# LCSL/nys-koop-lqr

Hardware: AMD Instinct MI355X
Metric: Nyström-Koopman fits/sec (K_nm build + A,B,C solve), N=1e5 m=2000 d=384 (higher is better)
Workload: dtype f64

## Files before the change

### include/nyskoop.h

```cpp
#ifndef NYSKOOP_H
#define NYSKOOP_H

#include <stdint.h>

#ifdef __cplusplus
extern "C" {
#endif

#define NK_ABI_VERSION 2

enum {
  NK_OK = 0,
  NK_ERR_BAD_ARG = -1,
  NK_ERR_HIP = -2,
  NK_ERR_NOT_SPD = -3,
  NK_ERR_OOM = -4,
  NK_ERR_NO_CONVERGENCE = -5,
  NK_ERR_NO_DEVICE = -6
};

enum { NK_KERNEL_RBF = 0, NK_KERNEL_MATERN52 = 1, NK_KERNEL_LINEAR = 2, NK_KERNEL_TPS = 3 };

typedef struct nk_kernel_desc {
  int32_t type;
  int32_t d;
  int32_t n_lengthscale;
  int32_t reserved;
  const double* lengthscale;
  double sigma0;
} nk_kernel_desc;

typedef struct nk_fit_stats {
  double ms_total;
  double ms_upload;
  double ms_kmat;
  double ms_gram;
  double ms_sqrt;
  double ms_solve;
  double ms_gram_kernel_avg;
  int32_t gram_kernel_launches;
  int32_t sqrt_iters;
  double sqrt_residual;
  double gram_flops;
  double kmat_pairs;
  int32_t rank_inner;
  int32_t rank_inner_rec;
  double pivot_ratio_inner;
  double pivot_ratio_inner_rec;
  int32_t refined;
  int32_t reserved_;
  double refine_ratio_inner;
  double refine_ratio_inner_rec;
} nk_fit_stats;

typedef struct nk_ctx nk_ctx;
typedef struct nk_model nk_model;

int nk_version(void);
const char* nk_last_error(void);
int nk_device_count(void);
int nk_create(int device, nk_ctx** out);
int nk_destroy(nk_ctx* ctx);
int nk_synchronize(nk_ctx* ctx);
void* nk_stream(nk_ctx* ctx);
int nk_set_kmat_mode(nk_ctx* ctx, int mode);
int nk_set_strict_spd(nk_ctx* ctx, int strict);
int nk_set_refine(nk_ctx* ctx, double pivot_ratio, int32_t steps);
#define NK_DTYPE_F64 0
#define NK_DTYPE_F32 1
int nk_set_compute_dtype(nk_ctx* ctx, int dtype);
int nk_wait_stream(nk_ctx* ctx, void* producer_stream);
int nk_group_create(int device, int size, nk_ctx** members);
typedef struct nk_cv_unit {
  const nk_kernel_desc* kernel;
  double gamma;
  double jitter;
  int32_t m;
  int32_t reserved;
  int64_t test_begin, test_end;
  const int64_t* landmark_rows;
} nk_cv_unit;
int nk_cv_grid(nk_ctx* const* members, int32_t n_members, const double* X, int64_t ldx, const double* Y, int64_t ldy,
               int64_t n, int32_t d, int32_t p, const nk_cv_unit* units, int32_t n_units, double* scores, int32_t* status);
typedef struct nk_spline_cv_unit {
  double gamma;
  int32_t m;
  int32_t reserved;
  int64_t test_begin, test_end;
  const double* centers;
} nk_spline_cv_unit;
int nk_spline_cv_grid(nk_ctx* const* members, int32_t n_members, const double* X, int64_t ldx, const double* Y,
                      int64_t ldy, int64_t n, int32_t d, int32_t p, const nk_spline_cv_unit* units, int32_t n_units,
                      double* scores, int32_t* status);
typedef struct nk_sysid_unit {
  const nk_kernel_desc* kernel;
  double gamma, jitter;
  int32_t m, n_ranges;
  const int64_t* row_ranges;
  const int64_t* landmark_rows;
  const double* centers;
  const int32_t* traj;
  int32_t n_traj, reserved;
} nk_sysid_unit;
int nk_sysid_grid(nk_ctx* const* members, int32_t n_members, const double* X, int64_t ldx, const double* Y, int64_t ldy,
                  int64_t n, int32_t d, int32_t p, const double* trajs, const double* U, int32_t n_trajs, int32_t T,
                  const nk_sysid_unit* units, int32_t n_units, double* err_abs, double* err_rel, int32_t* status);
int nk_group_enter(nk_ctx* member);
int nk_group_leave(nk_ctx* member);
int nk_group_stats(nk_ctx* member, uint64_t* out4);
int nk_runtime_counters(uint64_t* out, int32_t n);
int nk_shutdown(void);

void* nk_host_alloc(uint64_t bytes);
void nk_host_free(void* ptr);

int nk_kernel_matrix(nk_ctx* ctx, const nk_kernel_desc* kd,
                     const double* A, int64_t lda, int64_t nA,
                     const double* B, int64_t ldb, int64_t nB,
                     double* out, int64_t ldo);

int nk_nystrom_fit(nk_ctx* ctx, const nk_kernel_desc* kd,
                   const double* X, int64_t ldx, const double* Y, int64_t ldy,
                   int64_t n, int32_t d, int32_t p,
                   const int64_t* row_ranges, int32_t n_ranges,
                   const double* Zin, int64_t ldzi, const double* Zout, int64_t ldzo, int32_t m,
                   double gamma, double jitter,
                   nk_model** model, nk_fit_stats* stats);

int nk_gram_doubles(int32_t m, int32_t d, int32_t p, int64_t* count);
int nk_nystrom_gram(nk_ctx* ctx, const nk_kernel_desc* kd,
                    const double* X, int64_t ldx, const double* Y, int64_t ldy,
                    int64_t n, int32_t d, int32_t p,
                    const int64_t* row_ranges, int32_t n_ranges,
                    const double* Zin, int64_t ldzi, const double* Zout, int64_t ldzo, int32_t m,
                    double* gram, nk_fit_stats* stats);
int nk_nystrom_solve(nk_ctx* ctx, const nk_kernel_desc* kd,
                     const double* Zin, int64_t ldzi, const double* Zout, int64_t ldzo, int32_t m, int32_t d, int32_t p,
                     const double* gram, int64_t n_total, double gamma, double jitter,
                     nk_model** model, nk_fit_stats* stats);

int nk_model_create(nk_ctx* ctx, const nk_kernel_desc* kd, const double* Zout, int64_t ldz,
                    int32_t m, int32_t d, int32_t p, double jitter,
                    const double* A, const double* B, const double* C, const double* W,
                    nk_model** model);
int nk_model_destroy(nk_model* model);

int nk_spline_fit(nk_ctx* ctx, const double* X, int64_t ldx, const double* Y, int64_t ldy, int64_t n, int32_t d, int32_t p,
                  const int64_t* row_ranges, int32_t n_ranges, const double* centers, int64_t ldc, int32_t m, double gamma,
                  nk_model** model, nk_fit_stats* stats);
int nk_spline_model_create(nk_ctx* ctx, const double* centers, int64_t ldc, int32_t m, int32_t d, int32_t p,
                           const double* A, const double* B, const double* C, const double* W, nk_model** model);

int nk_model_get(nk_ctx* ctx, const nk_model* model, char which, double* out, int64_t ldo);
int nk_model_dims(const nk_model* model, int32_t* m, int32_t* d, int32_t* p);
int nk_model_get_ops(nk_ctx* ctx, const nk_model* model, double* G, int64_t ldg, double* C, int64_t ldc, double* W,
                     int64_t ldw);
int nk_model_get_ops_async(nk_ctx* ctx, nk_model* model, double* G, int64_t ldg, double* C, int64_t ldc, double* W,
                           int64_t ldw);
int nk_model_wait(nk_model* model);

int nk_lift(nk_ctx* ctx, const nk_model* model, const double* Xq, int64_t ldx, int64_t nq,
            double* out, int64_t ldo);

int nk_predict(nk_ctx* ctx, const nk_model* model, const double* Xaug, int64_t ldx, int64_t nq,
               double* out, int64_t ldo);

int nk_score_neg_rmse(nk_ctx* ctx, const nk_model* model, const double* Xaug, int64_t ldx,
                      const double* Ytrue, int64_t ldy, int64_t nq, double* score);

int nk_rollout(nk_ctx* ctx, const nk_model* model, const double* x0, int64_t ldx0,
               const double* U, int32_t T, int32_t batch, double* out_x, double* out_z);

int nk_rollout_err(nk_ctx* ctx, const nk_model* model, const double* traj, const double* U, int32_t T, int32_t batch,
                   double* err_abs, double* err_rel);

int nk_closed_loop(nk_ctx* ctx, const nk_model* model, const double* K, const double* phi0,
                   const double* phi_ref, int32_t steps, double* out_x, double* out_u);
int nk_closed_loop_batch(nk_ctx* ctx, const nk_model* model, const double* K, const double* phi0,
                         const double* phi_ref, int32_t steps, int32_t batch, double* out_x, double* out_u);
#define NK_PLANT_DUFFING 0
#define NK_PLANT_DOUBLE_INTEGRATOR 1
#define NK_PLANT_HJB 2
int nk_plant_step(int plant, double Ts, const double* x, const double* u, double* x_next);
int nk_plant_loop(nk_ctx* ctx, const nk_model* model, int plant, double Ts, const double* K, const double* x0,
                  const double* x_ref, int32_t steps, int32_t batch, double* out_x, double* out_u);
typedef struct nk_plant_unit {
  const nk_model* model;
  const double* K;
  const double* x0;
  const double* x_ref;
  int32_t uopt;
  int32_t reserved;
} nk_plant_unit;
int nk_plant_loop_multi(nk_ctx* ctx, int plant, double Ts, int32_t steps, const nk_plant_unit* units, int32_t n_units,
                        const double* u_opt, int32_t n_uopt, double* out_x, double* out_u, double* scores);
#define NK_DARE_WS_CAP_BYTES (1ll << 30)
typedef struct nk_dare_problem {
  int32_t m, p;
  const double* A; int64_t lda;
  const double* B; int64_t ldb;
  const double* Q; int64_t ldq;
  const double* R; int64_t ldr;
  double* out_K;
  double* out_P;
  double* out_delta;
} nk_dare_problem;
int nk_dare_batch(nk_ctx* ctx, const nk_dare_problem* problems, int32_t n, double tol, int32_t max_iter,
                  int32_t* out_status, int32_t* out_iters);
int nk_model_lqr_gain_batch(nk_ctx* ctx, const nk_model* const* models, int32_t n, double c, const double* R_or_NULL,
                            double tol, int32_t max_iter, double* out_K, int32_t* out_status, int32_t* out_iters);
int nk_model_lqr_cost(nk_ctx* ctx, const nk_model* model, double c, double* Q, int64_t ldq);
int nk_linear_rollout(nk_ctx* ctx, const double* A, const double* B, const double* C, int32_t m, int32_t d, int32_t p,
                      const double* z0, const double* U, int32_t T, int32_t batch, double* out_x, double* out_z);

int nk_gemm_f32(nk_ctx* ctx, int64_t M, int64_t N, int64_t K, const float* A, int64_t lda, const float* B, int64_t ldb,
                double* C, int64_t ldc);
int nk_gemm(nk_ctx* ctx, int transA, int transB, int64_t M, int64_t N, int64_t K, double alpha,
            const double* A, int64_t lda, const double* B, int64_t ldb, double beta, double* C, int64_t ldc);
int nk_sqrtm_spd(nk_ctx* ctx, const double* P, int64_t ldp, int32_t m, double* S, double* Sinv,
                 int32_t* iters, double* residual);
int nk_solve_spd(nk_ctx* ctx, const double* P, int64_t ldp, int32_t m, const double* R, int64_t ldr,
                 int32_t nrhs, double* X, int64_t ldxo);

int nk_bench_gram(nk_ctx* ctx, int64_t n, int32_t m, int32_t p, int32_t d, int32_t reps, double* ms_avg, double* flop);

#define NK_CHOL_FLOW_GIVEUP (-0x40000000)
int nk_chol_aug(nk_ctx* ctx, int32_t nsys, const double* const* P, const int64_t* ldp, const int32_t* m,
                const double* const* R, const int32_t* extra, double* const* L, double* const* X, int32_t* failed,
                double* piv_ratio);

#ifdef __cplusplus
}
#endif
#endif
```

### nys_koop_lqr_amd/_lib.py

```python
import atexit
import ctypes as C
import os
import sys
import threading

import numpy as np

_HERE = os.path.dirname(os.path.abspath(__file__))

NK_KERNEL_RBF, NK_KERNEL_MATERN52, NK_KERNEL_LINEAR, NK_KERNEL_TPS = 0, 1, 2, 3
NK_PLANT_DUFFING, NK_PLANT_DOUBLE_INTEGRATOR, NK_PLANT_HJB = 0, 1, 2
NK_OK = 0
_ERR_NAMES = {-1: "NK_ERR_BAD_ARG", -2: "NK_ERR_HIP", -3: "NK_ERR_NOT_SPD", -4: "NK_ERR_OOM",
              -5: "NK_ERR_NO_CONVERGENCE", -6: "NK_ERR_NO_DEVICE"}


class NyskoopError(RuntimeError):
    def __init__(self, code, msg):
        super().__init__(f"{_ERR_NAMES.get(code, code)}: {msg}")
        self.code = code


class KernelDesc(C.Structure):
    _fields_ = [("type", C.c_int32), ("d", C.c_int32), ("n_lengthscale", C.c_int32), ("reserved", C.c_int32),
                ("lengthscale", C.POINTER(C.c_double)), ("sigma0", C.c_double)]


class CvUnit(C.Structure):
    _fields_ = [("kernel", C.POINTER(KernelDesc)), ("gamma", C.c_double), ("jitter", C.c_double), ("m", C.c_int32),
                ("reserved", C.c_int32), ("test_begin", C.c_int64), ("test_end", C.c_int64),
                ("landmark_rows", C.POINTER(C.c_int64))]


class SplineCvUnit(C.Structure):
    _fields_ = [("gamma", C.c_double), ("m", C.c_int32), ("reserved", C.c_int32), ("test_begin", C.c_int64),
                ("test_end", C.c_int64), ("centers", C.POINTER(C.c_double))]


class SysidUnit(C.Structure):
    _fields_ = [("kernel", C.POINTER(KernelDesc)), ("gamma", C.c_double), ("jitter", C.c_double), ("m", C.c_int32),
                ("n_ranges", C.c_int32), ("row_ranges", C.POINTER(C.c_int64)), ("landmark_rows", C.POINTER(C.c_int64)),
                ("centers", C.POINTER(C.c_double)), ("traj", C.POINTER(C.c_int32)), ("n_traj", C.c_int32),
                ("reserved", C.c_int32)]


class PlantUnit(C.Structure):
    _fields_ = [("model", C.c_void_p), ("K", C.c_void_p), ("x0", C.c_void_p), ("x_ref", C.c_void_p),
                ("uopt", C.c_int32), ("reserved", C.c_int32)]


class DareProblem(C.Structure):
    _fields_ = [("m", C.c_int32), ("p", C.c_int32), ("A", C.c_void_p), ("lda", C.c_int64), ("B", C.c_void_p),
                ("ldb", C.c_int64), ("Q", C.c_void_p), ("ldq", C.c_int64), ("R", C.c_void_p), ("ldr", C.c_int64),
                ("out_K", C.c_void_p), ("out_P", C.c_void_p), ("out_delta", C.c_void_p)]


class FitStats(C.Structure):
    _fields_ = [("ms_total", C.c_double), ("ms_upload", C.c_double), ("ms_kmat", C.c_double),
                ("ms_gram", C.c_double), ("ms_sqrt", C.c_double), ("ms_solve", C.c_double),
                ("ms_gram_kernel_avg", C.c_double), ("gram_kernel_launches", C.c_int32),
                ("sqrt_iters", C.c_int32), ("sqrt_residual", C.c_double), ("gram_flops", C.c_double),
                ("kmat_pairs", C.c_double), ("rank_inner", C.c_int32), ("rank_inner_rec", C.c_int32),
                ("pivot_ratio_inner", C.c_double), ("pivot_ratio_inner_rec", C.c_double), ("refined", C.c_int32),
                ("reserved_", C.c_int32), ("refine_ratio_inner", C.c_double), ("refine_ratio_inner_rec", C.c_double)]

    def as_dict(self):
        return {k: getattr(self, k) for k, _ in self._fields_}


_P = C.c_void_p
_I64 = C.c_int64
_I32 = C.c_int32
_D = C.c_double

SIGNATURES = {
    "nk_version": (C.c_int, []),
    "nk_last_error": (C.c_char_p, []),
    "nk_device_count": (C.c_int, []),
    "nk_create": (C.c_int, [C.c_int, C.POINTER(_P)]),
    "nk_destroy": (C.c_int, [_P]),
    "nk_synchronize": (C.c_int, [_P]),
    "nk_stream": (_P, [_P]),
    "nk_set_kmat_mode": (C.c_int, [_P, C.c_int]),
    "nk_set_strict_spd": (C.c_int, [_P, C.c_int]),
    "nk_set_refine": (C.c_int, [_P, C.c_double, C.c_int32]),
    "nk_wait_stream": (C.c_int, [_P, _P]),
    "nk_shutdown": (C.c_int, []),
    "nk_group_create": (C.c_int, [C.c_int, C.c_int, C.POINTER(_P)]),
    "nk_group_enter": (C.c_int, [_P]),
    "nk_group_leave": (C.c_int, [_P]),
    "nk_set_compute_dtype": (C.c_int, [_P, C.c_int]),
    "nk_group_stats": (C.c_int, [_P, C.POINTER(C.c_uint64)]),
    "nk_runtime_counters": (C.c_int, [C.POINTER(C.c_uint64), C.c_int32]),
    "nk_cv_grid": (C.c_int, [C.POINTER(_P), _I32, _P, _I64, _P, _I64, _I64, _I32, _I32, C.POINTER(CvUnit), _I32,
                             C.POINTER(_D), C.POINTER(_I32)]),
    "nk_spline_cv_grid": (C.c_int, [C.POINTER(_P), _I32, _P, _I64, _P, _I64, _I64, _I32, _I32, C.POINTER(SplineCvUnit),
                                    _I32, C.POINTER(_D), C.POINTER(_I32)]),
    "nk_sysid_grid": (C.c_int, [C.POINTER(_P), _I32, _P, _I64, _P, _I64, _I64, _I32, _I32, _P, _P, _I32, _I32,
                                C.POINTER(SysidUnit), _I32, C.POINTER(_D), C.POINTER(_D), C.POINTER(_I32)]),
    "nk_host_alloc": (_P, [C.c_uint64]),
    "nk_host_free": (None, [_P]),
    "nk_kernel_matrix": (C.c_int, [_P, C.POINTER(KernelDesc), _P, _I64, _I64, _P, _I64, _I64, _P, _I64]),
    "nk_nystrom_fit": (C.c_int, [_P, C.POINTER(KernelDesc), _P, _I64, _P, _I64, _I64, _I32, _I32,
                                 C.POINTER(_I64), _I32, _P, _I64, _P, _I64, _I32, _D, _D,
                                 C.POINTER(_P), C.POINTER(FitStats)]),
    "nk_gram_doubles": (C.c_int, [_I32, _I32, _I32, C.POINTER(_I64)]),
    "nk_nystrom_gram": (C.c_int, [_P, C.POINTER(KernelDesc), _P, _I64, _P, _I64, _I64, _I32, _I32,
                                  C.POINTER(_I64), _I32, _P, _I64, _P, _I64, _I32, _P, C.POINTER(FitStats)]),
    "nk_nystrom_solve": (C.c_int, [_P, C.POINTER(KernelDesc), _P, _I64, _P, _I64, _I32, _I32, _I32, _P, _I64, _D, _D,
                                   C.POINTER(_P), C.POINTER(FitStats)]),
    "nk_model_create": (C.c_int, [_P, C.POINTER(KernelDesc), _P, _I64, _I32, _I32, _I32, _D, _P, _P, _P, _P,
                                  C.POINTER(_P)]),
    "nk_spline_fit": (C.c_int, [_P, _P, _I64, _P, _I64, _I64, _I32, _I32, C.POINTER(_I64), _I32, _P, _I64, _I32, _D,
                                C.POINTER(_P), C.POINTER(FitStats)]),
    "nk_spline_model_create": (C.c_int, [_P, _P, _I64, _I32, _I32, _I32, _P, _P, _P, _P, C.POINTER(_P)]),
    "nk_model_destroy": (C.c_int, [_P]),
    "nk_model_get": (C.c_int, [_P, _P, C.c_char, _P, _I64]),
    "nk_model_dims": (C.c_int, [_P, C.POINTER(_I32), C.POINTER(_I32), C.POINTER(_I32)]),
    "nk_model_get_ops": (C.c_int, [_P, _P, _P, _I64, _P, _I64, _P, _I64]),
    "nk_model_get_ops_async": (C.c_int, [_P, _P, _P, _I64, _P, _I64, _P, _I64]),
    "nk_model_wait": (C.c_int, [_P]),
    "nk_lift": (C.c_int, [_P, _P, _P, _I64, _I64, _P, _I64]),
    "nk_predict": (C.c_int, [_P, _P, _P, _I64, _I64, _P, _I64]),
    "nk_score_neg_rmse": (C.c_int, [_P, _P, _P, _I64, _P, _I64, _I64, C.POINTER(_D)]),
    "nk_rollout": (C.c_int, [_P, _P, _P, _I64, _P, _I32, _I32, _P, _P]),
    "nk_rollout_err": (C.c_int, [_P, _P, _P, _P, _I32, _I32, C.POINTER(_D), C.POINTER(_D)]),
    "nk_closed_loop": (C.c_int, [_P, _P, _P, _P, _P, _I32, _P, _P]),
    "nk_closed_loop_batch": (C.c_int, [_P, _P, _P, _P, _P, _I32, _I32, _P, _P]),
    "nk_plant_step": (C.c_int, [C.c_int, _D, _P, _P, _P]),
    "nk_plant_loop": (C.c_int, [_P, _P, C.c_int, _D, _P, _P, _P, _I32, _I32, _P, _P]),
    "nk_plant_loop_multi": (C.c_int, [_P, C.c_int, _D, _I32, C.POINTER(PlantUnit), _I32, _P, _I32, _P, _P, _P]),
    "nk_dare_batch": (C.c_int, [_P, C.POINTER(DareProblem), _I32, _D, _I32, C.POINTER(_I32), C.POINTER(_I32)]),
    "nk_model_lqr_gain_batch": (C.c_int, [_P, C.POINTER(_P), _I32, _D, _P, _D, _I32, _P, C.POINTER(_I32),
                                          C.POINTER(_I32)]),
    "nk_model_lqr_cost": (C.c_int, [_P, _P, _D, _P, _I64]),
    "nk_linear_rollout": (C.c_int, [_P, _P, _P, _P, _I32, _I32, _I32, _P, _P, _I32, _I32, _P, _P]),
    "nk_gemm_f32": (C.c_int, [_P, _I64, _I64, _I64, _P, _I64, _P, _I64, _P, _I64]),
    "nk_gemm": (C.c_int, [_P, C.c_int, C.c_int, _I64, _I64, _I64, _D, _P, _I64, _P, _I64, _D, _P, _I64]),
    "nk_sqrtm_spd": (C.c_int, [_P, _P, _I64, _I32, _P, _P, C.POINTER(_I32), C.POINTER(_D)]),
    "nk_solve_spd": (C.c_int, [_P, _P, _I64, _I32, _P, _I64, _I32, _P, _I64]),
    "nk_bench_gram": (C.c_int, [_P, _I64, _I32, _I32, _I32, _I32, C.POINTER(_D), C.POINTER(_D)]),
    "nk_chol_aug": (C.c_int, [_P, _I32, _P, _P, _P, _P, _P, _P, _P, _P, _P]),
}

_lib = None
_lib_lock = threading.Lock()


def library_path():
    return os.environ.get("NYSKOOP_LIB", os.path.join(_HERE, "libnyskoop.so"))


def load_library():
    global _lib
    with _lib_lock:
        if _lib is None:
            path = library_path()
            if not os.path.exists(path):
                raise NyskoopError(-6, f"{path} not found: build it with `python -c 'import __graft_entry__ as g; "
                                       f"g.build()'` or `make -C nys_koop_lqr_amd/csrc` (there is no CPU fallback)")
            if os.environ.get("NYSKOOP_PRELOAD_TORCH", "1") == "1" and "torch" not in sys.modules:
                try:
                    import torch
                except Exception:
                    pass
            lib = C.CDLL(path)
            for name, (res, args) in SIGNATURES.items():
                fn = getattr(lib, name)
                fn.restype = res
                fn.argtypes = args
            _lib = lib
            atexit.register(shutdown)
    return _lib


def shutdown():
    lib = _lib
    if lib is None:
        return
    with _pools_lock:
        pools = list(_pools.values())
        _pools.clear()
        lpools = list(_lockstep_pools.values())
        _lockstep_pools.clear()
    for pool in pools:
        pool.shutdown(wait=True)
    for pool in lpools:
        pool.close()
    _PinnedBlock.drain()
    lib.nk_shutdown()


def check(rc):
    if rc != NK_OK:
        raise NyskoopError(rc, load_library().nk_last_error().decode("utf-8", "replace"))


def runtime_counters():
    v = (C.c_uint64 * 5)()
    check(load_library().nk_runtime_counters(v, 5))
    return dict(chain_giveups=int(v[0]), jacobi_giveups=int(v[1]), rank_truncated_fits=int(v[2]), sqrt_retries=int(v[3]),
                refined_fits=int(v[4]))


def torch_if_cuda():
    try:
        import torch
    except Exception:
        return None
    try:
        return torch if torch.cuda.is_available() else None
    except Exception:
        return None


class Mat:

    def __init__(self, obj, rows=None, cols=None):
        if hasattr(obj, "data_ptr") and hasattr(obj, "stride"):
            if str(getattr(obj, "dtype", "")).split(".")[-1] not in ("float64", "double"):
                raise TypeError("device tensors must be float64")
            if obj.dim() != 2 or (obj.shape[1] > 1 and obj.stride(1) != 1):
                raise ValueError("device tensors must be 2-D with unit inner stride")
            self.owner, self.ptr, self.ld = obj, obj.data_ptr(), int(obj.stride(0))
            self.shape = (int(obj.shape[0]), int(obj.shape[1]))
        else:
            a = np.asarray(obj, dtype=np.float64)
            if a.ndim == 1:
                a = a.reshape(1, -1)
            if a.ndim != 2:
                raise ValueError("expected a 2-D array")
            if a.shape[1] > 0 and a.shape[0] > 0 and (a.strides[1] != 8 or a.strides[0] % 8 or a.strides[0] < 8 * a.shape[1]):
                a = np.ascontiguousarray(a)
            self.owner, self.ptr = a, a.ctypes.data
            self.ld = a.strides[0] // 8 if a.shape[0] > 1 else max(a.shape[1], 1)
            self.shape = a.shape
        if self.shape[0] <= 1:
            self.ld = max(self.ld, self.shape[1], 1)
        if rows is not None and self.shape[0] != rows or cols is not None and self.shape[1] != cols:
            raise ValueError(f"expected a {rows} x {cols} matrix, got {self.shape}")


class Context:

    def __init__(self, device=0, handle=None):
        self.lib = load_library()
        if handle is None:
            handle = _P()
            check(self.lib.nk_create(int(device), C.byref(handle)))
        self.handle = handle
        self.device = int(device)

    def enter(self):
        check(self.lib.nk_group_enter(self.handle))

# ... 445 lines not shown
```

### nys_koop_lqr_amd/csrc/nk_api.hip

```cpp
#include "nk_common.h"
#include "nk_api_internal.h"

#include <cmath>
#include <cstdarg>
#include <cstdio>
#include <cstring>
#include <cstdlib>
#include <algorithm>
#include <mutex>
#include <set>

namespace nk {

static thread_local std::string g_err;

void set_error(const char* fmt, ...) {
  char buf[1024];
  va_list ap;
  va_start(ap, fmt);
  vsnprintf(buf, sizeof(buf), fmt, ap);
  va_end(ap);
  g_err = buf;
}

// ... 477 lines not shown

int nk_set_compute_dtype(nk_ctx* ctx, int dtype) {
  NK_REQUIRE(ctx != nullptr && (dtype == NK_DTYPE_F64 || dtype == NK_DTYPE_F32), "nk_set_compute_dtype: bad argument");
  ctx->compute_f32 = dtype == NK_DTYPE_F32 ? 1 : 0;
  return NK_OK;
}

int nk_set_strict_spd(nk_ctx* ctx, int strict) {
  NK_REQUIRE(ctx != nullptr && strict >= 0 && strict <= 2, "nk_set_strict_spd: bad argument");
  ctx->strict_spd = strict;
  return NK_OK;
}

int nk_set_refine(nk_ctx* ctx, double pivot_ratio, int32_t steps) {
  NK_REQUIRE(ctx != nullptr && pivot_ratio >= 0.0 && pivot_ratio <= 1.0 && steps >= 0 && steps <= 8, "nk_set_refine: bad argument");
  ctx->refine_pivot = pivot_ratio;
  ctx->refine_steps = steps;
  return NK_OK;
}

int nk_wait_stream(nk_ctx* ctx, void* producer_stream) {
  NK_REQUIRE(ctx != nullptr, "nk_wait_stream: null context");
  NK_HIP(hipSetDevice(ctx->device));
  if (ctx->group) {
    hipError_t e = real_stream_sync(reinterpret_cast<hipStream_t>(producer_stream));
    if (e != hipSuccess) { set_error("synchronising the producer stream failed: %s", hipGetErrorString(e)); return NK_ERR_HIP; }
    return NK_OK;
  }
  NK_HIP(hipEventRecord(ctx->ev_ext, reinterpret_cast<hipStream_t>(producer_stream)));
  NK_HIP(hipStreamWaitEvent(ctx->stream_main, ctx->ev_ext, 0));
  NK_HIP(hipStreamWaitEvent(ctx->stream_side, ctx->ev_ext, 0));
  NK_HIP(hipStreamWaitEvent(ctx->stream_prep, ctx->ev_ext, 0));
  NK_HIP(hipStreamWaitEvent(ctx->stream_copy, ctx->ev_ext, 0));
  return NK_OK;
}

int nk_group_create(int device, int size, nk_ctx** out) {
  NK_REQUIRE(out != nullptr && size >= 1 && size <= 256, "nk_group_create: bad argument");
  for (int i = 0; i < size; ++i) out[i] = nullptr;
  for (int i = 0; i < size; ++i) {
    int rc = nk_create(device, &out[i]);
    if (rc != NK_OK) {
      for (int j = 0; j < i; ++j) { nk_destroy(out[j]); out[j] = nullptr; }
      return rc;
    }
  }
  nk_group* g = group_new(device, size);
  if (!g) {
    for (int i = 0; i < size; ++i) { nk_destroy(out[i]); out[i] = nullptr; }
    set_error("nk_group_create: could not create the shared stream / argument table");
    return NK_ERR_HIP;
  }
  for (int i = 0; i < size; ++i) group_attach(g, i, out[i]);
  return NK_OK;
}

int nk_group_enter(nk_ctx* ctx) {
  NK_REQUIRE(ctx != nullptr, "nk_group_enter: null context");
  return group_enter(ctx);
}

int nk_group_leave(nk_ctx* ctx) {
  NK_REQUIRE(ctx != nullptr, "nk_group_leave: null context");
  tl_ctx = ctx;
  const int rc = group_leave(ctx);
  tl_ctx = nullptr;
  return rc;
}

int nk_runtime_counters(uint64_t* out, int32_t n) {
  NK_REQUIRE(out != nullptr && n >= 0, "nk_runtime_counters: bad argument");
  for (int i = 0; i < n && i < CNT_N; ++i) out[i] = nk::read_counter(i);
  return NK_OK;
}

int nk_group_stats(nk_ctx* ctx, uint64_t* out4) {
  NK_REQUIRE(ctx != nullptr && out4 != nullptr, "nk_group_stats: null argument");
  group_stats(ctx, out4);
  return NK_OK;
}

int nk_synchronize(nk_ctx* ctx) {
  NK_REQUIRE(ctx != nullptr, "null context");
  tl_ctx = ctx;
  NK_HIP(hipStreamSynchronize(ctx->stream));
  return NK_OK;
}

void* nk_stream(nk_ctx* ctx) { return ctx ? reinterpret_cast<void*>(ctx->stream) : nullptr; }

void* nk_host_alloc(uint64_t bytes) {
  void* p = nullptr;
  if (hipHostMalloc(&p, bytes ? bytes : 1, hipHostMallocDefault) != hipSuccess) {
    (void)hipGetLastError();
    set_error("hipHostMalloc of %llu bytes failed", (unsigned long long)bytes);
    return nullptr;
  }
  std::lock_guard<std::mutex> lk(g_reg_mu);
  g_host_blocks.insert(p);
  return p;
}

void nk_host_free(void* ptr) {
  if (!ptr) return;
  {
    std::lock_guard<std::mutex> lk(g_reg_mu);
    if (g_host_blocks.erase(ptr) == 0) return;
  }
  (void)hipHostFree(ptr);
}

int nk_set_kmat_mode(nk_ctx* ctx, int mode) {
  NK_REQUIRE(ctx != nullptr && (mode == 0 || mode == 1), "nk_set_kmat_mode: bad argument");
  ctx->kmat_mode = mode;
  return NK_OK;
}

int nk_kernel_matrix(nk_ctx* ctx, const nk_kernel_desc* kd, const double* A, int64_t lda, int64_t nA, const double* B,
                     int64_t ldb, int64_t nB, double* out, int64_t ldo) {
  NK_TRY(check_ctx(ctx));
  NK_REQUIRE(kd && A && B && out, "nk_kernel_matrix: null argument");
  NK_REQUIRE(nA >= 0 && nB >= 0 && kd->d > 0, "nk_kernel_matrix: negative size");
  NK_REQUIRE(lda >= kd->d && ldb >= kd->d && ldo >= nB, "nk_kernel_matrix: leading dimension too small");
  if (nA == 0 || nB == 0) return NK_OK;
  const int d = kd->d;
  double* winv = nullptr;
  NK_TRY(arena_alloc_t(ctx, (size_t)d, &winv));
  NK_TRY(make_winv(ctx, kd, d, winv));
  MatIn a, b;
  NK_TRY(stage_in(ctx, A, lda, nA, d, &a));
  NK_TRY(stage_in(ctx, B, ldb, nB, d, &b));
  MatOut o;
  NK_TRY(stage_out(ctx, out, ldo, nA, nB, &o));
  if (kd->type == NK_KERNEL_TPS && ctx->kmat_mode == 0 && d >= 32 && nA >= 2 && nB >= 2) {
    const int64_t lta = (nA + 1) & ~(int64_t)1, ltb = (nB + 1) & ~(int64_t)1;
    double *center = nullptr, *At = nullptr, *sqa = nullptr, *Bt = nullptr, *sqb = nullptr;
    NK_TRY(arena_alloc_t(ctx, (size_t)d, &center));
    NK_TRY(arena_alloc_t(ctx, (size_t)d * lta, &At));
    NK_TRY(arena_alloc_t(ctx, (size_t)nA, &sqa));
    NK_TRY(arena_alloc_t(ctx, (size_t)d * ltb, &Bt));
    NK_TRY(arena_alloc_t(ctx, (size_t)nB, &sqb));
    NK_TRY(launch_colmean(ctx, b.ptr, b.ld, (int)nB, d, center));
    NK_TRY(prep_rows(ctx, a.ptr, a.ld, nA, d, winv, center, At, lta, sqa));
    NK_TRY(prep_rows(ctx, b.ptr, b.ld, nB, d, winv, center, Bt, ltb, sqb));
    NK_TRY(launch_kmat_gram(ctx, NK_KERNEL_TPS, At, lta, sqa, nA, Bt, ltb, sqb, nB, d, 0.0, o.dev, o.ld));
  } else {
    NK_TRY(launch_kmat(ctx, kd->type, a.ptr, a.ld, nA, b.ptr, b.ld, nB, d, winv, kd->sigma0, o.dev, o.ld));
  }
  NK_TRY(finish_out(ctx, o));
  NK_HIP(hipStreamSynchronize(ctx->stream));
  return NK_OK;
}

int nk_model_create(nk_ctx* ctx, const nk_kernel_desc* kd, const double* Zout, int64_t ldz, int32_t m, int32_t d,
                    int32_t p, double jitter, const double* A, const double* B, const double* C, const double* W,
                    nk_model** model) {
  NK_TRY(check_ctx(ctx));
  NK_REQUIRE(kd && Zout && model, "nk_model_create: null argument");
  NK_REQUIRE(m > 0 && d > 0 && p >= 0 && ldz >= d, "nk_model_create: bad sizes");
  NK_REQUIRE(kd->type != NK_KERNEL_TPS, "nk_model_create: spline models come from nk_spline_model_create");
  *model = nullptr;
  nk_model* mdl = nullptr;
  NK_TRY(model_alloc(ctx, m, d, p, &mdl));
  struct Guard { nk_model* m; ~Guard() { if (m) nk_model_destroy(m); } } guard{mdl};
  mdl->ktype = kd->type; mdl->sigma0 = kd->sigma0; mdl->jitter = jitter;
  NK_TRY(make_winv(ctx, kd, d, mdl->winv));
  MatIn z;
  NK_TRY(stage_in(ctx, Zout, ldz, m, d, &z));
  NK_TRY(launch_copy2d(ctx, z.ptr, z.ld, mdl->Z, d, m, d));
  double* Kj = nullptr;
  NK_TRY(arena_alloc_t(ctx, (size_t)m * m, &Kj));
  NK_TRY(launch_kmat(ctx, kd->type, mdl->Z, d, m, mdl->Z, d, m, d, mdl->winv, kd->sigma0, Kj, m));
  NK_TRY(launch_add_diag(ctx, Kj, m, m, jitter));
  NK_TRY(sqrtm_spd(ctx, Kj, m, m, mdl->S, mdl->Sinv, nullptr, nullptr));
  const int mp = m + p;
  if (A && C) {
    NK_REQUIRE(p == 0 || B != nullptr, "nk_model_create: B missing");
    MatIn a, b, c, w;
    NK_TRY(stage_in(ctx, A, m, m, m, &a));
    NK_TRY(launch_copy2d(ctx, a.ptr, a.ld, mdl->A, mp, m, m));
    if (p > 0) {
      NK_TRY(stage_in(ctx, B, p, m, p, &b));
      NK_TRY(launch_copy2d(ctx, b.ptr, b.ld, mdl->B, mp, m, p));
    }
    NK_TRY(stage_in(ctx, C, m, d, m, &c));
    NK_TRY(launch_copy2d(ctx, c.ptr, c.ld, mdl->C, m, d, m));
    if (W) {
      NK_TRY(stage_in(ctx, W, mp, d, mp, &w));
      NK_TRY(launch_copy2d(ctx, w.ptr, w.ld, mdl->W, mp, d, mp));
    } else {
      NK_TRY(launch_gemm(ctx, false, false, d, mp, m, 1.0, mdl->C, m, mdl->A, mp, 0.0, mdl->W, mp));
    }
    mdl->has_ops = true;
  }
  NK_HIP(hipStreamSynchronize(ctx->stream));
  guard.m = nullptr;
  *model = mdl;
  return NK_OK;
}

int nk_spline_model_create(nk_ctx* ctx, const double* centers, int64_t ldc, int32_t m, int32_t d, int32_t p,
                           const double* A, const double* B, const double* C, const double* W, nk_model** model) {
  NK_TRY(check_ctx(ctx));
  NK_REQUIRE(centers && model, "nk_spline_model_create: null argument");
  NK_REQUIRE(m > 0 && d > 0 && p >= 0 && ldc >= d, "nk_spline_model_create: bad sizes");
  *model = nullptr;
  nk_model* mdl = nullptr;
  NK_TRY(model_alloc(ctx, m, d, p, &mdl, NK_MODEL_SPLINE));
  struct Guard { nk_model* m; ~Guard() { if (m) nk_model_destroy(m); } } guard{mdl};
  mdl->ktype = NK_KERNEL_TPS; mdl->sigma0 = 0.0; mdl->jitter = 0.0;
  NK_TRY(launch_fill(ctx, mdl->winv, d, 1, d, 1.0));
  MatIn z;
  NK_TRY(stage_in(ctx, centers, ldc, m, d, &z));
  NK_TRY(launch_copy2d(ctx, z.ptr, z.ld, mdl->Z, d, m, d));
  const int mp = m + p;
  if (A && C) {
    NK_REQUIRE(p == 0 || B != nullptr, "nk_spline_model_create: B missing");
    MatIn a, b, c, w;
    NK_TRY(stage_in(ctx, A, m, m, m, &a));
    NK_TRY(launch_copy2d(ctx, a.ptr, a.ld, mdl->A, mp, m, m));
    if (p > 0) {
      NK_TRY(stage_in(ctx, B, p, m, p, &b));
      NK_TRY(launch_copy2d(ctx, b.ptr, b.ld, mdl->B, mp, m, p));
    }
    NK_TRY(stage_in(ctx, C, m, d, m, &c));
    NK_TRY(launch_copy2d(ctx, c.ptr, c.ld, mdl->C, m, d, m));
    if (W) {
      NK_TRY(stage_in(ctx, W, mp, d, mp, &w));
      NK_TRY(launch_copy2d(ctx, w.ptr, w.ld, mdl->W, mp, d, mp));
    } else {
      NK_TRY(launch_gemm(ctx, false, false, d, mp, m, 1.0, mdl->C, m, mdl->A, mp, 0.0, mdl->W, mp));
    }
    mdl->has_ops = true;
  }
  NK_HIP(hipStreamSynchronize(ctx->stream));
  guard.m = nullptr;
  *model = mdl;
  return NK_OK;
}

int nk_model_destroy(nk_model* model) {
  if (!model) return NK_OK;
  {
    std::lock_guard<std::mutex> lk(g_reg_mu);
    if (g_models.erase(model) == 0) return NK_OK;
  }
  destroy_model_unregistered(model, true);
  return NK_OK;
}

int nk_model_dims(const nk_model* model, int32_t* m, int32_t* d, int32_t* p) {
  NK_REQUIRE(model != nullptr, "null model");
  if (m) *m = model->m;
  if (d) *d = model->d;
  if (p) *p = model->p;
  return NK_OK;
}

int nk_model_get(nk_ctx* ctx, const nk_model* mdl, char which, double* out, int64_t ldo) {
  NK_TRY(check_ctx(ctx));
  NK_REQUIRE(mdl && out, "nk_model_get: null argument");
  const int m = mdl->m, d = mdl->d, p = mdl->p, mp = m + p;
  const double* src = nullptr;
  int64_t lds = 0, rows = 0, cols = 0;
  switch (which) {
    case 'A': src = mdl->A; lds = mp; rows = m; cols = m; break;
    case 'B': src = mdl->B; lds = mp; rows = m; cols = p; break;
    case 'C': src = mdl->C; lds = m; rows = d; cols = m; break;
    case 'W': src = mdl->W; lds = mp; rows = d; cols = mp; break;
    case 'S': src = mdl->S; lds = m; rows = m; cols = m; break;
    case 'I': src = mdl->Sinv; lds = m; rows = m; cols = m; break;
  }
  if ((which == 'S' || which == 'I') && mdl->kind == NK_MODEL_SPLINE) {
    set_error("nk_model_get: a spline model has no K_mm^{1/2} / K_mm^{-1/2} ('%c')", which);
    return NK_ERR_BAD_ARG;
  }
  switch (which) {
    case 'A': case 'B': case 'C': case 'W': case 'S': case 'I': break;
    case 'Z': src = mdl->Z; lds = d; rows = m; cols = d; break;
    default: set_error("nk_model_get: unknown selector '%c'", which); return NK_ERR_BAD_ARG;
  }
  if ((which == 'A' || which == 'B' || which == 'C' || which == 'W') && !mdl->has_ops) {
    set_error("nk_model_get: model holds no fitted operators");
    return NK_ERR_BAD_ARG;
  }
  if (rows == 0 || cols == 0) return NK_OK;
  NK_REQUIRE(ldo >= cols, "nk_model_get: leading dimension too small");
  NK_HIP(hipMemcpy2DAsync(out, (size_t)ldo * 8, src, (size_t)lds * 8, (size_t)cols * 8, (size_t)rows,
                          is_device_ptr(out) ? hipMemcpyDeviceToDevice : hipMemcpyDeviceToHost, ctx->stream));
  NK_HIP(hipStreamSynchronize(ctx->stream));
  return NK_OK;
}

int nk_model_get_ops(nk_ctx* ctx, const nk_model* mdl, double* G, int64_t ldg, double* Cm, int64_t ldc, double* W,
                     int64_t ldw) {
  NK_TRY(check_ctx(ctx));
  NK_REQUIRE(mdl != nullptr, "nk_model_get_ops: null model");
  if (!mdl->has_ops) {
    set_error("nk_model_get_ops: model holds no fitted operators");
    return NK_ERR_BAD_ARG;
  }
  const int m = mdl->m, d = mdl->d, mp = m + mdl->p;
  NK_REQUIRE((!G || ldg >= mp) && (!Cm || ldc >= m) && (!W || ldw >= mp), "nk_model_get_ops: leading dimension too small");
  auto copy = [&](double* dst, int64_t ldd, const double* src, int64_t lds, int64_t rows, int64_t cols,
                  hipStream_t st) -> hipError_t {
    const hipMemcpyKind kind = is_device_ptr(dst) ? hipMemcpyDeviceToDevice : hipMemcpyDeviceToHost;
// ... 368 lines not shown
```

### nys_koop_lqr_amd/csrc/nk_common.h

```cpp
#pragma once
#include <hip/hip_runtime.h>
#include <stdint.h>
#include <stddef.h>
#include <string>
#include <vector>

#include "nyskoop.h"
#include "nk_lockstep.h"

namespace nk {

void set_error(const char* fmt, ...);

#define NK_HIP(call)                                                                         \
  do {                                                                                       \
    hipError_t e_ = (call);                                                                  \
    if (e_ != hipSuccess) {                                                                  \
      nk::set_error("%s failed: %s (%s:%d)", #call, hipGetErrorString(e_), __FILE__, __LINE__); \
      return e_ == hipErrorOutOfMemory ? NK_ERR_OOM : NK_ERR_HIP;                            \
    }                                                                                        \
  } while (0)

#define NK_TRY(call)            \
  do {                          \
// ... 56 lines not shown
  nk::Arena arena;
  nk::Arena arena_side;
  nk::Arena* cur_arena = nullptr;
  hipStream_t stream_la[2] = {nullptr, nullptr};
  hipEvent_t ev_la[2][4] = {};
  int compute_f32 = 0;
  hipEvent_t ev_fork = nullptr, ev_join = nullptr, ev_chain = nullptr;
  int* d_info = nullptr;
  unsigned long long* d_piv = nullptr;
  unsigned long long* h_piv = nullptr;
  double* d_scalars = nullptr;
  double* h_scalars = nullptr;
  int* h_info = nullptr;
  double* d_zeros = nullptr;
  hipEvent_t ev[EV_COUNT];
  int num_cu = 256;
  int kmat_mode = 0;
  double refine_pivot = 0.0;
  int refine_steps = 2;
  int strict_spd = 0;
  hipEvent_t ev_ext = nullptr;
  hipEvent_t ev_up[8] = {};
  nk_group* group = nullptr;
  nk_member_state* gstate = nullptr;
  int* d_flow[2] = {nullptr, nullptr};
  size_t flow_words[2] = {0, 0};
  bool spline_defer_svd = false;
  bool chol_flow_off = false;
  double* h_stage = nullptr;
  size_t h_stage_bytes = 0;
};

enum { NK_MODEL_NYSTROM = 0, NK_MODEL_SPLINE = 1 };
struct nk_model {
  int device = 0;
  int32_t m = 0, d = 0, p = 0;
  int32_t ktype = 0;
  double sigma0 = 0.0;
  double jitter = 0.0;
  double* buf = nullptr;
  size_t bytes = 0;
  double *A = nullptr, *B = nullptr, *C = nullptr, *W = nullptr, *S = nullptr, *Sinv = nullptr, *Z = nullptr,
         *winv = nullptr;
  bool has_ops = false;
  int32_t kind = 0;
  hipEvent_t ev_fetch = nullptr;
};

namespace nk {

struct SideScope {
  nk_ctx* c;
  hipStream_t s0;
  Arena* a0;
  explicit SideScope(nk_ctx* ctx, hipStream_t s = nullptr) : c(ctx), s0(ctx->stream), a0(ctx->cur_arena) {
    c->stream = s ? s : c->stream_side;
    c->cur_arena = &c->arena_side;
  }
  ~SideScope() {
    c->stream = s0;
    c->cur_arena = a0;
  }
};

struct ChainOnly {
  nk_ctx* c;
  bool b0;
  explicit ChainOnly(nk_ctx* ctx) : c(ctx), b0(ctx->chol_flow_off) { c->chol_flow_off = true; }
  ~ChainOnly() { c->chol_flow_off = b0; }
};

inline int info_base(const nk_ctx* c) { return c->stream != c->stream_main ? 2 : 0; }

__device__ __forceinline__ double exp_nonpos_ca() {
  double ca = __longlong_as_double(0x3e5ade156a5dcb37LL);
  asm volatile("" : "+v"(ca));
  return ca;
}
__device__ __forceinline__ double exp_nonpos(double x, double ca_v) {
  const double k = __builtin_rint(x * __longlong_as_double(0x3ff71547652b82feLL));
  double r = __builtin_fma(__longlong_as_double((long long)0xbfe62e42fefa39efULL), k, x);
  r = __builtin_fma(__longlong_as_double((long long)0xbc7abc9e3b39803fULL), k, r);
  double p;
#define NK_EXP_STEP(c) asm("v_fma_f64 %0, %1, %2, %3" : "=v"(p) : "v"(r), "v"(p), "s"(c))
  asm("v_fma_f64 %0, %1, %2, %3" : "=v"(p) : "v"(r), "v"(ca_v), "s"(__longlong_as_double(0x3e928af3fca7ab0cLL)));
  NK_EXP_STEP(__longlong_as_double(0x3ec71dee623fde64LL));
  NK_EXP_STEP(__longlong_as_double(0x3efa01997c89e6b0LL));
  NK_EXP_STEP(__longlong_as_double(0x3f2a01a014761f6eLL));
  NK_EXP_STEP(__longlong_as_double(0x3f56c16c1852b7b0LL));
  NK_EXP_STEP(__longlong_as_double(0x3f81111111122322LL));
  NK_EXP_STEP(__longlong_as_double(0x3fa55555555502a1LL));
  NK_EXP_STEP(__longlong_as_double(0x3fc5555555555511LL));
  NK_EXP_STEP(__longlong_as_double(0x3fe000000000000bLL));
#undef NK_EXP_STEP
  p = __builtin_fma(r, p, 1.0);
  p = __builtin_fma(r, p, 1.0);
  return x < -1075.0 ? 0.0 : ldexp(p, (int)k);
}
__device__ __forceinline__ double exp_nonpos(double x) { return exp_nonpos(x, exp_nonpos_ca()); }

__host__ __device__ __forceinline__ double log_pos(double x) {
#pragma clang fp contract(off)
  const double ln2_hi = 6.93147180369123816490e-01, ln2_lo = 1.90821492927058770002e-10;
  const double Lg1 = 6.666666666666735130e-01, Lg2 = 3.999999999940941908e-01, Lg3 = 2.857142874366239149e-01,
               Lg4 = 2.222219843214978396e-01, Lg5 = 1.818357216161805012e-01, Lg6 = 1.531383769920937332e-01,
               Lg7 = 1.479819860511658591e-01;
  uint64_t bits;
  __builtin_memcpy(&bits, &x, 8);
  int32_t hx = (int32_t)(bits >> 32);
  int k = 0;
  if (hx < 0x00100000) {
    x *= 1.80143985094819840000e+16;
    k -= 54;
    __builtin_memcpy(&bits, &x, 8);
    hx = (int32_t)(bits >> 32);
  }
  k += (hx >> 20) - 1023;
  hx &= 0x000fffff;
  const int32_t i = (hx + 0x95f64) & 0x100000;
  bits = ((uint64_t)(uint32_t)(hx | (i ^ 0x3ff00000)) << 32) | (bits & 0xffffffffULL);
  __builtin_memcpy(&x, &bits, 8);
  k += i >> 20;
  const double f = x - 1.0;
  const double dk = (double)k;
  if ((0x000fffff & (2 + hx)) < 3) {
    if (f == 0.0) return k == 0 ? 0.0 : dk * ln2_hi + dk * ln2_lo;
    const double R = f * f * (0.5 - 0.33333333333333333 * f);
    return k == 0 ? f - R : dk * ln2_hi - ((R - dk * ln2_lo) - f);
  }
  const double s = f / (2.0 + f);
  const double z = s * s;
  const double w = z * z;
  const double t1 = w * (Lg2 + w * (Lg4 + w * Lg6));
  const double t2 = z * (Lg1 + w * (Lg3 + w * (Lg5 + w * Lg7)));
  const double R = t2 + t1;
  if (((hx - 0x6147a) | (0x6b851 - hx)) > 0) {
    const double hfsq = 0.5 * f * f;
    return k == 0 ? f - (hfsq - s * (hfsq + R)) : dk * ln2_hi - ((hfsq - (s * (hfsq + R) + dk * ln2_lo)) - f);
  }
  return k == 0 ? f - s * (f - R) : dk * ln2_hi - ((s * (f - R) - dk * ln2_lo) - f);
}
__host__ __device__ __forceinline__ double tps_value(double r2) {
#pragma clang fp contract(off)
  return r2 > 0.0 ? r2 * log_pos(sqrt(r2)) : 0.0;
}

nk_group* group_new(int device, int size);
void group_attach(nk_group* g, int slot, nk_ctx* c);
void group_detach(nk_ctx* c);
int group_enter(nk_ctx* c);
int group_leave(nk_ctx* c);
void group_stats(nk_ctx* c, uint64_t out[4]);
enum { CNT_CHAIN_GIVEUP = 0, CNT_JACOBI_GIVEUP = 1, CNT_RANK_TRUNCATED = 2, CNT_SQRT_RETRY = 3, CNT_REFINED = 4,
       CNT_CHOL_FLOW_GIVEUP = 5, CNT_CHOL_FLOW = 6, CNT_N = 7 };
void count_event(int which);
uint64_t read_counter(int which);
hipError_t real_stream_sync(hipStream_t s);
hipError_t real_event_sync(hipEvent_t e);

int arena_reset(nk_ctx* ctx);
ArenaMark arena_mark(nk_ctx* ctx);
void arena_release(nk_ctx* ctx, ArenaMark mk);
int arena_alloc(nk_ctx* ctx, size_t bytes, void** out);
template <typename T>
inline int arena_alloc_t(nk_ctx* ctx, size_t count, T** out) {
  return arena_alloc(ctx, count * sizeof(T), reinterpret_cast<void**>(out));
}
bool is_device_ptr(const void* p);

int launch_kmat(nk_ctx* ctx, int ktype, const double* A, int64_t lda, int64_t nA, const double* B, int64_t ldb,
                int64_t nB, int d, const double* winv, double sigma0, double* out, int64_t ldo);

enum { TRI_FULL = 0, TRI_UPPER_MIRROR = 1, TRI_LOWER = 2 };
struct GemmOpts {
  int tri = TRI_FULL;
  int splitk = 0;
};
int launch_gemm(nk_ctx* ctx, bool transA, bool transB, int64_t M, int64_t N, int64_t K, double alpha, const double* A,
                int64_t lda, const double* B, int64_t ldb, double beta, double* C, int64_t ldc,
                const GemmOpts& opts = GemmOpts(), float* ms_kernel = nullptr);

struct GemmCall {
  int64_t M = 0, N = 0, K = 0;
  double alpha = 1.0, beta = 0.0;
  const double* A = nullptr;
  const double* B = nullptr;
  double* C = nullptr;
  int64_t lda = 0, ldb = 0, ldc = 0;
  GemmOpts opts;
};
int launch_gemm_pair(nk_ctx* ctx, bool transA, bool transB, const GemmCall* calls, int ncalls);

struct TnSkip;
int launch_add_diag(nk_ctx* ctx, double* A, int64_t lda, int n, double v);
int launch_copy2d(nk_ctx* ctx, const double* src, int64_t lds, double* dst, int64_t ldd, int64_t rows, int64_t cols);
int launch_axpby2d(nk_ctx* ctx, double a, const double* X, int64_t ldx, double b, double* Y, int64_t ldy,
                   int64_t rows, int64_t cols);
int launch_scale_add_identity(nk_ctx* ctx, double a, const double* X, int64_t ldx, double c, double* Y, int64_t ldy,
                              int n, const TnSkip* skip = nullptr);
int launch_fill(nk_ctx* ctx, double* A, int64_t lda, int64_t rows, int64_t cols, double v);
int launch_frob_minus_identity(nk_ctx* ctx, const double* M, int64_t ldm, int n, double* d_out,
                               const TnSkip* skip = nullptr);
int launch_max_abs_rowsum(nk_ctx* ctx, const double* M, int64_t ldm, int n, double* d_out);
int launch_colsum_sqdiff(nk_ctx* ctx, const double* P, int64_t ldp, const double* Y, int64_t ldy, int64_t rows,
                         int cols, double* d_colsum);

int sqrtm_spd(nk_ctx* ctx, const double* P, int64_t ldp, int m, double* S, double* Sinv, int* iters, double* resid);
struct SqrtPlan {
  const double* P = nullptr;
  int64_t ldp = 0;
  int m = 0;
  double* W = nullptr;
  double* Linv = nullptr;
  double* X0 = nullptr;
  double* X0t = nullptr;
  double* d_sc = nullptr;
  ArenaMark mark{0, 0};
  bool deferred = false;
  int rc = 0, iters = 0, kmax = 0;
  double resid = 0.0;
  double lambda_min_hint = 0.0;
  bool early = false;
  int info_slot = 2;
  bool flow_gave_up = false;
  hipEvent_t pause_event = nullptr;
  int pause_step = -1;
};
constexpr int NK_SQRT_RETRY = 1;
int sqrtm_spd_coupled(nk_ctx* ctx, const double* P, int64_t ldp, int m, double* S, double* Sinv, int* iters, double* resid);
int sqrtm_prepare(nk_ctx* ctx, const double* P, int64_t ldp, int m, SqrtPlan* plan);
int sqrtm_finish(nk_ctx* ctx, SqrtPlan* plan, double* S, double* Sinv);
int sqrtm_verdict(nk_ctx* ctx, SqrtPlan* plan, int* iters, double* resid);
int cholesky_lower(nk_ctx* ctx, double* P, int64_t ldp, int m, double* Linv );
int cholesky_solve(nk_ctx* ctx, const double* L, int64_t ldl, int m, const double* Linv, double* R, int64_t ldr,
                   int nrhs);
struct CholSys {
  double* P = nullptr;
  int64_t ldp = 0;
  int m = 0;
  int extra = 0;
  bool backward = true;
  double* Linv = nullptr;
  double* pivlog = nullptr;
  double* R = nullptr;
  int64_t ldr = 0;
  int nrhs = 0;
};
int cholesky_lower_pair(nk_ctx* ctx, const CholSys* sys, int nsys);
int cholesky_lower_pair_async(nk_ctx* ctx, const CholSys* sys, int nsys);
int cholesky_check_pair(nk_ctx* ctx, const CholSys* sys, int nsys);
int cholesky_solve_pair(nk_ctx* ctx, const CholSys* sys, int nsys);
int cholesky_aug_pair_async(nk_ctx* ctx, const CholSys* sys, int nsys, hipEvent_t pause = nullptr, int pause_step = -1);
constexpr int CHOL_NB = 64;
constexpr int CHOL_WS = 2 * CHOL_NB * CHOL_NB + 8;
constexpr double CHOL_FIX_KAPPA = 8.0 * CHOL_NB;
inline int chol_fix_enabled() {
  const char* e = getenv("NYSKOOP_CHOL_FIX");
  return (e && e[0] == '0') ? 0 : ((e && e[0] == '2') ? 2 : 1);
}
bool launch_chol_trail_pair(nk_ctx* ctx, const GemmCall* calls, int ncalls, int* rc);
bool launch_chol_trail_potrf_pair(nk_ctx* ctx, const GemmCall* calls, int ncalls, const int* nb, double* const* Linv, int blk,
                                  double* const* plog, int* rc);
inline bool chol_fuse_enabled() {
  const char* e = getenv("NYSKOOP_CHOL_FUSE");
  return !(e && e[0] == '0');
}
bool chol_flow_enabled();
int cholesky_flow_pair(nk_ctx* ctx, const CholSys* sys, int nsys);
constexpr int CHOL_FLOW_GIVEUP = -0x40000000;
bool launch_chol_panel_pair(nk_ctx* ctx, const GemmCall* calls, int ncalls, int* rc);
int launch_trsm_right_lower_pair(nk_ctx* ctx, const CholSys* sys, int nsys);

struct PinvInfo {
  int rank = 0, sweeps = 0;
  bool converged = false;
  double sigma_max = 0.0, sigma_min_kept = 0.0, sigma_min = 0.0;
};
int pinv_right_divide(nk_ctx* ctx, const double* P, int64_t ldp, int m, const double* E, int64_t lde, int rows,
                      double* E_out, int64_t ldeo, double rcond, PinvInfo* info);
int cholesky_fail_flags(nk_ctx* ctx, const CholSys* sys, int nsys, int* failed , double* piv_ratio = nullptr);

int launch_lifted_step(nk_ctx* ctx, const double* G, int64_t ldg, int m, int mz, int pu, const double* z, int64_t zstride,
                       const double* u, int64_t ustride, const double* bias, double* out, int64_t ostride, int batch);

struct ChainArgs {
  const double* G = nullptr; int64_t ldg = 0; int m = 0, pu = 0;
  const double* z0 = nullptr; int64_t z0_stride = 0;
  bool lift = false;
  const double* x0 = nullptr; int64_t x0_stride = 0;
  const double* Zl = nullptr; int d = 0; const double* winv = nullptr; const double* Sinv = nullptr; int ktype = 0;
  double sigma0 = 0.0;
  const double* U = nullptr; int64_t u_stride = 0;
  const double* bias = nullptr; int64_t bias_stride = 0;
  double* Zall = nullptr; int64_t z_stride = 0;
  int T = 0, batch = 0;
};
int launch_ref_minus_traj(nk_ctx* ctx, const double* ref, int64_t ref_stride, const double* Phi, int64_t phi_stride,
                          double* D, int64_t d_stride, int steps, int m, int batch);
bool lifted_chain_ok(int m, int pu, int d_lift);
int traj_err_tile(int m);
int launch_traj_err(nk_ctx* ctx, const double* Zall, int64_t z_stride, const double* Cop, int64_t ldc, const double* Xtrue,
                    int64_t x_stride, int m, int d, int T, int batch, double* out);
int launch_lifted_chain(nk_ctx* ctx, const ChainArgs& a);
bool lifted_chain_mw_ok(const nk_ctx* ctx, int m, int pu);
int chain_mw_workgroups(int m);
int chain_mw_group(int m, int batch);
int launch_lifted_chain_mw(nk_ctx* ctx, const ChainArgs& a);
int lifted_chain_mw_reset(nk_ctx* ctx);
int lifted_chain_mw_fetch_status(nk_ctx* ctx);
bool lifted_chain_mw_timed_out(nk_ctx* ctx, int* row, int* step, int* traj);

int plant_loop_max_m();
int launch_plant_loop(nk_ctx* ctx, const nk_model* mdl, int plant, double Ts, const double* w, const double* x0,
                      int64_t x0_stride, const double* xref, int64_t xref_stride, int steps, int batch, double* out_x,
                      int64_t ldx, double* out_u, int64_t ldu);
struct PlantLoopUnit {
  const double* Z;
  const double* winv;
  const double* w;
  const double* x0;
  const double* xref;
  double* out_x;
  double* out_u;
  const double* u_opt;
  double* score;
  int64_t ldx, ldu;
  double sigma0sq;
  int m, reserved;
};
int launch_plant_loop_multi(nk_ctx* ctx, int plant, double Ts, int steps, PlantLoopUnit* units, const int* ktypes,
                            int n_units);

constexpr int DARE_MAX_M = 256;
constexpr int DARE_MAX_P = 8;
struct DareRec {
  const double* A; int64_t lda;
  const double* B; int64_t ldb;
  const double* Q; int64_t ldq;
  const double* C; int64_t ldc;
  const double* R;
  double c;
  double* ws;
  double* outK;
  double* outP;
  double* delta;
  int* status;
  int* iters;
  int m, p, M, d;
  int q_only;
  int reserved;
};
inline int dare_pad(int m) { return (m + 15) & ~15; }
inline size_t dare_ws_doubles(int M) { return (size_t)7 * M * M; }
int launch_dare(nk_ctx* ctx, const DareRec* table_dev, int count, double tol, int max_iter);

}

namespace nk {
enum { KTRIM_NONE = 0, KTRIM_B_UPPER = 1 , KTRIM_A_LOWER = 2  };
struct TnProblem {
  const double* A = nullptr;
  const double* B = nullptr;
  double* C = nullptr;
  int64_t lda = 0, ldb = 0, ldc = 0;
  int M = 0, N = 0;
  int tri = TRI_FULL;
  int ktrim = 0;
  double alpha = 1.0, beta = 0.0;
  double* Ct = nullptr;
  int64_t ldct = 0;
  const double* A_even = nullptr;
  const double* B_even = nullptr;
  double* Caff = nullptr;
  double aff_a = 0.0, aff_c = 0.0;
};
struct TnSkip {
  const double* state = nullptr;
  int step = 0;
  const double* select = nullptr;
  double* resid_partials = nullptr;
  int* resid_count = nullptr;
};
bool tn_fast_ok(const TnProblem& p);
struct TnProblemF {
  const float* A = nullptr;
  const float* B = nullptr;
  double* C = nullptr;
  int64_t lda = 0, ldb = 0, ldc = 0;
  int M = 0, N = 0;
  int tri = TRI_FULL;
  double beta = 0.0;
};
bool tnf_fast_ok(const TnProblemF& p);
int launch_gemm_tn_f32_multi(nk_ctx* ctx, const TnProblemF* probs, int nprob, int64_t K, int splitk ,
                             float* ms_kernel = nullptr, bool sync_timing = true);
int prep_rows_f32(nk_ctx* ctx, const double* X, int64_t ldx, int64_t rows, int d, const double* winv, const double* center,
                  float* Xt, int64_t ldt, float* sq);
int launch_cvt_f64_f32(nk_ctx* ctx, const double* src, int64_t lds_, float* dst, int64_t ldd, int64_t rows, int cols);
int launch_kmat_gram_f32(nk_ctx* ctx, int ktype, const float* At, int64_t ldat, const float* sqa, int64_t nA, const float* Bt,
                         int64_t ldbt, const float* sqb, int64_t nB, int d, double sigma0, float* out, int64_t ldo);
int launch_gemm_tn_multi(nk_ctx* ctx, const TnProblem* probs, int nprob, int64_t K, int splitk ,
                         float* ms_kernel = nullptr, bool sync_timing = true, const TnSkip* skip = nullptr);
int launch_transpose(nk_ctx* ctx, const double* src, int64_t lds, double* dst, int64_t ldd, int rows, int cols);
constexpr int refine_partial_blocks() { return 512; }
int launch_refine_apply(nk_ctx* ctx, const double* dX, int64_t ldd, double* X, int64_t ldx, int64_t rows, int64_t cols, int step,
                        double* state, double* partial);
int launch_resid_dd(nk_ctx* ctx, const double* X, int64_t ldx, const double* P, int64_t ldp, const double* R, int64_t ldr,
                    double* Res, int64_t ldres, int nr, int mq);
int launch_colmean(nk_ctx* ctx, const double* Z, int64_t ldz, int rows, int d, double* mean);
int prep_rows(nk_ctx* ctx, const double* X, int64_t ldx, int64_t rows, int d, const double* winv, const double* center,
              double* Xt, int64_t ldt, double* sq);
int launch_kmat_gram(nk_ctx* ctx, int ktype, const double* At, int64_t ldat, const double* sqa, int64_t nA,
                     const double* Bt, int64_t ldbt, const double* sqb, int64_t nB, int d, double sigma0, double* out,
                     int64_t ldo);
}

#if defined(__HIPCC__)
namespace nk {
typedef unsigned chain_u2 __attribute__((ext_vector_type(2)));
template <int CTRL> __device__ __forceinline__ double dpp_f64(double v) {
  int lo = __double2loint(v), hi = __double2hiint(v);
  lo = __builtin_amdgcn_update_dpp(0, lo, CTRL, 0xf, 0xf, true);
  hi = __builtin_amdgcn_update_dpp(0, hi, CTRL, 0xf, 0xf, true);
  return __hiloint2double(hi, lo);
}
__device__ __forceinline__ void swap16_f64(double& a, double& b) {
  const chain_u2 lo = __builtin_amdgcn_permlane16_swap((unsigned)__double2loint(a), (unsigned)__double2loint(b), false, false);
  const chain_u2 hi = __builtin_amdgcn_permlane16_swap((unsigned)__double2hiint(a), (unsigned)__double2hiint(b), false, false);
  a = __hiloint2double((int)hi.x, (int)lo.x);
  b = __hiloint2double((int)hi.y, (int)lo.y);
}
__device__ __forceinline__ void swap32_f64(double& a, double& b) {
  const chain_u2 lo = __builtin_amdgcn_permlane32_swap((unsigned)__double2loint(a), (unsigned)__double2loint(b), false, false);
  const chain_u2 hi = __builtin_amdgcn_permlane32_swap((unsigned)__double2hiint(a), (unsigned)__double2hiint(b), false, false);
  a = __hiloint2double((int)hi.x, (int)lo.x);
  b = __hiloint2double((int)hi.y, (int)lo.y);
}
__device__ __forceinline__ double wave_sum64_dpp(double c) {
  c += dpp_f64<0xB1>(c);
  c += dpp_f64<0x4E>(c);
  c += dpp_f64<0x141>(c);
  c += dpp_f64<0x140>(c);
  double a = c, b = c;
  swap16_f64(a, b);
  c = a + b;
  a = c; b = c;
  swap32_f64(a, b);
  return a + b;
}

__device__ __forceinline__ double chain_kfun(int ktype, double acc, double sigma0sq) {
  if (ktype == NK_KERNEL_RBF) return exp_nonpos(-0.5 * acc);
  if (ktype == NK_KERNEL_MATERN52) {
    const double t = sqrt(acc) * 2.23606797749978969641;
    return (1.0 + t + t * t / 3.0) * exp_nonpos(-t);
  }
  return acc + sigma0sq;
}

}
#endif
```

### nys_koop_lqr_amd/csrc/nk_fit.hip

```cpp
#include "nk_common.h"
#include "nk_api_internal.h"

#include <cmath>
#include <cstring>
#include <cstdlib>
#include <algorithm>
#include <initializer_list>

using namespace nk;

static inline size_t gram_block1(int m, int p) { return (((size_t)(2 * m + p) * (m + p)) + 1) & ~(size_t)1; }
static inline size_t gram_doubles(int m, int d, int p) { return gram_block1(m, p) + (size_t)(m + d) * m; }


static int select_rows(const char* who, const int64_t* row_ranges, int32_t n_ranges, int64_t n, std::vector<int64_t>* rng,
                       int64_t* n_eff) {
  if (row_ranges && n_ranges > 0) {
    for (int i = 0; i < n_ranges; ++i) {
      const int64_t b = row_ranges[2 * i], e = row_ranges[2 * i + 1];
      NK_REQUIRE(0 <= b && b <= e && e <= n, "%s: row range %d = [%lld,%lld) outside [0,%lld)", who, i, (long long)b,
                 (long long)e, (long long)n);
      if (e > b) { rng->push_back(b); rng->push_back(e); }
    }
  } else {
    rng->push_back(0); rng->push_back(n);
  }
  *n_eff = 0;
  for (size_t i = 0; i < rng->size(); i += 2) *n_eff += (*rng)[i + 1] - (*rng)[i];
  NK_REQUIRE(*n_eff > 0, "%s: no training rows selected", who);
  return NK_OK;
}

static int gather_ranges(nk_ctx* ctx, int d, int p, int64_t n_eff, std::vector<int64_t>* rng, MatIn* x, MatIn* y) {
  if (!(rng->size() > 2 && (double)n_eff * (2.0 * d + p) * 8.0 <= 256e6)) return NK_OK;
  const int64_t ldxg = (d + p + 1) & ~(int64_t)1, ldyg = (d + 1) & ~(int64_t)1;
  double *xg = nullptr, *yg = nullptr;
  NK_TRY(arena_alloc_t(ctx, (size_t)n_eff * ldxg, &xg));
  NK_TRY(arena_alloc_t(ctx, (size_t)n_eff * ldyg, &yg));
  int64_t o = 0;
  for (size_t i = 0; i < rng->size(); i += 2) {
    const int64_t b = (*rng)[i], len = (*rng)[i + 1] - (*rng)[i];
    NK_TRY(launch_copy2d(ctx, x->ptr + b * x->ld, x->ld, xg + o * ldxg, ldxg, len, d + p));
    NK_TRY(launch_copy2d(ctx, y->ptr + b * y->ld, y->ld, yg + o * ldyg, ldyg, len, d));
    o += len;
  }
  x->ptr = xg; x->ld = ldxg; y->ptr = yg; y->ld = ldyg;
  rng->assign({(int64_t)0, n_eff});
  return NK_OK;
}

static int64_t pass_rows_for(int64_t ldf, double bytes_per_elem) {
  const char* b = getenv("NYSKOOP_F_BUDGET_GB");
  const double budget = (b ? atof(b) : 48.0) * 1073741824.0;
  int64_t pass_rows = (int64_t)(budget / ((double)ldf * bytes_per_elem));
  if (pass_rows < 1024) pass_rows = 1024;
  return pass_rows & ~(int64_t)1023;
}

struct Piece { int64_t b, len; };
static std::vector<std::vector<Piece>> plan_passes(const std::vector<int64_t>& rng, int64_t pass_rows) {
  std::vector<std::vector<Piece>> passes(1);
  int64_t used = 0;
  for (size_t i = 0; i < rng.size(); i += 2) {
    int64_t b = rng[i];
    const int64_t e = rng[i + 1];
    while (b < e) {
      if (used == pass_rows) { passes.emplace_back(); used = 0; }
      const int64_t len = std::min(e - b, pass_rows - used);
      passes.back().push_back(Piece{b, len});
      used += len;
      b += len;
    }
  }
  return passes;
}

struct KernelBlocks {
  int ktype = 0;
  double sigma0 = 0.0;
  int d = 0, p = 0, m = 0;
  const double* winv = nullptr;
  bool gram_form = false;
  MatIn zi, zo;
  double *center = nullptr, *Rt = nullptr, *sqr = nullptr, *Zto = nullptr, *sqzo = nullptr, *Zti = nullptr, *sqzi = nullptr;
  int64_t ldt = 0, ldzt = 0;
  int64_t ldf = 0, off_out = 0;
  int copy_inputs(nk_ctx* ctx, const double* xs, int64_t ldx, int64_t len, double* Fo) const {
    if (p > 0) NK_TRY(launch_copy2d(ctx, xs + d, ldx, Fo + m, ldf, len, p));
    return NK_OK;
  }
  int piece(nk_ctx* ctx, const double* xs, int64_t ldx, const double* ys, int64_t ldy, int64_t len, double* Fo) const {
    if (gram_form) {
      NK_TRY(prep_rows(ctx, xs, ldx, len, d, winv, center, Rt, ldt, sqr));
      NK_TRY(launch_kmat_gram(ctx, ktype, Rt, ldt, sqr, len, Zti, ldzt, sqzi, m, d, sigma0, Fo, ldf));
      NK_TRY(prep_rows(ctx, ys, ldy, len, d, winv, center, Rt, ldt, sqr));
      NK_TRY(launch_kmat_gram(ctx, ktype, Rt, ldt, sqr, len, Zto, ldzt, sqzo, m, d, sigma0, Fo + off_out, ldf));
    } else {
      NK_TRY(launch_kmat(ctx, ktype, xs, ldx, len, zi.ptr, zi.ld, m, d, winv, sigma0, Fo, ldf));
      NK_TRY(launch_kmat(ctx, ktype, ys, ldy, len, zo.ptr, zo.ld, m, d, winv, sigma0, Fo + off_out, ldf));
    }
    return copy_inputs(ctx, xs, ldx, len, Fo);
  }
};

static void fill_gram_stats(nk_ctx* ctx, nk_fit_stats* stats, bool staged, bool gram_deferred, float ms_gram_kernel,
                            int gram_launches) {
  memset(stats, 0, sizeof(*stats));
  stats->ms_upload = staged ? ev_ms(ctx, EV_FIT_BEGIN, EV_STAGED) : 0.0;
  stats->ms_kmat = ev_ms(ctx, EV_STAGED, EV_KMAT_DONE);
  stats->ms_gram = ev_ms(ctx, EV_KMAT_DONE, EV_GRAM_DONE);
  if (gram_deferred) ms_gram_kernel = ev_ms(ctx, EV_GEMM_T0, EV_GEMM_T1);
  stats->ms_gram_kernel_avg = gram_launches ? ms_gram_kernel / gram_launches : 0.0;
  stats->gram_kernel_launches = gram_launches;
}

struct FitGuard {
  nk_model* m = nullptr;
  hipStream_t s[5] = {};
  int ns = 0;
  void arm(nk_model* mdl, std::initializer_list<hipStream_t> streams) {
    m = mdl;
    for (hipStream_t q : streams) s[ns++] = q;
  }
  ~FitGuard() {
    if (m) {
      for (int i = 0; i < ns; ++i) (void)hipStreamSynchronize(s[i]);
      nk_model_destroy(m);
    }
  }
};


enum { FIT_FULL = 0, FIT_GRAM = 1, FIT_SOLVE = 2 };

struct NystromFit {
  nk_ctx* ctx; const nk_kernel_desc* kd;
  const double* X; int64_t ldx; const double* Y; int64_t ldy; int64_t n; int32_t d, p;
  const int64_t* row_ranges; int32_t n_ranges;
  const double* Zin; int64_t ldzi; const double* Zout; int64_t ldzo; int32_t m;
  double gamma, jitter; nk_model** model; nk_fit_stats* stats; int mode; double* gram_io;
  HostTrace tr;
  std::vector<int64_t> rng;
  int64_t n_eff = 0;
  bool same_centers = false;
  int mp = 0;
  double gamma_n = 0.0;
  nk_model* mdl = nullptr;
  FitGuard guard;
  MatIn x, y, zi, zo;
  int host_passes = 1;
  double *Kmm = nullptr, *Kj = nullptr, *Kj_in = nullptr, *Kxo = nullptr;
  bool landmarks_aside = false;
  double *G1 = nullptr, *G2 = nullptr, *G3 = nullptr, *G4 = nullptr;
  int64_t ldd = 0;
  float ms_gram_kernel = 0.f;
  int gram_launches = 0;
  bool gram_deferred = false, timed = false;
  bool f32 = false, overlap_prep = false, multi_pass = false, pipelined = false;
  KernelBlocks kb;
  std::vector<std::vector<Piece>> passes;
  int64_t f_rows = 0, maxlen = 0, ldt32 = 0, ldzt32 = 0, ldy32 = 0;
  double *F = nullptr, *Rt2 = nullptr, *sqr2 = nullptr;
  float *F32 = nullptr, *Rt32 = nullptr, *sq32 = nullptr, *Zt32 = nullptr, *sqz32 = nullptr, *Y32 = nullptr;
  SqrtPlan splan;
  int it = 0;
  double resid = 0.0;
  double *Sinvt = nullptr, *T1t = nullptr, *X1 = nullptr;
  double *Gsave = nullptr, *V1 = nullptr, *Wc = nullptr, *Ct = nullptr;
  CholSys sys[2];
  int chol_failed[2] = {0, 0}, rank_sys[2] = {0, 0}, refined[2] = {0, 0};
  double piv_ratio[2] = {1.0, 1.0}, refine_ratio[2] = {0.0, 0.0};
  bool redo_products = false;

  int run();
  int validate(), stage_rows(), stage_landmarks(), landmark_matrices(), alloc_gram(), load_gram(), prepare_features(), run_passes();
  int upload_pass(size_t ip), pass_f32(size_t ip), pass_f64(size_t ip), blocks_overlapped(const Piece& pc, double* Fo);
  int return_gram();
  int queue_sqrt_prep(), assemble_and_factor(), queue_sqrt_side(), sqrt_products(), operator_products();
  int settle_factorisations(), refine(), settle_sqrt();
  void read_refinement(), write_stats();
};

int NystromFit::validate() {
  NK_TRY(check_ctx(ctx));
  tr.mark("check_ctx/arena_reset");
  NK_REQUIRE(kd && Zout, "nk_nystrom_fit: null argument");
  NK_REQUIRE(mode == FIT_SOLVE || (X && Y), "nk_nystrom_fit: null data pointer");
  NK_REQUIRE(mode == FIT_GRAM || model != nullptr, "nk_nystrom_fit: null model pointer");
  NK_REQUIRE(mode == FIT_FULL || gram_io != nullptr, "nk_nystrom_gram/solve: null accumulator");
  NK_REQUIRE(n > 0 && d > 0 && p >= 0 && m > 0, "nk_nystrom_fit: sizes must be positive (n=%lld d=%d p=%d m=%d)",
             (long long)n, d, p, m);
  NK_REQUIRE(mode == FIT_SOLVE || (ldx >= d + p && ldy >= d), "nk_nystrom_fit: leading dimension too small");
  NK_REQUIRE(ldzo >= d, "nk_nystrom_fit: leading dimension too small");
  NK_REQUIRE(std::isfinite(gamma) && std::isfinite(jitter), "nk_nystrom_fit: gamma/jitter not finite");
  NK_REQUIRE(kd->type != NK_KERNEL_TPS, "nk_nystrom_fit: the thin-plate spline has no Nystrom fit (nk_spline_fit)");
  if (model) *model = nullptr;
  NK_TRY(select_rows("nk_nystrom_fit", row_ranges, n_ranges, n, &rng, &n_eff));
  same_centers = (Zin == nullptr) || (Zin == Zout && ldzi == ldzo);
  mp = m + p;
  gamma_n = gamma * (double)n_eff;

  NK_TRY(model_alloc(ctx, m, d, p, &mdl));
  guard.arm(mdl, {ctx->stream_main, ctx->stream_side, ctx->stream_prep, ctx->stream_la[0], ctx->stream_la[1]});
  mdl->ktype = kd->type; mdl->sigma0 = kd->sigma0; mdl->jitter = jitter;
  tr.mark("validate + model_alloc");
  return NK_OK;
}

int NystromFit::stage_rows() {
  const char* e = getenv("NYSKOOP_HOST_PASSES");
  const int want = e ? atoi(e) : 6;
  if (want > 1 && rng.size() == 2 && !ctx_recording(ctx) && (double)n_eff * (2.0 * d + p) * 8.0 >= 64e6 &&
      !is_device_ptr(X) && !is_device_ptr(Y))
    host_passes = want > 8 ? 8 : want;
  if (host_passes > 1) {
    x.ld = (d + p + 1) & ~(int64_t)1;
    y.ld = (d + 1) & ~(int64_t)1;
    double *xd = nullptr, *yd = nullptr;
    NK_TRY(arena_alloc_t(ctx, (size_t)n * x.ld, &xd));
    NK_TRY(arena_alloc_t(ctx, (size_t)n * y.ld, &yd));
    x.ptr = xd; y.ptr = yd; x.staged = y.staged = true;
  } else {
    NK_TRY(stage_in(ctx, X, ldx, n, d + p, &x));
    NK_TRY(stage_in(ctx, Y, ldy, n, d, &y));
  }
  return gather_ranges(ctx, d, p, n_eff, &rng, &x, &y);
}

int NystromFit::stage_landmarks() {
  NK_TRY(stage_in(ctx, Zout, ldzo, m, d, &zo));
  if (same_centers) zi = zo; else NK_TRY(stage_in(ctx, Zin, ldzi, m, d, &zi));
  NK_TRY(launch_copy2d(ctx, zo.ptr, zo.ld, mdl->Z, d, m, d));
  NK_HIP(hipEventRecord(ctx->ev[EV_STAGED], ctx->stream));
  tr.mark("staging issued");
  return NK_OK;
}

int NystromFit::landmark_matrices() {
  NK_TRY(arena_alloc_t(ctx, (size_t)m * m, &Kmm));
  NK_TRY(arena_alloc_t(ctx, (size_t)m * m, &Kj));
  if (same_centers) {
    Kj_in = Kj;
    Kxo = Kmm;
  } else {
    NK_TRY(arena_alloc_t(ctx, (size_t)m * m, &Kj_in));
    NK_TRY(arena_alloc_t(ctx, (size_t)m * m, &Kxo));
  }
  {
    const char* la = getenv("NYSKOOP_LANDMARKS_ASIDE");
    landmarks_aside = mode == FIT_FULL && n_eff >= 20000 && m >= 1024 && !ctx_recording(ctx) && !(la && la[0] == '0');
  }
  hipStream_t s0 = ctx->stream;
  if (landmarks_aside) {
    NK_HIP(hipEventRecord(ctx->ev[EV_FORK], ctx->stream));
    ctx->stream = ctx->stream_prep;
    NK_HIP(hipStreamWaitEvent(ctx->stream, ctx->ev[EV_FORK], 0));
  }
  int rc_l = launch_kmat(ctx, kd->type, zo.ptr, zo.ld, m, zo.ptr, zo.ld, m, d, mdl->winv, kd->sigma0, Kmm, m);
  if (rc_l == NK_OK) rc_l = launch_copy2d(ctx, Kmm, m, Kj, m, m, m);
  if (rc_l == NK_OK) rc_l = launch_add_diag(ctx, Kj, m, m, jitter);
  if (rc_l == NK_OK && !same_centers) {
    rc_l = launch_kmat(ctx, kd->type, zi.ptr, zi.ld, m, zi.ptr, zi.ld, m, d, mdl->winv, kd->sigma0, Kj_in, m);
    if (rc_l == NK_OK) rc_l = launch_add_diag(ctx, Kj_in, m, m, jitter);
    if (rc_l == NK_OK) rc_l = launch_kmat(ctx, kd->type, zi.ptr, zi.ld, m, zo.ptr, zo.ld, m, d, mdl->winv, kd->sigma0, Kxo, m);
  }
  const hipError_t he = rc_l == NK_OK ? hipEventRecord(ctx->ev[EV_LANDMARKS], ctx->stream) : hipSuccess;
  ctx->stream = s0;
  NK_TRY(rc_l);
  NK_HIP(he);
  return NK_OK;
}

int NystromFit::alloc_gram() {
  ldd = d + (d & 1);
  NK_TRY(arena_alloc_t(ctx, gram_doubles(m, d, p), &G1));
  G2 = G1 + (size_t)mp * mp;
  G3 = G1 + gram_block1(m, p);
  G4 = G3 + (size_t)m * m;
  timed = stats != nullptr;
  return NK_OK;
}

int NystromFit::load_gram() {
  NK_HIP(hipMemcpyAsync(G1, gram_io, gram_doubles(m, d, p) * sizeof(double),
                        is_device_ptr(gram_io) ? hipMemcpyDeviceToDevice : hipMemcpyHostToDevice, ctx->stream));
  NK_HIP(hipEventRecord(ctx->ev[EV_KMAT_DONE], ctx->stream));
  return NK_OK;
}

int NystromFit::prepare_features() {
  f32 = ctx->compute_f32 != 0 && ctx->kmat_mode == 0 && d >= 32 && !ctx_recording(ctx) && m >= 4 && d >= 4;
  kb.off_out = f32 ? ((mp + 3) & ~3) : ((mp + 1) & ~1);
  kb.ldf = f32 ? ((kb.off_out + m + 3) & ~(int64_t)3) : ((kb.off_out + m + 1) & ~(int64_t)1);
  const int64_t ldf = kb.ldf;
  int64_t pass_rows = pass_rows_for(ldf, f32 ? 4.0 : 8.0);
  if (host_passes > 1) {
    const int64_t per = ((n_eff + host_passes - 1) / host_passes + 1023) & ~(int64_t)1023;
    if (per < pass_rows) pass_rows = per;
  }
  passes = plan_passes(rng, pass_rows);
  f_rows = passes.size() > 1 ? pass_rows : n_eff;
  NK_TRY(arena_alloc_t(ctx, f32 ? ((size_t)f_rows * ldf + 1) / 2 + 64 : (size_t)f_rows * ldf + 64, &F));
  kb.ktype = kd->type; kb.sigma0 = kd->sigma0; kb.d = d; kb.p = p; kb.m = m; kb.winv = mdl->winv; kb.zi = zi; kb.zo = zo;
  kb.gram_form = ctx->kmat_mode == 0 && d >= 32;
  for (auto& ps : passes) for (auto& pc : ps) maxlen = std::max(maxlen, pc.len);
  kb.ldt = (maxlen + 1) & ~(int64_t)1;
  kb.ldzt = (m + 1) & ~1;
  overlap_prep = kb.gram_form && passes.size() == 1 && passes[0].size() == 1;
  if (kb.gram_form) {
    NK_TRY(arena_alloc_t(ctx, (size_t)d, &kb.center));
    if (!f32) {
      NK_TRY(arena_alloc_t(ctx, (size_t)d * kb.ldt, &kb.Rt));
      NK_TRY(arena_alloc_t(ctx, (size_t)maxlen, &kb.sqr));
    }
    if (overlap_prep && !f32) {
      NK_TRY(arena_alloc_t(ctx, (size_t)d * kb.ldt, &Rt2));
      NK_TRY(arena_alloc_t(ctx, (size_t)maxlen, &sqr2));
    }
    NK_TRY(arena_alloc_t(ctx, (size_t)d * kb.ldzt, &kb.Zto));
    NK_TRY(arena_alloc_t(ctx, (size_t)m, &kb.sqzo));
    if (kd->type == NK_KERNEL_LINEAR) NK_TRY(launch_fill(ctx, kb.center, d, 1, d, 0.0));
    else NK_TRY(launch_colmean(ctx, zo.ptr, zo.ld, m, d, kb.center));
    NK_TRY(prep_rows(ctx, zo.ptr, zo.ld, m, d, mdl->winv, kb.center, kb.Zto, kb.ldzt, kb.sqzo));
    if (same_centers) {
      kb.Zti = kb.Zto; kb.sqzi = kb.sqzo;
    } else {
      NK_TRY(arena_alloc_t(ctx, (size_t)d * kb.ldzt, &kb.Zti));
      NK_TRY(arena_alloc_t(ctx, (size_t)m, &kb.sqzi));
      NK_TRY(prep_rows(ctx, zi.ptr, zi.ld, m, d, mdl->winv, kb.center, kb.Zti, kb.ldzt, kb.sqzi));
    }
  }
  F32 = reinterpret_cast<float*>(F);
  ldt32 = (maxlen + 3) & ~(int64_t)3; ldzt32 = (m + 3) & ~3; ldy32 = (d + 3) & ~3;
  if (f32) {
    NK_REQUIRE(same_centers, "fp32 engine: separate input landmarks are not supported");
    double* tmp = nullptr;
    NK_TRY(arena_alloc_t(ctx, ((size_t)d * ldt32 + 1) / 2 + 2, &tmp)); Rt32 = reinterpret_cast<float*>(tmp);
    NK_TRY(arena_alloc_t(ctx, ((size_t)maxlen + 1) / 2 + 2, &tmp)); sq32 = reinterpret_cast<float*>(tmp);
    NK_TRY(arena_alloc_t(ctx, ((size_t)d * ldzt32 + 1) / 2 + 2, &tmp)); Zt32 = reinterpret_cast<float*>(tmp);
    NK_TRY(arena_alloc_t(ctx, ((size_t)m + 1) / 2 + 2, &tmp)); sqz32 = reinterpret_cast<float*>(tmp);
    NK_TRY(arena_alloc_t(ctx, ((size_t)f_rows * ldy32 + 1) / 2 + 2, &tmp)); Y32 = reinterpret_cast<float*>(tmp);
    NK_TRY(prep_rows_f32(ctx, zo.ptr, zo.ld, m, d, mdl->winv, kb.center, Zt32, ldzt32, sqz32));
  }
  multi_pass = passes.size() > 1;
  pipelined = host_passes > 1;
  return NK_OK;
}

int NystromFit::upload_pass(size_t ip) {
  for (const Piece& pc : passes[ip]) {
    NK_HIP(hipMemcpy2DAsync(const_cast<double*>(x.ptr) + pc.b * x.ld, (size_t)x.ld * 8, X + pc.b * ldx, (size_t)ldx * 8,
                            (size_t)(d + p) * 8, (size_t)pc.len, hipMemcpyHostToDevice, ctx->stream_side));
    NK_HIP(hipMemcpy2DAsync(const_cast<double*>(y.ptr) + pc.b * y.ld, (size_t)y.ld * 8, Y + pc.b * ldy, (size_t)ldy * 8,
                            (size_t)d * 8, (size_t)pc.len, hipMemcpyHostToDevice, ctx->stream_side));
  }
  NK_HIP(hipEventRecord(ctx->ev_up[ip & 7], ctx->stream_side));
  return NK_OK;
}

int NystromFit::run_passes() {
  if (pipelined) {
    NK_HIP(hipEventRecord(ctx->ev[EV_FORK], ctx->stream));
    NK_HIP(hipStreamWaitEvent(ctx->stream_side, ctx->ev[EV_FORK], 0));
    NK_TRY(upload_pass(0));
  }
  for (size_t ip = 0; ip < passes.size(); ++ip) {
    if (pipelined) NK_HIP(hipStreamWaitEvent(ctx->stream, ctx->ev_up[ip & 7], 0));
    NK_TRY(f32 ? pass_f32(ip) : pass_f64(ip));
    if (pipelined && ip + 1 < passes.size()) NK_TRY(upload_pass(ip + 1));
  }
  return NK_OK;
}

int NystromFit::pass_f32(size_t ip) {
  const std::vector<Piece>& ps = passes[ip];
  const double beta = ip == 0 ? 0.0 : 1.0;
  const int64_t ldf = kb.ldf, off_out = kb.off_out;
  int64_t o32 = 0;
  for (const Piece& pc : ps) {
    const double* xs = x.ptr + pc.b * x.ld;
    const double* ys = y.ptr + pc.b * y.ld;
    NK_TRY(prep_rows_f32(ctx, xs, x.ld, pc.len, d, mdl->winv, kb.center, Rt32, ldt32, sq32));
    NK_TRY(launch_kmat_gram_f32(ctx, kd->type, Rt32, ldt32, sq32, pc.len, Zt32, ldzt32, sqz32, m, d, kd->sigma0,
                                F32 + o32 * ldf, ldf));
    NK_TRY(prep_rows_f32(ctx, ys, y.ld, pc.len, d, mdl->winv, kb.center, Rt32, ldt32, sq32));
    NK_TRY(launch_kmat_gram_f32(ctx, kd->type, Rt32, ldt32, sq32, pc.len, Zt32, ldzt32, sqz32, m, d, kd->sigma0,
                                F32 + o32 * ldf + off_out, ldf));
    if (p > 0) NK_TRY(launch_cvt_f64_f32(ctx, xs + d, x.ld, F32 + o32 * ldf + m, ldf, pc.len, p));
    NK_TRY(launch_cvt_f64_f32(ctx, ys, y.ld, Y32 + o32 * ldy32, ldy32, pc.len, d));
    o32 += pc.len;
  }
  if (ip == 0) {
    NK_HIP(hipEventRecord(ctx->ev[EV_KMAT_DONE], ctx->stream));
    tr.mark("kmat issued");
  }
  TnProblemF pf[4];
  pf[0].A = F32; pf[0].B = F32; pf[0].lda = pf[0].ldb = ldf; pf[0].M = pf[0].N = mp; pf[0].C = G1; pf[0].ldc = mp;
  pf[0].tri = TRI_UPPER_MIRROR;
  pf[1].A = F32 + off_out; pf[1].B = F32; pf[1].lda = pf[1].ldb = ldf; pf[1].M = m; pf[1].N = mp; pf[1].C = G2; pf[1].ldc = mp;
  pf[2].A = F32 + off_out; pf[2].B = F32 + off_out; pf[2].lda = pf[2].ldb = ldf; pf[2].M = pf[2].N = m; pf[2].C = G3;
  pf[2].ldc = m; pf[2].tri = TRI_UPPER_MIRROR;
  pf[3].A = Y32; pf[3].lda = ldy32; pf[3].M = d; pf[3].N = m; pf[3].C = G4; pf[3].ldc = m; pf[3].B = F32 + off_out;
  pf[3].ldb = ldf;
  for (int q = 0; q < 4; ++q) pf[q].beta = beta;
  float ms1 = 0.f;
  NK_TRY(launch_gemm_tn_f32_multi(ctx, pf, 4, o32, 0, timed ? &ms1 : nullptr, multi_pass));
  if (multi_pass) ms_gram_kernel += ms1; else gram_deferred = timed;
  gram_launches += 1;
  return NK_OK;
}

int NystromFit::blocks_overlapped(const Piece& pc, double* Fo) {
  const double* xs = x.ptr + pc.b * x.ld;
  const double* ys = y.ptr + pc.b * y.ld;
  NK_HIP(hipEventRecord(ctx->ev[EV_FORK], ctx->stream));
  {
    SideScope side(ctx);
    NK_HIP(hipStreamWaitEvent(ctx->stream, ctx->ev[EV_FORK], 0));
    NK_TRY(prep_rows(ctx, ys, y.ld, pc.len, d, mdl->winv, kb.center, Rt2, kb.ldt, sqr2));
    NK_HIP(hipEventRecord(ctx->ev[EV_YPREP_DONE], ctx->stream));
  }
  NK_TRY(prep_rows(ctx, xs, x.ld, pc.len, d, mdl->winv, kb.center, kb.Rt, kb.ldt, kb.sqr));
  NK_TRY(launch_kmat_gram(ctx, kd->type, kb.Rt, kb.ldt, kb.sqr, pc.len, kb.Zti, kb.ldzt, kb.sqzi, m, d, kd->sigma0, Fo, kb.ldf));
  NK_HIP(hipStreamWaitEvent(ctx->stream, ctx->ev[EV_YPREP_DONE], 0));
  NK_TRY(launch_kmat_gram(ctx, kd->type, Rt2, kb.ldt, sqr2, pc.len, kb.Zto, kb.ldzt, kb.sqzo, m, d, kd->sigma0,
                          Fo + kb.off_out, kb.ldf));
  return kb.copy_inputs(ctx, xs, x.ld, pc.len, Fo);
}

int NystromFit::pass_f64(size_t ip) {
  const std::vector<Piece>& ps = passes[ip];
  const double beta = ip == 0 ? 0.0 : 1.0;
  const int64_t ldf = kb.ldf, off_out = kb.off_out;
  int64_t o = 0;
  for (const Piece& pc : ps) {
    if (overlap_prep) NK_TRY(blocks_overlapped(pc, F + o * ldf));
    else NK_TRY(kb.piece(ctx, x.ptr + pc.b * x.ld, x.ld, y.ptr + pc.b * y.ld, y.ld, pc.len, F + o * ldf));
    o += pc.len;
  }
  const int64_t rows = o;
  if (ip == 0) {
    NK_HIP(hipEventRecord(ctx->ev[EV_KMAT_DONE], ctx->stream));
    tr.mark("kmat issued");
  }
  TnProblem pr[4];
  pr[0].A = F; pr[0].B = F; pr[0].lda = pr[0].ldb = ldf; pr[0].M = pr[0].N = mp; pr[0].C = G1; pr[0].ldc = mp;
  pr[0].tri = TRI_UPPER_MIRROR;
  pr[1].A = F + off_out; pr[1].B = F; pr[1].lda = pr[1].ldb = ldf; pr[1].M = m; pr[1].N = mp; pr[1].C = G2;
  pr[1].ldc = mp;
  pr[2].A = F + off_out; pr[2].B = F + off_out; pr[2].lda = pr[2].ldb = ldf; pr[2].M = pr[2].N = m; pr[2].C = G3;
  pr[2].ldc = m; pr[2].tri = TRI_UPPER_MIRROR;
  pr[3].A = y.ptr + ps[0].b * y.ld; pr[3].lda = y.ld; pr[3].M = d; pr[3].N = m; pr[3].C = G4; pr[3].ldc = m;
  pr[3].B = F + off_out; pr[3].ldb = ldf;
  for (int q = 0; q < 4; ++q) pr[q].beta = beta;
  const bool single = ps.size() == 1;
  const bool fast = tn_fast_ok(pr[0]) && tn_fast_ok(pr[1]) && tn_fast_ok(pr[2]);
  const bool fast_y = fast && tn_fast_ok(pr[3]);
  bool y_done = false;
  if (fast) {
    const int np = (single && fast_y) ? 4 : 3;
    float ms1 = 0.f;
    NK_TRY(launch_gemm_tn_multi(ctx, pr, np, rows, 0, (timed && !pipelined) ? &ms1 : nullptr, multi_pass));
    if (multi_pass) ms_gram_kernel += ms1; else gram_deferred = timed;
    gram_launches += 1;
    y_done = np == 4;
  } else {
    GemmOpts sym;
    sym.tri = TRI_UPPER_MIRROR;
    float t3[3] = {0.f, 0.f, 0.f};
    NK_TRY(launch_gemm(ctx, true, false, mp, mp, rows, 1.0, F, ldf, F, ldf, beta, G1, mp, sym, timed ? &t3[0] : nullptr));
    NK_TRY(launch_gemm(ctx, true, false, m, mp, rows, 1.0, F + off_out, ldf, F, ldf, beta, G2, mp, GemmOpts(),
                       timed ? &t3[1] : nullptr));
    NK_TRY(launch_gemm(ctx, true, false, m, m, rows, 1.0, F + off_out, ldf, F + off_out, ldf, beta, G3, m, sym,
                       timed ? &t3[2] : nullptr));
    ms_gram_kernel += t3[0] + t3[1] + t3[2];
    gram_launches += 3;
  }
  if (!y_done) {
    int64_t oo = 0;
    bool first = true;
    for (const Piece& pc : ps) {
      NK_TRY(launch_gemm(ctx, true, false, d, m, pc.len, 1.0, y.ptr + pc.b * y.ld, y.ld, F + oo * ldf + off_out, ldf,
                         (first && ip == 0) ? 0.0 : 1.0, G4, m));
      oo += pc.len;
      first = false;
    }
  }
  return NK_OK;
}

int NystromFit::return_gram() {
  NK_HIP(hipMemcpyAsync(gram_io, G1, gram_doubles(m, d, p) * sizeof(double),
                        is_device_ptr(gram_io) ? hipMemcpyDeviceToDevice : hipMemcpyDeviceToHost, ctx->stream));
  NK_HIP(hipStreamSynchronize(ctx->stream));
  if (stats) {
    fill_gram_stats(ctx, stats, x.staged || y.staged, gram_deferred, ms_gram_kernel, gram_launches);
    stats->ms_total = ev_ms(ctx, EV_FIT_BEGIN, EV_GRAM_DONE);
  }
  if (ctx->arena.chunks.size() > 1 || ctx->arena_side.chunks.size() > 1) NK_TRY(arena_reset(ctx));
  return NK_OK;
}


int NystromFit::sqrt_products() {
  NK_TRY(launch_transpose(ctx, mdl->Sinv, m, Sinvt, m, m, m));
  if (same_centers) {
    NK_TRY(launch_copy2d(ctx, mdl->S, m, T1t, m, m, m));
    NK_TRY(launch_axpby2d(ctx, -jitter, mdl->Sinv, m, 1.0, T1t, m, m, m));
  } else {
    NK_TRY(launch_transpose(ctx, Kxo, m, X1, m, m, m));
    NK_TRY(launch_gemm(ctx, true, false, m, m, m, 1.0, X1, m, mdl->Sinv, m, 0.0, T1t, m));
  }
  return NK_OK;
}

int NystromFit::queue_sqrt_prep() {
  SideScope prep(ctx, ctx->stream_prep);
  NK_HIP(hipStreamWaitEvent(ctx->stream, ctx->ev[EV_LANDMARKS], 0));
  splan.lambda_min_hint = jitter > 0.0 ? jitter : 0.0;
  if (mode == FIT_FULL && n_eff >= 20000 && m >= 1024) {
    static const double frac = getenv("NYSKOOP_PREP_PAUSE") ? atof(getenv("NYSKOOP_PREP_PAUSE")) : 0.0;
    const int nb = (m + CHOL_NB - 1) / CHOL_NB;
    if (frac < 1.0) {
      splan.pause_event = ctx->ev_fork;
      splan.pause_step = std::max(0, std::min(nb - 1, (int)(frac * nb)));
    }
  }
  NK_TRY(sqrtm_prepare(ctx, Kj, m, m, &splan));
  NK_HIP(hipEventRecord(ctx->ev[EV_SQRT_PREPARED], ctx->stream));
  return NK_OK;
}

int NystromFit::assemble_and_factor() {
  if (landmarks_aside) NK_HIP(hipStreamWaitEvent(ctx->stream, ctx->ev[EV_LANDMARKS], 0));
  NK_TRY(launch_axpby2d(ctx, gamma_n, Kj_in, m, 1.0, G1, mp, m, m));
  if (p > 0) NK_TRY(launch_add_diag(ctx, G1 + (int64_t)m * mp + m, mp, p, gamma_n));
  NK_TRY(launch_axpby2d(ctx, gamma_n, Kj, m, 1.0, G3, m, m, m));
  NK_TRY(arena_alloc_t(ctx, gram_doubles(m, d, p), &Gsave));
  NK_HIP(hipMemcpyAsync(Gsave, G1, gram_doubles(m, d, p) * sizeof(double), hipMemcpyDeviceToDevice, ctx->stream));
  double *Linv = nullptr, *Linv2 = nullptr, *pivlog = nullptr;
  const int nblk = (mp + CHOL_NB - 1) / CHOL_NB;
  NK_TRY(arena_alloc_t(ctx, (size_t)nblk * CHOL_WS, &Linv));
  NK_TRY(arena_alloc_t(ctx, (size_t)nblk * CHOL_WS, &Linv2));
  NK_TRY(arena_alloc_t(ctx, (size_t)m * m, &V1));
  NK_TRY(arena_alloc_t(ctx, (size_t)m * m, &Sinvt));
  NK_TRY(arena_alloc_t(ctx, (size_t)m * m, &T1t));
  NK_TRY(arena_alloc_t(ctx, (size_t)m * m, &X1));
  NK_TRY(arena_alloc_t(ctx, (size_t)m * ldd, &Wc));
  NK_TRY(arena_alloc_t(ctx, (size_t)m * ldd, &Ct));
  NK_TRY(arena_alloc_t(ctx, (size_t)mp + m + 4, &pivlog));
  sys[0].P = G1; sys[0].ldp = mp; sys[0].m = mp; sys[0].Linv = Linv; sys[0].extra = m;
  sys[1].P = G3; sys[1].ldp = m; sys[1].m = m; sys[1].Linv = Linv2; sys[1].extra = d;
  sys[0].pivlog = pivlog; sys[1].pivlog = pivlog + mp + (mp & 1);
  NK_TRY(cholesky_aug_pair_async(ctx, sys, 2));
  tr.mark("cholesky + solves issued");
  return NK_OK;
}

int NystromFit::queue_sqrt_side() {
  SideScope side(ctx);
  NK_HIP(hipStreamWaitEvent(ctx->stream, ctx->ev_fork, 0));
  NK_HIP(hipStreamWaitEvent(ctx->stream, ctx->ev[EV_SQRT_PREPARED], 0));
  NK_HIP(hipEventRecord(ctx->ev[EV_SQRT_BEGIN], ctx->stream));
  NK_TRY(sqrtm_finish(ctx, &splan, mdl->S, mdl->Sinv));
  NK_HIP(hipEventRecord(ctx->ev[EV_SQRT_END], ctx->stream));
  NK_TRY(sqrt_products());
  NK_HIP(hipEventRecord(ctx->ev_join, ctx->stream));
  return NK_OK;
}

int NystromFit::operator_products() {
  NK_TRY(launch_transpose(ctx, G2, mp, V1, m, m, m));
  NK_TRY(launch_gemm(ctx, true, false, m, m, m, 1.0, V1, m, T1t, m, 0.0, X1, m));
  NK_TRY(launch_gemm(ctx, true, false, m, m, m, 1.0, Sinvt, m, X1, m, 0.0, mdl->A, mp));
  if (p > 0) NK_TRY(launch_gemm(ctx, true, false, m, p, m, 1.0, Sinvt, m, G2 + m, mp, 0.0, mdl->B, mp));
  NK_TRY(launch_transpose(ctx, G4, m, Wc, ldd, d, m));
  NK_TRY(launch_gemm(ctx, true, false, m, d, m, 1.0, mdl->S, m, Wc, ldd, 0.0, Ct, ldd));
  NK_TRY(launch_transpose(ctx, Ct, ldd, mdl->C, m, m, d));
  NK_TRY(launch_gemm(ctx, true, false, d, mp, m, 1.0, Ct, ldd, mdl->A, mp, 0.0, mdl->W, mp));
// ... 404 lines not shown
```

### nys_koop_lqr_amd/csrc/nk_gemm_tn.hip

```cpp
#include "nk_common.h"
#include "nk_tn_kstep.inc"
#include "nk_tn_shared.h"

#include <cstdlib>
#include <cstring>

namespace nk {

typedef double d4 __attribute__((ext_vector_type(4)));

constexpr int TBK = 16;
constexpr int TSTRIDE = 144;
constexpr int TSTAGE = 2 * TBK * TSTRIDE;
constexpr int TN_LDS_BYTES = 2 * TSTAGE * 8;

struct TnDev {
  const double* A;
  const double* B;
  int64_t lda, ldb;
  int M, N;
  int tiles_n;
  int tri;
  int ktrim;
  int tile_begin;
  double* C;
  int64_t ldc;
  double alpha, beta;
  double* Ct;
  int64_t ldct;
  const double* A_even;
  const double* B_even;
  double* Caff;
  double aff_a, aff_c;
};
struct TnParams {
  TnDev p[TN_MAXP];
  int nprob;
  int ntiles;
  int K, splitk, klen;
  int kmask;
  int use_asm;
  const double* zeros;
  double* slab;
  const double* skip_state;
  int skip_step;
  const double* select_state;
  const double* sqa;
  const double* sqb;
  double* out;
  int64_t ldo;
  int ktype;
  double sigma0sq;
};

__device__ __forceinline__ uint64_t uniform_u64(uint64_t v) {
  return ((uint64_t)(uint32_t)__builtin_amdgcn_readfirstlane((uint32_t)(v >> 32)) << 32) |
         (uint64_t)(uint32_t)__builtin_amdgcn_readfirstlane((uint32_t)v);
}
__device__ __forceinline__ void dma_row(const double* row_base, uint32_t lane_off_bytes, uint32_t lds_addr) {
  const uint64_t rbu = uniform_u64((uint64_t)(uintptr_t)row_base);
  asm volatile("s_mov_b32 m0, %2\n\ts_nop 0\n\tglobal_load_lds_dwordx4 %0, %1"
               :
               : "v"(lane_off_bytes), "s"(rbu), "s"((uint32_t)__builtin_amdgcn_readfirstlane(lds_addr))
               : "m0");
}
__device__ __forceinline__ void dma_wait_all() { asm volatile("s_waitcnt vmcnt(0)" ::: "memory"); }

template <int EPI>
__device__ __forceinline__ void tn_body(const TnParams& P) {
  extern __shared__ __attribute__((aligned(16))) double smem[];
  const int split = blockIdx.x % P.splitk;
  const int gt = blockIdx.x / P.splitk;
  int pi = 0;
#pragma unroll
  for (int q = 1; q < TN_MAXP; ++q)
    if (q < P.nprob && gt >= P.p[q].tile_begin) pi = q;
  const TnDev pr = P.p[pi];
  int tm, tn;
  if (EPI >= 1) {
    const int xcd = blockIdx.x & 7, i = blockIdx.x >> 3;
    const int cols = (pr.tiles_n - xcd + 7) >> 3;
    if (cols <= 0) return;
    tm = i / cols;
    tn = xcd + 8 * (i - tm * cols);
    if (tm * TBM >= pr.M) return;
  } else {
    tn_tile_coords(gt - pr.tile_begin, pr.tri, pr.tiles_n, pr.M, tm, tn);
  }
  const int lane = threadIdx.x & 63;
  const int wave = __builtin_amdgcn_readfirstlane(threadIdx.x >> 6);
  if (EPI == 0 && P.skip_state != nullptr) {
    const double f = P.skip_state[0];
    if (f != 0.0 && f <= (double)P.skip_step) return;
  }
  const double* opA = pr.A;
  const double* opB = pr.B;
  if (EPI == 0 && P.select_state != nullptr && (((int)P.select_state[0]) & 1) == 0) {
    if (pr.A_even) opA = pr.A_even;
    if (pr.B_even) opB = pr.B_even;
  }
  int kbeg = split * P.klen;
  int kend = min(P.K, kbeg + P.klen);
  if (pr.ktrim == KTRIM_B_UPPER) kend = min(kend, (tn + 1) * TBM);
  if (pr.ktrim == KTRIM_A_LOWER) kbeg = max(kbeg, tm * TBM);
  const int ktiles = kend > kbeg ? (kend - kbeg + TBK - 1) / TBK : 0;

  const uint32_t offa = (uint32_t)min(tm * TBM + lane * 2, (pr.M - 1) & ~1) * 8u;
  const uint32_t offb = (uint32_t)min(tn * TBM + lane * 2, (pr.N - 1) & ~1) * 8u;
  const uint32_t offz = (uint32_t)lane * 16u;

  const uint32_t lds0 = (uint32_t)(uintptr_t)smem;
  auto issue = [&](int kt, int stage) {
    const uint32_t sa = lds0 + (uint32_t)(stage * TSTAGE) * 8u;
    const uint32_t sb = sa + (uint32_t)(TBK * TSTRIDE) * 8u;
    const int k0 = kbeg + kt * TBK;
    if (k0 + TBK <= kend) {
#pragma unroll
      for (int q = 0; q < 4; ++q) {
        const int r = wave + 4 * q;
        dma_row(opA + (int64_t)((k0 + r) & P.kmask) * pr.lda, offa, sa + (uint32_t)(r * TSTRIDE) * 8u);
        dma_row(opB + (int64_t)((k0 + r) & P.kmask) * pr.ldb, offb, sb + (uint32_t)(r * TSTRIDE) * 8u);
      }
    } else {
#pragma unroll
      for (int q = 0; q < 4; ++q) {
        const int r = wave + 4 * q;
        const int k = k0 + r;
        if (k < kend) {
          dma_row(opA + (int64_t)k * pr.lda, offa, sa + (uint32_t)(r * TSTRIDE) * 8u);
          dma_row(opB + (int64_t)k * pr.ldb, offb, sb + (uint32_t)(r * TSTRIDE) * 8u);
        } else {
          dma_row(P.zeros, offz, sa + (uint32_t)(r * TSTRIDE) * 8u);
          dma_row(P.zeros, offz, sb + (uint32_t)(r * TSTRIDE) * 8u);
        }
      }
    }
  };

  d4 acc[4][4];
#pragma unroll
  for (int i = 0; i < 4; ++i)
#pragma unroll
    for (int j = 0; j < 4; ++j) acc[i][j] = d4{0.0, 0.0, 0.0, 0.0};

  const int wm = wave >> 1, wn = wave & 1;
  const int r16 = lane & 15, g4 = lane >> 4;

  auto frag = [&](int stage, int ks, double (&a)[4], double (&b)[4]) {
    const double* a_base = smem + stage * TSTAGE + wm * 64 + r16 + (ks * 4 + g4) * TSTRIDE;
    const double* b_base = a_base + TBK * TSTRIDE + (wn - wm) * 64;
#pragma unroll
    for (int i = 0; i < 4; ++i) a[i] = a_base[i * 16];
#pragma unroll
    for (int j = 0; j < 4; ++j) b[j] = b_base[j * 16];
  };
  auto mma = [&](const double (&a)[4], const double (&b)[4]) {
#pragma unroll
    for (int i = 0; i < 4; ++i)
#pragma unroll
      for (int j = 0; j < 4; ++j)
        acc[i][j] = __builtin_amdgcn_mfma_f64_16x16x4f64(a[i], b[j], acc[i][j], 0, 0, 0);
  };
  double a0[4], b0[4], a1[4], b1[4];
  if (ktiles > 0) {
    issue(0, 0);
    dma_wait_all();
    __syncthreads();
    frag(0, 0, a0, b0);
  }
  const uint32_t ard0 = lds0 + (uint32_t)(wm * 64 + r16 + g4 * TSTRIDE) * 8u;
  const uint32_t brd0 = lds0 + (uint32_t)(TBK * TSTRIDE + wn * 64 + r16 + g4 * TSTRIDE) * 8u;
  constexpr uint32_t STAGE_B = (uint32_t)TSTAGE * 8u;
  const uint32_t stra = (uint32_t)__builtin_amdgcn_readfirstlane((uint32_t)(pr.lda * 32));
  const uint32_t strb = (uint32_t)__builtin_amdgcn_readfirstlane((uint32_t)(pr.ldb * 32));
#define NK_TN_ACC_OPERANDS                                                                                             \
  [c00] "+v"(acc[0][0]), [c01] "+v"(acc[0][1]), [c02] "+v"(acc[0][2]), [c03] "+v"(acc[0][3]), [c10] "+v"(acc[1][0]),   \
      [c11] "+v"(acc[1][1]), [c12] "+v"(acc[1][2]), [c13] "+v"(acc[1][3]), [c20] "+v"(acc[2][0]),                      \
      [c21] "+v"(acc[2][1]), [c22] "+v"(acc[2][2]), [c23] "+v"(acc[2][3]), [c30] "+v"(acc[3][0]),                      \
      [c31] "+v"(acc[3][1]), [c32] "+v"(acc[3][2]), [c33] "+v"(acc[3][3]), [a00] "+v"(a0[0]), [a01] "+v"(a0[1]),       \
      [a02] "+v"(a0[2]), [a03] "+v"(a0[3]), [b00] "+v"(b0[0]), [b01] "+v"(b0[1]), [b02] "+v"(b0[2]), [b03] "+v"(b0[3]), \
      [a10] "=&v"(a1[0]), [a11] "=&v"(a1[1]), [a12] "=&v"(a1[2]), [a13] "=&v"(a1[3]), [b10] "=&v"(b1[0]),              \
      [b11] "=&v"(b1[1]), [b12] "=&v"(b1[2]), [b13] "=&v"(b1[3])
#define NK_TN_IN_OPERANDS                                                                                             \
  [ard0] "v"(ard0), [brd0] "v"(brd0), [ard1] "v"(ard1), [brd1] "v"(brd1), [voa] "v"(offa), [vob] "v"(offb),           \
      [rowa] "s"(rowa), [rowb] "s"(rowb), [stra] "s"(stra), [strb] "s"(strb), [dst0] "s"(dst0), [dst1] "s"(dst1)
#define NK_TN_CLOBBERS "memory", "m0", "scc", "s92", "s93", "s94", "s95"
  const int nfull = (kend - kbeg) / TBK;
  int kt_start = 0;
  if (P.kmask == -1 && P.use_asm && nfull >= 1) {
    const uint32_t dst0 = (uint32_t)__builtin_amdgcn_readfirstlane(lds0 + (uint32_t)(wave * TSTRIDE) * 8u);
    const uint32_t dst1 = dst0 + STAGE_B;
    const uint32_t ard1 = ard0 + STAGE_B, brd1 = brd0 + STAGE_B;
    const int steady = nfull - 1;
    uint32_t cnt = (uint32_t)__builtin_amdgcn_readfirstlane((uint32_t)(steady / 2));
    const uint32_t flags =
        (uint32_t)__builtin_amdgcn_readfirstlane((uint32_t)((steady & 1) | (nfull == ktiles ? 2 : 0)));
    kt_start = 2 * (int)cnt + (int)(flags & 1) + (int)(flags >> 1);
    const uint64_t rowa = uniform_u64((uint64_t)(uintptr_t)(opA + (int64_t)(kbeg + TBK + wave) * pr.lda));
    const uint64_t rowb = uniform_u64((uint64_t)(uintptr_t)(opB + (int64_t)(kbeg + TBK + wave) * pr.ldb));
    if (kt_start > 0)
      asm volatile(NK_TN_KSTEPS_ASM
                   : NK_TN_ACC_OPERANDS, [cnt] "+s"(cnt)
                   : NK_TN_IN_OPERANDS, [flags] "s"(flags)
                   : NK_TN_CLOBBERS);
  }
  for (int kt = kt_start; kt < ktiles; ++kt) {
    const int st = kt & 1;
    const bool more = kt + 1 < ktiles;
    frag(st, 1, a1, b1);
    if (more) issue(kt + 1, st ^ 1);
    mma(a0, b0);
    __builtin_amdgcn_sched_barrier(0);
    frag(st, 2, a0, b0);
    __builtin_amdgcn_sched_barrier(0);
    mma(a1, b1);
    __builtin_amdgcn_sched_barrier(0);
    frag(st, 3, a1, b1);
    __builtin_amdgcn_sched_barrier(0);
    mma(a0, b0);
    __builtin_amdgcn_sched_barrier(0);
    dma_wait_all();
    __syncthreads();
    if (more) frag(st ^ 1, 0, a0, b0);
    __builtin_amdgcn_sched_barrier(0);
    mma(a1, b1);
    __builtin_amdgcn_sched_barrier(0);
  }

  if (EPI == 0 && P.splitk == 1) {
    const bool mirror = pr.tri == TRI_UPPER_MIRROR && tm != tn;
#pragma unroll
    for (int i = 0; i < 4; ++i)
#pragma unroll
      for (int j = 0; j < 4; ++j)
#pragma unroll
        for (int reg = 0; reg < 4; ++reg) {
          const int row = tm * TBM + wm * 64 + i * 16 + g4 + 4 * reg;
          const int col = tn * TBM + wn * 64 + j * 16 + r16;
          if (row < pr.M && col < pr.N) {
            double v = pr.alpha * acc[i][j][reg];
            if (pr.beta != 0.0) v += pr.beta * pr.C[(int64_t)row * pr.ldc + col];
            pr.C[(int64_t)row * pr.ldc + col] = v;
            if (mirror) pr.C[(int64_t)col * pr.ldc + row] = v;
            if (pr.Ct) pr.Ct[(int64_t)col * pr.ldct + row] = v;
            if (pr.Caff) {
              pr.Caff[(int64_t)row * pr.ldc + col] = pr.aff_a * v + (row == col ? pr.aff_c : 0.0);
              if (mirror) pr.Caff[(int64_t)col * pr.ldc + row] = pr.aff_a * v;
            }
          }
        }
  } else if (EPI == 0) {
    double* out = P.slab + ((int64_t)gt * P.splitk + split) * (TBM * TBM);
#pragma unroll
    for (int i = 0; i < 4; ++i)
#pragma unroll
      for (int j = 0; j < 4; ++j)
#pragma unroll
        for (int reg = 0; reg < 4; ++reg) {
          const int row = wm * 64 + i * 16 + g4 + 4 * reg;
          const int col = wn * 64 + j * 16 + r16;
          out[row * TBM + col] = acc[i][j][reg];
        }
  } else {
    const bool interior = (tm + 1) * TBM <= pr.M && (tn + 1) * TBM <= pr.N;
    const double exp_ca = exp_nonpos_ca();
    double sb[4];
#pragma unroll
    for (int j = 0; j < 4; ++j) {
      const int col = tn * TBM + wn * 64 + j * 16 + r16;
      sb[j] = (EPI != 3 && col < pr.N) ? P.sqb[col] : 0.0;
    }
#pragma unroll
    for (int i = 0; i < 4; ++i)
#pragma unroll
      for (int reg = 0; reg < 4; ++reg) {
        const int row = tm * TBM + wm * 64 + i * 16 + g4 + 4 * reg;
        if (!interior && row >= pr.M) continue;
        const double sa = EPI != 3 ? P.sqa[row] : 0.0;
        double* orow = P.out + (int64_t)row * P.ldo + tn * TBM + wn * 64 + r16;
#pragma unroll
        for (int j = 0; j < 4; ++j) {
          const double dot = acc[i][j][reg];
          double v;
          if (EPI == 3) {
            v = dot + P.sigma0sq;
          } else {
            const double D = fmax(sa + sb[j] - 2.0 * dot, 0.0);
            if (EPI == 1) {
              v = exp_nonpos(-0.5 * D, exp_ca);
            } else if (EPI == 4) {
              v = tps_value(D);
            } else {
              const double t = sqrt(D) * 2.23606797749978969641;
              v = (1.0 + t + t * t / 3.0) * exp_nonpos(-t, exp_ca);
            }
          }
          if (interior || tn * TBM + wn * 64 + j * 16 + r16 < pr.N) orow[j * 16] = v;
        }
      }
  }
}

template <int EPI>
__global__ void __launch_bounds__(256, 2) gemm_tn_f64_kernel(TnParams P) {
  tn_body<EPI>(P);
}
__global__ void __launch_bounds__(256, 2) gram_fused_f64_kernel(TnParams P) {
  tn_body<0>(P);
}
template <int EPI>
__global__ void __launch_bounds__(256, 2) gemm_tn_f64_kernel_batched(const nk::ArgPack<TnParams>* table) {
  tn_body<EPI>(table[blockIdx.z].v);
}
__global__ void __launch_bounds__(256, 2) gram_fused_f64_kernel_batched(const nk::ArgPack<TnParams>* table) {
  tn_body<0>(table[blockIdx.z].v);
}
#define NK_TN_TWIN(E)                                                                                                   \
  static nk::TwinReg tn_twin_reg_##E(reinterpret_cast<const void*>(static_cast<void (*)(TnParams)>(gemm_tn_f64_kernel<E>)), \
                                     reinterpret_cast<const void*>(gemm_tn_f64_kernel_batched<E>),                        \
                                     sizeof(nk::ArgPack<TnParams>), "gemm_tn_f64_kernel<" #E ">");
NK_TN_TWIN(0) NK_TN_TWIN(1) NK_TN_TWIN(2) NK_TN_TWIN(3) NK_TN_TWIN(4)
static nk::TwinReg gram_fused_twin_reg(reinterpret_cast<const void*>(static_cast<void (*)(TnParams)>(gram_fused_f64_kernel)),
                                       reinterpret_cast<const void*>(gram_fused_f64_kernel_batched),
                                       sizeof(nk::ArgPack<TnParams>), "gram_fused_f64_kernel");

__device__ __forceinline__ void gemm_tn_reduce_kernel_body(const TnRedParams& P) {
  __shared__ double sh[16][130];
  if (P.skip_state != nullptr) {
    const double f = P.skip_state[0];
    if (f != 0.0 && f <= (double)P.skip_step) return;
  }
  const int gt = blockIdx.x / RPARTS, part = blockIdx.x % RPARTS;
  int pi = 0;
#pragma unroll
  for (int q = 1; q < TN_MAXP; ++q)
    if (q < P.nprob && gt >= P.p[q].tile_begin) pi = q;
  const TnRed pr = P.p[pi];
  int tm, tn;
  tn_tile_coords(gt - pr.tile_begin, pr.tri, pr.tiles_n, pr.M, tm, tn);
  typedef double d2 __attribute__((ext_vector_type(2)));
  const double* base = P.slab + (int64_t)gt * P.splitk * (TBM * TBM) + part * (16 * TBM) + threadIdx.x * 2;
  d2 s[4];
#pragma unroll
  for (int i = 0; i < 4; ++i) s[i] = d2{0.0, 0.0};
  for (int k = 0; k < P.splitk; ++k) {
    const double* bk = base + (int64_t)k * (TBM * TBM);
#pragma unroll
    for (int i = 0; i < 4; ++i) s[i] += *reinterpret_cast<const d2*>(bk + 512 * i);
  }
  const bool mirror = pr.tri == TRI_UPPER_MIRROR && tm != tn;
  const bool transposed = mirror || pr.Ct != nullptr;
  const int row0 = tm * TBM + part * 16, col0 = tn * TBM;
  double rsum = 0.0;
#pragma unroll
  for (int i = 0; i < 4; ++i) {
    const int idx = threadIdx.x * 2 + 512 * i;
    const int r = idx >> 7, c = idx & 127;
    const int row = row0 + r;
#pragma unroll
    for (int h = 0; h < 2; ++h) {
      const int col = col0 + c + h;
      double v = 0.0;
      if (row < pr.M && col < pr.N) {
        v = pr.alpha * s[i][h];
        if (pr.beta != 0.0) v += pr.beta * pr.C[(int64_t)row * pr.ldc + col];
        pr.C[(int64_t)row * pr.ldc + col] = v;
        if (pr.Caff) pr.Caff[(int64_t)row * pr.ldc + col] = pr.aff_a * v + (row == col ? pr.aff_c : 0.0);
        const double e = v - (row == col ? 1.0 : 0.0);
        rsum = fma(e, e, rsum);
      }
      if (transposed) sh[r][c + h] = v;
    }
  }
  if (P.resid_partials != nullptr) {
    __shared__ double wsum[4];
#pragma unroll
    for (int off = 32; off > 0; off >>= 1) rsum += __shfl_down(rsum, off, 64);
    if ((threadIdx.x & 63) == 0) wsum[threadIdx.x >> 6] = rsum;
    __syncthreads();
    if (threadIdx.x == 0) {
      const double w = (wsum[0] + wsum[1]) + (wsum[2] + wsum[3]);
      P.resid_partials[blockIdx.x] = mirror ? 2.0 * w : w;
    }
  }
  if (!transposed) return;
  __syncthreads();
  const int c = threadIdx.x >> 1, rb = (threadIdx.x & 1) * 8;
  const int col = col0 + c;
  if (col >= pr.N) return;
#pragma unroll
  for (int q = 0; q < 8; ++q) {
    const int row = row0 + rb + q;
    if (row >= pr.M) break;
    const double v = sh[rb + q][c];
    if (mirror) pr.C[(int64_t)col * pr.ldc + row] = v;
    if (pr.Ct) pr.Ct[(int64_t)col * pr.ldct + row] = v;
    if (mirror && pr.Caff) pr.Caff[(int64_t)col * pr.ldc + row] = pr.aff_a * v;
  }
}
__global__ void __launch_bounds__(256) gemm_tn_reduce_kernel(TnRedParams P) { gemm_tn_reduce_kernel_body(P); }
__global__ void __launch_bounds__(256) gemm_tn_reduce_kernel_batched(const nk::ArgPack<TnRedParams>* table) {
  gemm_tn_reduce_kernel_body(table[blockIdx.z].v);
}
static nk::TwinReg gemm_tn_reduce_twin_reg(reinterpret_cast<const void*>(static_cast<void (*)(TnRedParams)>(gemm_tn_reduce_kernel)),
                                           reinterpret_cast<const void*>(gemm_tn_reduce_kernel_batched),
                                           sizeof(nk::ArgPack<TnRedParams>), "gemm_tn_reduce_kernel");

int launch_tn_reduce(nk_ctx* ctx, const TnRedParams& R, int ntiles) {
  hipLaunchKernelGGL(gemm_tn_reduce_kernel, dim3((unsigned)ntiles * RPARTS), dim3(256), 0, ctx->stream, R);
  NK_HIP(hipGetLastError());
  return NK_OK;
}

__device__ __forceinline__ void transpose_kernel_body(const double* __restrict__ src, int64_t lds_, double* __restrict__ dst, int64_t ldd, int rows, int cols) {
  __shared__ double tile[32][33];
  const int bx = blockIdx.x * 32, by = blockIdx.y * 32;
  const int tx = threadIdx.x & 31, ty = threadIdx.x >> 5;
  for (int r = ty; r < 32; r += 8) {
    const int row = by + r, col = bx + tx;
    if (row < rows && col < cols) tile[r][tx] = src[(int64_t)row * lds_ + col];
  }
  __syncthreads();
  for (int r = ty; r < 32; r += 8) {
    const int orow = bx + r, ocol = by + tx;
    if (orow < cols && ocol < rows) dst[(int64_t)orow * ldd + ocol] = tile[tx][r];
  }
}
__global__ void __launch_bounds__(256) transpose_kernel(const double* __restrict__ src, int64_t lds_, double* __restrict__ dst, int64_t ldd, int rows, int cols) { transpose_kernel_body(src, lds_, dst, ldd, rows, cols); }
NK_BATCHED_TWIN(transpose_kernel, (256), const double*, int64_t, double*, int64_t, int, int)

int launch_transpose(nk_ctx* ctx, const double* src, int64_t lds_, double* dst, int64_t ldd, int rows, int cols) {
  if (rows <= 0 || cols <= 0) return NK_OK;
  dim3 grid((cols + 31) / 32, (rows + 31) / 32);
  hipLaunchKernelGGL(transpose_kernel, grid, dim3(256), 0, ctx->stream, src, lds_, dst, ldd, rows, cols);
  NK_HIP(hipGetLastError());
  return NK_OK;
}

static inline bool aligned16(const void* p) { return (reinterpret_cast<uintptr_t>(p) & 15) == 0; }

bool tn_fast_ok(const TnProblem& p) {
  return p.M >= 2 && p.N >= 2 && aligned16(p.A) && aligned16(p.B) && p.lda % 2 == 0 && p.ldb % 2 == 0 &&
         p.lda >= ((p.M + 1) & ~1) && p.ldb >= ((p.N + 1) & ~1);
}

static bool g_tn_attr_set = false;
static int tn_use_asm() {
  const char* e = getenv("NYSKOOP_TN_ASM");
  return (e && e[0] == '0') ? 0 : 1;
}

int tn_ensure_zero_page(nk_ctx* ctx) {
  if (ctx->d_zeros) return NK_OK;
  NK_HIP(hipMalloc(reinterpret_cast<void**>(&ctx->d_zeros), 4096));
  NK_HIP(hipMemset(ctx->d_zeros, 0, 4096));
  return NK_OK;
}

int launch_gemm_tn_multi(nk_ctx* ctx, const TnProblem* probs, int nprob, int64_t K, int splitk, float* ms_kernel,
                         bool sync_timing, const TnSkip* skip) {
  NK_REQUIRE(nprob >= 1 && nprob <= TN_MAXP, "gemm_tn_multi: 1..4 problems");
  NK_REQUIRE(K >= 0 && K < (1LL << 31), "gemm_tn_multi: K out of range");
  NK_TRY(tn_ensure_zero_page(ctx));
  TnParams P;
  TnRedParams R;
  int ntiles = 0;
  for (int q = 0; q < nprob; ++q) {
    const TnProblem& s = probs[q];
    NK_REQUIRE(tn_fast_ok(s), "gemm_tn_multi: problem %d violates the alignment contract", q);
    NK_REQUIRE(s.tri == TRI_FULL || (s.tri == TRI_UPPER_MIRROR && s.M == s.N), "gemm_tn_multi: bad tri mode");
    const int tmn = (s.M + TBM - 1) / TBM, tnn = (s.N + TBM - 1) / TBM;
    TnDev& d = P.p[q];
    d.A = s.A; d.B = s.B; d.lda = s.lda; d.ldb = s.ldb; d.M = s.M; d.N = s.N;
    d.tiles_n = tnn; d.tri = s.tri; d.ktrim = s.ktrim; d.tile_begin = ntiles;
    d.C = s.C; d.ldc = s.ldc; d.alpha = s.alpha; d.beta = s.beta; d.Ct = s.Ct; d.ldct = s.ldct;
    d.A_even = s.A_even; d.B_even = s.B_even;
    d.Caff = s.Caff; d.aff_a = s.aff_a; d.aff_c = s.aff_c;
    TnRed& r = R.p[q];
    r.Caff = s.Caff; r.aff_a = s.aff_a; r.aff_c = s.aff_c;
    r.Ct = s.Ct; r.ldct = s.ldct;
    r.C = s.C; r.ldc = s.ldc; r.M = s.M; r.N = s.N; r.tiles_n = tnn; r.tri = s.tri; r.tile_begin = ntiles;
    r.alpha = s.alpha; r.beta = s.beta;
    ntiles += s.tri == TRI_FULL ? tmn * tnn : tmn * (tmn + 1) / 2;
  }
  for (int q = nprob; q < TN_MAXP; ++q) {
    P.p[q] = P.p[0];
    P.p[q].tile_begin = 1 << 30;
    R.p[q] = R.p[0];
    R.p[q].tile_begin = 1 << 30;
  }
  const int ktiles_total = (int)((K + TBK - 1) / TBK);
  const bool want_resid = skip && skip->resid_partials != nullptr;
  if (splitk <= 0) {
    const int slots = 2 * ctx->num_cu;
    const int max_split = ktiles_total / 8 > 1 ? ktiles_total / 8 : 1;
    double best = 1e300;
    splitk = 1;
    for (int c = 1; c <= 64 && c <= max_split; ++c) {
      const int64_t wgs = (int64_t)ntiles * c;
      const double steps = (double)((ktiles_total + c - 1) / c);
      const int64_t full = wgs / slots, rem = wgs % slots;
      double t = full * 2.44 * steps;
      if (rem > 0) t += (rem <= ctx->num_cu ? 2.35 : 2.44) * steps;
      t *= 4096.0;
      if (c > 1) t += (double)wgs * (TBM * TBM * 8.0 * 2.0) / 4.0e12 * 2.4e9;
      t += 2000.0 * c / 8.0;
      if (c % 8 == 0) t *= 0.97;
      if (t < best) { best = t; splitk = c; }
    }
  }
  if (want_resid && splitk < 2) splitk = 2;
  if (nprob >= 3 && getenv("NYSKOOP_TN_SPLITK")) splitk = atoi(getenv("NYSKOOP_TN_SPLITK"));
  P.kmask = getenv("NYSKOOP_TN_KMASK") ? (int)strtol(getenv("NYSKOOP_TN_KMASK"), nullptr, 0) : -1;
  P.use_asm = tn_use_asm();
  P.nprob = nprob; P.ntiles = ntiles; P.K = (int)K; P.splitk = splitk;
  P.klen = ((ktiles_total + splitk - 1) / splitk) * TBK;
  if (P.klen == 0) P.klen = TBK;
  P.zeros = ctx->d_zeros;
  const ArenaMark mark = arena_mark(ctx);
  double* slab = nullptr;
  if (splitk > 1) NK_TRY(arena_alloc_t(ctx, (size_t)ntiles * splitk * TBM * TBM, &slab));
  P.slab = slab;
  R.nprob = nprob; R.splitk = splitk; R.slab = slab;
  P.skip_state = R.skip_state = skip ? skip->state : nullptr;
  P.skip_step = R.skip_step = skip ? skip->step : 0;
  P.select_state = skip ? skip->select : nullptr;
  R.resid_partials = (skip && splitk > 1 && nprob == 1) ? skip->resid_partials : nullptr;
  if (skip && skip->resid_count) *skip->resid_count = R.resid_partials ? ntiles * RPARTS : 0;
  if (!g_tn_attr_set) {
    NK_HIP(hipFuncSetAttribute(reinterpret_cast<const void*>(gemm_tn_f64_kernel<0>),
                               hipFuncAttributeMaxDynamicSharedMemorySize, TN_LDS_BYTES));
    NK_HIP(hipFuncSetAttribute(reinterpret_cast<const void*>(gram_fused_f64_kernel),
                               hipFuncAttributeMaxDynamicSharedMemorySize, TN_LDS_BYTES));
    NK_HIP(hipFuncSetAttribute(reinterpret_cast<const void*>(gemm_tn_f64_kernel<1>),
                               hipFuncAttributeMaxDynamicSharedMemorySize, TN_LDS_BYTES));
    NK_HIP(hipFuncSetAttribute(reinterpret_cast<const void*>(gemm_tn_f64_kernel<2>),
                               hipFuncAttributeMaxDynamicSharedMemorySize, TN_LDS_BYTES));
    NK_HIP(hipFuncSetAttribute(reinterpret_cast<const void*>(gemm_tn_f64_kernel<3>),
                               hipFuncAttributeMaxDynamicSharedMemorySize, TN_LDS_BYTES));
    NK_HIP(hipFuncSetAttribute(reinterpret_cast<const void*>(gemm_tn_f64_kernel<4>),
                               hipFuncAttributeMaxDynamicSharedMemorySize, TN_LDS_BYTES));
    NK_HIP(hipFuncSetAttribute(reinterpret_cast<const void*>(gemm_tn_f64_kernel_batched<0>),
                               hipFuncAttributeMaxDynamicSharedMemorySize, TN_LDS_BYTES));
    NK_HIP(hipFuncSetAttribute(reinterpret_cast<const void*>(gemm_tn_f64_kernel_batched<1>),
                               hipFuncAttributeMaxDynamicSharedMemorySize, TN_LDS_BYTES));
    NK_HIP(hipFuncSetAttribute(reinterpret_cast<const void*>(gemm_tn_f64_kernel_batched<2>),
                               hipFuncAttributeMaxDynamicSharedMemorySize, TN_LDS_BYTES));
    NK_HIP(hipFuncSetAttribute(reinterpret_cast<const void*>(gemm_tn_f64_kernel_batched<3>),
                               hipFuncAttributeMaxDynamicSharedMemorySize, TN_LDS_BYTES));
    NK_HIP(hipFuncSetAttribute(reinterpret_cast<const void*>(gemm_tn_f64_kernel_batched<4>),
                               hipFuncAttributeMaxDynamicSharedMemorySize, TN_LDS_BYTES));
    NK_HIP(hipFuncSetAttribute(reinterpret_cast<const void*>(gram_fused_f64_kernel_batched),
                               hipFuncAttributeMaxDynamicSharedMemorySize, TN_LDS_BYTES));
    g_tn_attr_set = true;
  }
  if (ms_kernel) NK_HIP(hipEventRecord(ctx->ev[EV_GEMM_T0], ctx->stream));
  P.sqa = P.sqb = nullptr; P.out = nullptr; P.ldo = 0; P.ktype = 0; P.sigma0sq = 0.0;
  if (nprob >= 3)
    hipLaunchKernelGGL(gram_fused_f64_kernel, dim3((unsigned)(ntiles * splitk)), dim3(256), TN_LDS_BYTES, ctx->stream, P);
  else
    hipLaunchKernelGGL(gemm_tn_f64_kernel<0>, dim3((unsigned)(ntiles * splitk)), dim3(256), TN_LDS_BYTES, ctx->stream, P);
  NK_HIP(hipGetLastError());
  if (ms_kernel) NK_HIP(hipEventRecord(ctx->ev[EV_GEMM_T1], ctx->stream));
  if (splitk > 1) {
    hipLaunchKernelGGL(gemm_tn_reduce_kernel, dim3((unsigned)ntiles * RPARTS), dim3(256), 0, ctx->stream, R);
    NK_HIP(hipGetLastError());
  }
  if (ms_kernel && sync_timing) {
    NK_HIP(hipEventSynchronize(ctx->ev[EV_GEMM_T1]));
    NK_HIP(hipEventElapsedTime(ms_kernel, ctx->ev[EV_GEMM_T0], ctx->ev[EV_GEMM_T1]));
  }
  arena_release(ctx, mark);
  return NK_OK;
}


__device__ __forceinline__ void prep_rows_kernel_body(const double* __restrict__ X, int64_t ldx, int rows, int d, const double* __restrict__ winv, const double* __restrict__ center, double* __restrict__ Xt, int64_t ldt) {
  __shared__ double tile[32][33];
  const int k0 = blockIdx.x * 32, r0 = blockIdx.y * 32;
  const int tx = threadIdx.x & 31, ty = threadIdx.x >> 5;
  for (int r = ty; r < 32; r += 8) {
    const int row = r0 + r, k = k0 + tx;
    if (row < rows && k < d) tile[r][tx] = (X[(int64_t)row * ldx + k] - center[k]) * winv[k];
  }
  __syncthreads();
  for (int r = ty; r < 32; r += 8) {
    const int k = k0 + r, row = r0 + tx;
    if (k < d && row < rows) Xt[(int64_t)k * ldt + row] = tile[tx][r];
  }
}
__global__ void __launch_bounds__(256) prep_rows_kernel(const double* __restrict__ X, int64_t ldx, int rows, int d, const double* __restrict__ winv, const double* __restrict__ center, double* __restrict__ Xt, int64_t ldt) { prep_rows_kernel_body(X, ldx, rows, d, winv, center, Xt, ldt); }
NK_BATCHED_TWIN(prep_rows_kernel, (256), const double*, int64_t, int, int, const double*, const double*, double*, int64_t)
__device__ __forceinline__ void colsq_kernel_body(const double* __restrict__ Xt, int64_t ldt, int rows, int d, double* __restrict__ sq) {
  __shared__ double part[4][64];
  const int lane = threadIdx.x & 63, w = threadIdx.x >> 6;
  const int i = blockIdx.x * 64 + lane;
  double s0 = 0.0, s1 = 0.0, s2 = 0.0, s3 = 0.0;
  if (i < rows) {
    int k = w;
    for (; k + 12 < d; k += 16) {
      const double v0 = Xt[(int64_t)k * ldt + i], v1 = Xt[(int64_t)(k + 4) * ldt + i];
      const double v2 = Xt[(int64_t)(k + 8) * ldt + i], v3 = Xt[(int64_t)(k + 12) * ldt + i];
      s0 = fma(v0, v0, s0); s1 = fma(v1, v1, s1); s2 = fma(v2, v2, s2); s3 = fma(v3, v3, s3);
    }
    for (; k < d; k += 4) {
      const double v = Xt[(int64_t)k * ldt + i];
      s0 = fma(v, v, s0);
    }
  }
  part[w][lane] = (s0 + s1) + (s2 + s3);
  __syncthreads();
  if (w == 0 && i < rows) sq[i] = (part[0][lane] + part[1][lane]) + (part[2][lane] + part[3][lane]);
}
__global__ void __launch_bounds__(256) colsq_kernel(const double* __restrict__ Xt, int64_t ldt, int rows, int d, double* __restrict__ sq) { colsq_kernel_body(Xt, ldt, rows, d, sq); }
NK_BATCHED_TWIN(colsq_kernel, (256), const double*, int64_t, int, int, double*)
__device__ __forceinline__ void colsum_partial_kernel_body(const double* __restrict__ Z, int64_t ldz, int rows, int d, int rows_per_chunk, double* __restrict__ partial) {
  const int k = blockIdx.x * blockDim.x + threadIdx.x;
  if (k >= d) return;
  const int r0 = blockIdx.y * rows_per_chunk;
  const int r1 = min(rows, r0 + rows_per_chunk);
  double s = 0.0;
  for (int r = r0; r < r1; ++r) s += Z[(int64_t)r * ldz + k];
  partial[(int64_t)blockIdx.y * d + k] = s;
}
__global__ void __launch_bounds__(256) colsum_partial_kernel(const double* __restrict__ Z, int64_t ldz, int rows, int d, int rows_per_chunk, double* __restrict__ partial) { colsum_partial_kernel_body(Z, ldz, rows, d, rows_per_chunk, partial); }
NK_BATCHED_TWIN(colsum_partial_kernel, (256), const double*, int64_t, int, int, int, double*)
__device__ __forceinline__ void colmean_finish_kernel_body(const double* __restrict__ partial, int chunks, int rows, int d, double* __restrict__ mean) {
  const int k = blockIdx.x * blockDim.x + threadIdx.x;
  if (k >= d) return;
  double s = 0.0;
  for (int c = 0; c < chunks; ++c) s += partial[(int64_t)c * d + k];
  mean[k] = s / rows;
}
__global__ void __launch_bounds__(256) colmean_finish_kernel(const double* __restrict__ partial, int chunks, int rows, int d, double* __restrict__ mean) { colmean_finish_kernel_body(partial, chunks, rows, d, mean); }
NK_BATCHED_TWIN(colmean_finish_kernel, (256), const double*, int, int, int, double*)

int launch_colmean(nk_ctx* ctx, const double* Z, int64_t ldz, int rows, int d, double* mean) {
  const ArenaMark mk = arena_mark(ctx);
  const int rpc = 32;
  const int chunks = (rows + rpc - 1) / rpc;
  double* partial = nullptr;
  NK_TRY(arena_alloc_t(ctx, (size_t)chunks * d, &partial));
  hipLaunchKernelGGL(colsum_partial_kernel, dim3((d + 255) / 256, chunks), dim3(256), 0, ctx->stream, Z, ldz, rows, d, rpc,
                     partial);
  hipLaunchKernelGGL(colmean_finish_kernel, dim3((d + 255) / 256), dim3(256), 0, ctx->stream, partial, chunks, rows, d, mean);
  NK_HIP(hipGetLastError());
  arena_release(ctx, mk);
  return NK_OK;
}

int prep_rows(nk_ctx* ctx, const double* X, int64_t ldx, int64_t rows, int d, const double* winv, const double* center,
              double* Xt, int64_t ldt, double* sq) {
  dim3 grid((d + 31) / 32, (unsigned)((rows + 31) / 32));
  hipLaunchKernelGGL(prep_rows_kernel, grid, dim3(256), 0, ctx->stream, X, ldx, (int)rows, d, winv, center, Xt, ldt);
  hipLaunchKernelGGL(colsq_kernel, dim3((unsigned)((rows + 63) / 64)), dim3(256), 0, ctx->stream, Xt, ldt, (int)rows, d, sq);
  NK_HIP(hipGetLastError());
  return NK_OK;
}

int launch_kmat_gram(nk_ctx* ctx, int ktype, const double* At, int64_t ldat, const double* sqa, int64_t nA,
                     const double* Bt, int64_t ldbt, const double* sqb, int64_t nB, int d, double sigma0, double* out,
                     int64_t ldo) {
  NK_TRY(tn_ensure_zero_page(ctx));
  TnProblem tp;
  tp.A = At; tp.B = Bt; tp.lda = ldat; tp.ldb = ldbt; tp.M = (int)nA; tp.N = (int)nB;
  NK_REQUIRE(tn_fast_ok(tp), "kmat_gram: operands violate the alignment contract");
  TnParams P;
  P.skip_state = nullptr; P.skip_step = 0; P.select_state = nullptr;
  const int tmn = (int)((nA + TBM - 1) / TBM), tnn = (int)((nB + TBM - 1) / TBM);
  TnDev& dv = P.p[0];
  dv.A = At; dv.B = Bt; dv.lda = ldat; dv.ldb = ldbt; dv.M = (int)nA; dv.N = (int)nB; dv.tiles_n = tnn; dv.tri = TRI_FULL;
  dv.tile_begin = 0; dv.ktrim = KTRIM_NONE; dv.A_even = dv.B_even = nullptr; dv.Caff = nullptr; dv.aff_a = dv.aff_c = 0.0;
  dv.C = nullptr; dv.ldc = 0; dv.alpha = 1.0; dv.beta = 0.0; dv.Ct = nullptr; dv.ldct = 0;
  for (int q = 1; q < TN_MAXP; ++q) { P.p[q] = P.p[0]; P.p[q].tile_begin = 1 << 30; }
  P.nprob = 1; P.ntiles = tmn * tnn; P.K = d; P.splitk = 1; P.kmask = -1; P.use_asm = tn_use_asm();
  P.klen = ((d + TBK - 1) / TBK) * TBK;
  P.zeros = ctx->d_zeros; P.slab = nullptr;
  P.sqa = sqa; P.sqb = sqb; P.out = out; P.ldo = ldo; P.ktype = ktype; P.sigma0sq = sigma0 * sigma0;
  if (!g_tn_attr_set) {
    NK_HIP(hipFuncSetAttribute(reinterpret_cast<const void*>(gemm_tn_f64_kernel<0>),
                               hipFuncAttributeMaxDynamicSharedMemorySize, TN_LDS_BYTES));
    NK_HIP(hipFuncSetAttribute(reinterpret_cast<const void*>(gram_fused_f64_kernel),
                               hipFuncAttributeMaxDynamicSharedMemorySize, TN_LDS_BYTES));
    NK_HIP(hipFuncSetAttribute(reinterpret_cast<const void*>(gemm_tn_f64_kernel<1>),
                               hipFuncAttributeMaxDynamicSharedMemorySize, TN_LDS_BYTES));
    NK_HIP(hipFuncSetAttribute(reinterpret_cast<const void*>(gemm_tn_f64_kernel<2>),
                               hipFuncAttributeMaxDynamicSharedMemorySize, TN_LDS_BYTES));
    NK_HIP(hipFuncSetAttribute(reinterpret_cast<const void*>(gemm_tn_f64_kernel<3>),
                               hipFuncAttributeMaxDynamicSharedMemorySize, TN_LDS_BYTES));
    NK_HIP(hipFuncSetAttribute(reinterpret_cast<const void*>(gemm_tn_f64_kernel<4>),
                               hipFuncAttributeMaxDynamicSharedMemorySize, TN_LDS_BYTES));
    NK_HIP(hipFuncSetAttribute(reinterpret_cast<const void*>(gemm_tn_f64_kernel_batched<0>),
                               hipFuncAttributeMaxDynamicSharedMemorySize, TN_LDS_BYTES));
    NK_HIP(hipFuncSetAttribute(reinterpret_cast<const void*>(gemm_tn_f64_kernel_batched<1>),
                               hipFuncAttributeMaxDynamicSharedMemorySize, TN_LDS_BYTES));
    NK_HIP(hipFuncSetAttribute(reinterpret_cast<const void*>(gemm_tn_f64_kernel_batched<2>),
                               hipFuncAttributeMaxDynamicSharedMemorySize, TN_LDS_BYTES));
    NK_HIP(hipFuncSetAttribute(reinterpret_cast<const void*>(gemm_tn_f64_kernel_batched<3>),
                               hipFuncAttributeMaxDynamicSharedMemorySize, TN_LDS_BYTES));
    NK_HIP(hipFuncSetAttribute(reinterpret_cast<const void*>(gemm_tn_f64_kernel_batched<4>),
                               hipFuncAttributeMaxDynamicSharedMemorySize, TN_LDS_BYTES));
    NK_HIP(hipFuncSetAttribute(reinterpret_cast<const void*>(gram_fused_f64_kernel_batched),
                               hipFuncAttributeMaxDynamicSharedMemorySize, TN_LDS_BYTES));
    g_tn_attr_set = true;
  }
  const unsigned grid = 8u * (unsigned)tmn * (unsigned)((tnn + 7) / 8);
  if (ktype == NK_KERNEL_RBF)
    hipLaunchKernelGGL(gemm_tn_f64_kernel<1>, dim3(grid), dim3(256), TN_LDS_BYTES, ctx->stream, P);
  else if (ktype == NK_KERNEL_MATERN52)
    hipLaunchKernelGGL(gemm_tn_f64_kernel<2>, dim3(grid), dim3(256), TN_LDS_BYTES, ctx->stream, P);
  else if (ktype == NK_KERNEL_TPS)
    hipLaunchKernelGGL(gemm_tn_f64_kernel<4>, dim3(grid), dim3(256), TN_LDS_BYTES, ctx->stream, P);
  else
    hipLaunchKernelGGL(gemm_tn_f64_kernel<3>, dim3(grid), dim3(256), TN_LDS_BYTES, ctx->stream, P);
  NK_HIP(hipGetLastError());
  return NK_OK;
}

}
```

Baseline: 24.48.

## Fuse K_in/K_out kernel-block GEMMs into one launch with persistent row runs

Builds both Nyström kernel blocks (X vs Zin and Y vs Zout) in a single fused gemm_tn launch instead of two, with each workgroup walking a run of consecutive row tiles (default 4) for a fixed column tile. Per-problem sq norms and output pointers move into the per-problem descriptor, and the epilogue is restructured so the next tile's first DMA can overlap. This removes one launch and the serialization between the two blocks, and is meant to reuse B-tile data across row runs. In exchange the kernel gets more complex control flow and register pressure, the input block now waits for Y prep before starting, and an env var can fall back to the old path. It also adds a new nk_kernel_blocks API.

After: 24.54 (median of 5 runs). No clear change (+0.2%).

```diff
diff --git a/include/nyskoop.h b/include/nyskoop.h
--- a/include/nyskoop.h
+++ b/include/nyskoop.h
@@ -119,6 +119,11 @@
                      const double* B, int64_t ldb, int64_t nB,
                      double* out, int64_t ldo);
 
+int nk_kernel_blocks(nk_ctx* ctx, const nk_kernel_desc* kd,
+                     const double* X, int64_t ldx, const double* Y, int64_t ldy, int64_t n,
+                     const double* Zin, int64_t ldzi, const double* Zout, int64_t ldzo, int32_t m,
+                     double* out_in, double* out_out, int64_t ldo);
+
 int nk_nystrom_fit(nk_ctx* ctx, const nk_kernel_desc* kd,
                    const double* X, int64_t ldx, const double* Y, int64_t ldy,
                    int64_t n, int32_t d, int32_t p,
diff --git a/nys_koop_lqr_amd/_lib.py b/nys_koop_lqr_amd/_lib.py
--- a/nys_koop_lqr_amd/_lib.py
+++ b/nys_koop_lqr_amd/_lib.py
@@ -101,6 +101,8 @@
     "nk_host_alloc": (_P, [C.c_uint64]),
     "nk_host_free": (None, [_P]),
     "nk_kernel_matrix": (C.c_int, [_P, C.POINTER(KernelDesc), _P, _I64, _I64, _P, _I64, _I64, _P, _I64]),
+    "nk_kernel_blocks": (C.c_int, [_P, C.POINTER(KernelDesc), _P, _I64, _P, _I64, _I64, _P, _I64, _P, _I64, _I32, _P, _P,
+                                   _I64]),
     "nk_nystrom_fit": (C.c_int, [_P, C.POINTER(KernelDesc), _P, _I64, _P, _I64, _I64, _I32, _I32,
                                  C.POINTER(_I64), _I32, _P, _I64, _P, _I64, _I32, _D, _D,
                                  C.POINTER(_P), C.POINTER(FitStats)]),
diff --git a/nys_koop_lqr_amd/csrc/nk_api.hip b/nys_koop_lqr_amd/csrc/nk_api.hip
--- a/nys_koop_lqr_amd/csrc/nk_api.hip
+++ b/nys_koop_lqr_amd/csrc/nk_api.hip
@@ -653,6 +653,56 @@
   return NK_OK;
 }
 
+int nk_kernel_blocks(nk_ctx* ctx, const nk_kernel_desc* kd, const double* X, int64_t ldx, const double* Y, int64_t ldy,
+                     int64_t n, const double* Zin, int64_t ldzi, const double* Zout, int64_t ldzo, int32_t m, double* out_in,
+                     double* out_out, int64_t ldo) {
+  NK_TRY(check_ctx(ctx));
+  NK_REQUIRE(kd && X && Y && Zin && Zout && out_in && out_out, "nk_kernel_blocks: null argument");
+  NK_REQUIRE(kd->type != NK_KERNEL_TPS && kd->d >= 32 && n >= 2 && m >= 2, "nk_kernel_blocks: needs d >= 32, n >= 2, m >= 2");
+  const int d = kd->d;
+  NK_REQUIRE(ldx >= d && ldy >= d && ldzi >= d && ldzo >= d && ldo >= m, "nk_kernel_blocks: leading dimension too small");
+  double *winv = nullptr, *center = nullptr, *Xt = nullptr, *Yt = nullptr, *Zti = nullptr, *Zto = nullptr;
+  double *sqx = nullptr, *sqy = nullptr, *sqzi = nullptr, *sqzo = nullptr;
+  const int64_t ldt = (n + 1) & ~(int64_t)1, ldzt = (m + 1) & ~1;
+  NK_TRY(arena_alloc_t(ctx, (size_t)d, &winv));
+  NK_TRY(make_winv(ctx, kd, d, winv));
+  MatIn x, y, zi, zo;
+  NK_TRY(stage_in(ctx, X, ldx, n, d, &x));
+  NK_TRY(stage_in(ctx, Y, ldy, n, d, &y));
+  NK_TRY(stage_in(ctx, Zin, ldzi, m, d, &zi));
+  NK_TRY(stage_in(ctx, Zout, ldzo, m, d, &zo));
+  MatOut oi, oo;
+  NK_TRY(stage_out(ctx, out_in, ldo, n, m, &oi));
+  NK_TRY(stage_out(ctx, out_out, ldo, n, m, &oo));
+  NK_TRY(arena_alloc_t(ctx, (size_t)d, &center));
+  NK_TRY(arena_alloc_t(ctx, (size_t)d * ldt, &Xt));
+  NK_TRY(arena_alloc_t(ctx, (size_t)d * ldt, &Yt));
+  NK_TRY(arena_alloc_t(ctx, (size_t)d * ldzt, &Zti));
+  NK_TRY(arena_alloc_t(ctx, (size_t)d * ldzt, &Zto));
+  NK_TRY(arena_alloc_t(ctx, (size_t)n, &sqx));
+  NK_TRY(arena_alloc_t(ctx, (size_t)n, &sqy));
+  NK_TRY(arena_alloc_t(ctx, (size_t)m, &sqzi));
+  NK_TRY(arena_alloc_t(ctx, (size_t)m, &sqzo));
+  if (kd->type == NK_KERNEL_LINEAR) NK_TRY(launch_fill(ctx, center, d, 1, d, 0.0));
+  else NK_TRY(launch_colmean(ctx, zo.ptr, zo.ld, m, d, center));
+  NK_TRY(prep_rows(ctx, zo.ptr, zo.ld, m, d, winv, center, Zto, ldzt, sqzo));
+  NK_TRY(prep_rows(ctx, zi.ptr, zi.ld, m, d, winv, center, Zti, ldzt, sqzi));
+  NK_TRY(prep_rows(ctx, x.ptr, x.ld, n, d, winv, center, Xt, ldt, sqx));
+  NK_TRY(prep_rows(ctx, y.ptr, y.ld, n, d, winv, center, Yt, ldt, sqy));
+  if (kb_pair_enabled()) {
+    const KmatGramProblem bin{Xt, ldt, sqx, Zti, ldzt, sqzi, oi.dev, oi.ld};
+    const KmatGramProblem bout{Yt, ldt, sqy, Zto, ldzt, sqzo, oo.dev, oo.ld};
+    NK_TRY(launch_kmat_gram_pair(ctx, kd->type, bin, bout, n, m, d, kd->sigma0));
+  } else {
+    NK_TRY(launch_kmat_gram(ctx, kd->type, Xt, ldt, sqx, n, Zti, ldzt, sqzi, m, d, kd->sigma0, oi.dev, oi.ld));
+    NK_TRY(launch_kmat_gram(ctx, kd->type, Yt, ldt, sqy, n, Zto, ldzt, sqzo, m, d, kd->sigma0, oo.dev, oo.ld));
+  }
+  NK_TRY(finish_out(ctx, oi));
+  NK_TRY(finish_out(ctx, oo));
+  NK_HIP(hipStreamSynchronize(ctx->stream));
+  return NK_OK;
+}
+
 int nk_model_create(nk_ctx* ctx, const nk_kernel_desc* kd, const double* Zout, int64_t ldz, int32_t m, int32_t d,
                     int32_t p, double jitter, const double* A, const double* B, const double* C, const double* W,
                     nk_model** model) {
diff --git a/nys_koop_lqr_amd/csrc/nk_common.h b/nys_koop_lqr_amd/csrc/nk_common.h
--- a/nys_koop_lqr_amd/csrc/nk_common.h
+++ b/nys_koop_lqr_amd/csrc/nk_common.h
@@ -232,7 +232,7 @@
 int group_leave(nk_ctx* c);
 void group_stats(nk_ctx* c, uint64_t out[4]);
 enum { CNT_CHAIN_GIVEUP = 0, CNT_JACOBI_GIVEUP = 1, CNT_RANK_TRUNCATED = 2, CNT_SQRT_RETRY = 3, CNT_REFINED = 4,
-       CNT_CHOL_FLOW_GIVEUP = 5, CNT_CHOL_FLOW = 6, CNT_N = 7 };
+       CNT_CHOL_FLOW_GIVEUP = 5, CNT_CHOL_FLOW = 6, CNT_KB_PAIR = 7, CNT_N = 8 };
 void count_event(int which);
 uint64_t read_counter(int which);
 hipError_t real_stream_sync(hipStream_t s);
@@ -493,6 +493,17 @@
 int launch_kmat_gram(nk_ctx* ctx, int ktype, const double* At, int64_t ldat, const double* sqa, int64_t nA,
                      const double* Bt, int64_t ldbt, const double* sqb, int64_t nB, int d, double sigma0, double* out,
                      int64_t ldo);
+struct KmatGramProblem {
+  const double* At; int64_t ldat; const double* sqa;
+  const double* Bt; int64_t ldbt; const double* sqb;
+  double* out; int64_t ldo;
+};
+int launch_kmat_gram_pair(nk_ctx* ctx, int ktype, const KmatGramProblem& in, const KmatGramProblem& outp, int64_t nA,
+                          int64_t nB, int d, double sigma0);
+inline bool kb_pair_enabled() {
+  const char* e = getenv("NYSKOOP_KB_PAIR");
+  return !(e && e[0] == '0');
+}
 }
 
 #if defined(__HIPCC__)
diff --git a/nys_koop_lqr_amd/csrc/nk_fit.hip b/nys_koop_lqr_amd/csrc/nk_fit.hip
--- a/nys_koop_lqr_amd/csrc/nk_fit.hip
+++ b/nys_koop_lqr_amd/csrc/nk_fit.hip
@@ -156,7 +156,7 @@
   float ms_gram_kernel = 0.f;
   int gram_launches = 0;
   bool gram_deferred = false, timed = false;
-  bool f32 = false, overlap_prep = false, multi_pass = false, pipelined = false;
+  bool f32 = false, overlap_prep = false, kb_pair = false, multi_pass = false, pipelined = false;
   KernelBlocks kb;
   std::vector<std::vector<Piece>> passes;
   int64_t f_rows = 0, maxlen = 0, ldt32 = 0, ldzt32 = 0, ldy32 = 0;
@@ -307,6 +307,7 @@
   kb.ldt = (maxlen + 1) & ~(int64_t)1;
   kb.ldzt = (m + 1) & ~1;
   overlap_prep = kb.gram_form && passes.size() == 1 && passes[0].size() == 1;
+  kb_pair = kb_pair_enabled();
   if (kb.gram_form) {
     NK_TRY(arena_alloc_t(ctx, (size_t)d, &kb.center));
     if (!f32) {
@@ -421,10 +422,17 @@
     NK_HIP(hipEventRecord(ctx->ev[EV_YPREP_DONE], ctx->stream));
   }
   NK_TRY(prep_rows(ctx, xs, x.ld, pc.len, d, mdl->winv, kb.center, kb.Rt, kb.ldt, kb.sqr));
-  NK_TRY(launch_kmat_gram(ctx, kd->type, kb.Rt, kb.ldt, kb.sqr, pc.len, kb.Zti, kb.ldzt, kb.sqzi, m, d, kd->sigma0, Fo, kb.ldf));
-  NK_HIP(hipStreamWaitEvent(ctx->stream, ctx->ev[EV_YPREP_DONE], 0));
-  NK_TRY(launch_kmat_gram(ctx, kd->type, Rt2, kb.ldt, sqr2, pc.len, kb.Zto, kb.ldzt, kb.sqzo, m, d, kd->sigma0,
-                          Fo + kb.off_out, kb.ldf));
+  if (kb_pair) {
+    NK_HIP(hipStreamWaitEvent(ctx->stream, ctx->ev[EV_YPREP_DONE], 0));
+    const KmatGramProblem bin{kb.Rt, kb.ldt, kb.sqr, kb.Zti, kb.ldzt, kb.sqzi, Fo, kb.ldf};
+    const KmatGramProblem bout{Rt2, kb.ldt, sqr2, kb.Zto, kb.ldzt, kb.sqzo, Fo + kb.off_out, kb.ldf};
+    NK_TRY(launch_kmat_gram_pair(ctx, kd->type, bin, bout, pc.len, m, d, kd->sigma0));
+  } else {
+    NK_TRY(launch_kmat_gram(ctx, kd->type, kb.Rt, kb.ldt, kb.sqr, pc.len, kb.Zti, kb.ldzt, kb.sqzi, m, d, kd->sigma0, Fo, kb.ldf));
+    NK_HIP(hipStreamWaitEvent(ctx->stream, ctx->ev[EV_YPREP_DONE], 0));
+    NK_TRY(launch_kmat_gram(ctx, kd->type, Rt2, kb.ldt, sqr2, pc.len, kb.Zto, kb.ldzt, kb.sqzo, m, d, kd->sigma0,
+                            Fo + kb.off_out, kb.ldf));
+  }
   return kb.copy_inputs(ctx, xs, x.ld, pc.len, Fo);
 }
 
diff --git a/nys_koop_lqr_amd/csrc/nk_gemm_tn.hip b/nys_koop_lqr_amd/csrc/nk_gemm_tn.hip
--- a/nys_koop_lqr_amd/csrc/nk_gemm_tn.hip
+++ b/nys_koop_lqr_amd/csrc/nk_gemm_tn.hip
@@ -32,6 +32,8 @@
   const double* B_even;
   double* Caff;
   double aff_a, aff_c;
+  const double* sqa;
+  const double* sqb;
 };
 struct TnParams {
   TnDev p[TN_MAXP];
@@ -45,10 +47,7 @@
   const double* skip_state;
   int skip_step;
   const double* select_state;
-  const double* sqa;
-  const double* sqb;
-  double* out;
-  int64_t ldo;
+  int run, stagger;
   int ktype;
   double sigma0sq;
 };
@@ -72,20 +71,28 @@
   const int split = blockIdx.x % P.splitk;
   const int gt = blockIdx.x / P.splitk;
   int pi = 0;
-#pragma unroll
-  for (int q = 1; q < TN_MAXP; ++q)
-    if (q < P.nprob && gt >= P.p[q].tile_begin) pi = q;
-  const TnDev pr = P.p[pi];
-  int tm, tn;
+  int tm, tn, tm_end;
   if (EPI >= 1) {
     const int xcd = blockIdx.x & 7, i = blockIdx.x >> 3;
-    const int cols = (pr.tiles_n - xcd + 7) >> 3;
+    const int cols = (P.p[0].tiles_n - xcd + 7) >> 3;
     if (cols <= 0) return;
-    tm = i / cols;
-    tn = xcd + 8 * (i - tm * cols);
-    if (tm * TBM >= pr.M) return;
+    const int ctot = cols * P.nprob;
+    const int r = i / ctot, c = i - r * ctot;
+    pi = c >= cols ? 1 : 0;
+    tn = xcd + 8 * (c - pi * cols);
+    const int half = (P.stagger && (c & 1)) ? P.run >> 1 : 0;
+    tm = max(r * P.run - half, 0);
+    tm_end = min((r + 1) * P.run - half, (P.p[0].M + TBM - 1) / TBM);
+    if (tm >= tm_end) return;
   } else {
+#pragma unroll
+    for (int q = 1; q < TN_MAXP; ++q)
+      if (q < P.nprob && gt >= P.p[q].tile_begin) pi = q;
+  }
+  const TnDev pr = P.p[pi];
+  if (EPI == 0) {
     tn_tile_coords(gt - pr.tile_begin, pr.tri, pr.tiles_n, pr.M, tm, tn);
+    tm_end = tm + 1;
   }
   const int lane = threadIdx.x & 63;
   const int wave = __builtin_amdgcn_readfirstlane(threadIdx.x >> 6);
@@ -99,13 +106,17 @@
     if (pr.A_even) opA = pr.A_even;
     if (pr.B_even) opB = pr.B_even;
   }
-  int kbeg = split * P.klen;
-  int kend = min(P.K, kbeg + P.klen);
-  if (pr.ktrim == KTRIM_B_UPPER) kend = min(kend, (tn + 1) * TBM);
-  if (pr.ktrim == KTRIM_A_LOWER) kbeg = max(kbeg, tm * TBM);
-  const int ktiles = kend > kbeg ? (kend - kbeg + TBK - 1) / TBK : 0;
-
-  const uint32_t offa = (uint32_t)min(tm * TBM + lane * 2, (pr.M - 1) & ~1) * 8u;
+  int kbeg = 0, kend = 0, ktiles = 0;
+  uint32_t offa = 0;
+  auto set_tile = [&](int t) {
+    kbeg = split * P.klen;
+    kend = min(P.K, kbeg + P.klen);
+    if (pr.ktrim == KTRIM_B_UPPER) kend = min(kend, (tn + 1) * TBM);
+    if (pr.ktrim == KTRIM_A_LOWER) kbeg = max(kbeg, t * TBM);
+    ktiles = kend > kbeg ? (kend - kbeg + TBK - 1) / TBK : 0;
+    offa = (uint32_t)min(t * TBM + lane * 2, (pr.M - 1) & ~1) * 8u;
+  };
+  set_tile(tm);
   const uint32_t offb = (uint32_t)min(tn * TBM + lane * 2, (pr.N - 1) & ~1) * 8u;
   const uint32_t offz = (uint32_t)lane * 16u;
 
@@ -138,11 +149,6 @@
   };
 
   d4 acc[4][4];
-#pragma unroll
-  for (int i = 0; i < 4; ++i)
-#pragma unroll
-    for (int j = 0; j < 4; ++j) acc[i][j] = d4{0.0, 0.0, 0.0, 0.0};
-
   const int wm = wave >> 1, wn = wave & 1;
   const int r16 = lane & 15, g4 = lane >> 4;
 
@@ -161,13 +167,6 @@
       for (int j = 0; j < 4; ++j)
         acc[i][j] = __builtin_amdgcn_mfma_f64_16x16x4f64(a[i], b[j], acc[i][j], 0, 0, 0);
   };
-  double a0[4], b0[4], a1[4], b1[4];
-  if (ktiles > 0) {
-    issue(0, 0);
-    dma_wait_all();
-    __syncthreads();
-    frag(0, 0, a0, b0);
-  }
   const uint32_t ard0 = lds0 + (uint32_t)(wm * 64 + r16 + g4 * TSTRIDE) * 8u;
   const uint32_t brd0 = lds0 + (uint32_t)(TBK * TSTRIDE + wn * 64 + r16 + g4 * TSTRIDE) * 8u;
   constexpr uint32_t STAGE_B = (uint32_t)TSTAGE * 8u;
@@ -185,119 +184,164 @@
   [ard0] "v"(ard0), [brd0] "v"(brd0), [ard1] "v"(ard1), [brd1] "v"(brd1), [voa] "v"(offa), [vob] "v"(offb),           \
       [rowa] "s"(rowa), [rowb] "s"(rowb), [stra] "s"(stra), [strb] "s"(strb), [dst0] "s"(dst0), [dst1] "s"(dst1)
 #define NK_TN_CLOBBERS "memory", "m0", "scc", "s92", "s93", "s94", "s95"
-  const int nfull = (kend - kbeg) / TBK;
-  int kt_start = 0;
-  if (P.kmask == -1 && P.use_asm && nfull >= 1) {
-    const uint32_t dst0 = (uint32_t)__builtin_amdgcn_readfirstlane(lds0 + (uint32_t)(wave * TSTRIDE) * 8u);
-    const uint32_t dst1 = dst0 + STAGE_B;
-    const uint32_t ard1 = ard0 + STAGE_B, brd1 = brd0 + STAGE_B;
-    const int steady = nfull - 1;
-    uint32_t cnt = (uint32_t)__builtin_amdgcn_readfirstlane((uint32_t)(steady / 2));
-    const uint32_t flags =
-        (uint32_t)__builtin_amdgcn_readfirstlane((uint32_t)((steady & 1) | (nfull == ktiles ? 2 : 0)));
-    kt_start = 2 * (int)cnt + (int)(flags & 1) + (int)(flags >> 1);
-    const uint64_t rowa = uniform_u64((uint64_t)(uintptr_t)(opA + (int64_t)(kbeg + TBK + wave) * pr.lda));
-    const uint64_t rowb = uniform_u64((uint64_t)(uintptr_t)(opB + (int64_t)(kbeg + TBK + wave) * pr.ldb));
-    if (kt_start > 0)
-      asm volatile(NK_TN_KSTEPS_ASM
-                   : NK_TN_ACC_OPERANDS, [cnt] "+s"(cnt)
-                   : NK_TN_IN_OPERANDS, [flags] "s"(flags)
-                   : NK_TN_CLOBBERS);
-  }
-  for (int kt = kt_start; kt < ktiles; ++kt) {
-    const int st = kt & 1;
-    const bool more = kt + 1 < ktiles;
-    frag(st, 1, a1, b1);
-    if (more) issue(kt + 1, st ^ 1);
-    mma(a0, b0);
-    __builtin_amdgcn_sched_barrier(0);
-    frag(st, 2, a0, b0);
-    __builtin_amdgcn_sched_barrier(0);
-    mma(a1, b1);
-    __builtin_amdgcn_sched_barrier(0);
-    frag(st, 3, a1, b1);
-    __builtin_amdgcn_sched_barrier(0);
-    mma(a0, b0);
-    __builtin_amdgcn_sched_barrier(0);
-    dma_wait_all();
-    __syncthreads();
-    if (more) frag(st ^ 1, 0, a0, b0);
-    __builtin_amdgcn_sched_barrier(0);
-    mma(a1, b1);
-    __builtin_amdgcn_sched_barrier(0);
-  }
-
-  if (EPI == 0 && P.splitk == 1) {
-    const bool mirror = pr.tri == TRI_UPPER_MIRROR && tm != tn;
+  double a0[4], b0[4], a1[4], b1[4];
+  double sqa_t[4][4], sqb_t[4];
+  bool fetched = false;
+  for (;;) {
 #pragma unroll
     for (int i = 0; i < 4; ++i)
 #pragma unroll
-      for (int j = 0; j < 4; ++j)
+      for (int j = 0; j < 4; ++j) acc[i][j] = d4{0.0, 0.0, 0.0, 0.0};
+    if (EPI >= 1) {
+#pragma unroll
+      for (int j = 0; j < 4; ++j) {
+        const int col = tn * TBM + wn * 64 + j * 16 + r16;
+        sqb_t[j] = (EPI != 3 && col < pr.N) ? pr.sqb[col] : 0.0;
+      }
+#pragma unroll
+      for (int i = 0; i < 4; ++i)
 #pragma unroll
         for (int reg = 0; reg < 4; ++reg) {
           const int row = tm * TBM + wm * 64 + i * 16 + g4 + 4 * reg;
-          const int col = tn * TBM + wn * 64 + j * 16 + r16;
-          if (row < pr.M && col < pr.N) {
-            double v = pr.alpha * acc[i][j][reg];
-            if (pr.beta != 0.0) v += pr.beta * pr.C[(int64_t)row * pr.ldc + col];
-            pr.C[(int64_t)row * pr.ldc + col] = v;
-            if (mirror) pr.C[(int64_t)col * pr.ldc + row] = v;
-            if (pr.Ct) pr.Ct[(int64_t)col * pr.ldct + row] = v;
-            if (pr.Caff) {
-              pr.Caff[(int64_t)row * pr.ldc + col] = pr.aff_a * v + (row == col ? pr.aff_c : 0.0);
-              if (mirror) pr.Caff[(int64_t)col * pr.ldc + row] = pr.aff_a * v;
+          sqa_t[i][reg] = (EPI != 3 && row < pr.M) ? pr.sqa[row] : 0.0;
+        }
+    }
+    if (ktiles > 0) {
+      if (!fetched) issue(0, 0);
+      dma_wait_all();
+      __syncthreads();
+      frag(0, 0, a0, b0);
+    }
+    if (EPI >= 1) {
+#pragma unroll
+      for (int j = 0; j < 4; ++j) asm volatile("" : "+v"(sqb_t[j]));
+#pragma unroll
+      for (int i = 0; i < 4; ++i)
+#pragma unroll
+        for (int reg = 0; reg < 4; ++reg) asm volatile("" : "+v"(sqa_t[i][reg]));
+    }
+    bool stage0_busy = false;
+    const int nfull = (kend - kbeg) / TBK;
+    int kt_start = 0;
+    if (P.kmask == -1 && P.use_asm && nfull >= 1) {
+      const uint32_t dst0 = (uint32_t)__builtin_amdgcn_readfirstlane(lds0 + (uint32_t)(wave * TSTRIDE) * 8u);
+      const uint32_t dst1 = dst0 + STAGE_B;
+      const uint32_t ard1 = ard0 + STAGE_B, brd1 = brd0 + STAGE_B;
+      const int steady = nfull - 1;
+      uint32_t cnt = (uint32_t)__builtin_amdgcn_readfirstlane((uint32_t)(steady / 2));
+      const uint32_t flags =
+          (uint32_t)__builtin_amdgcn_readfirstlane((uint32_t)((steady & 1) | (nfull == ktiles ? 2 : 0)));
+      kt_start = 2 * (int)cnt + (int)(flags & 1) + (int)(flags >> 1);
+      const uint64_t rowa = uniform_u64((uint64_t)(uintptr_t)(opA + (int64_t)(kbeg + TBK + wave) * pr.lda));
+      const uint64_t rowb = uniform_u64((uint64_t)(uintptr_t)(opB + (int64_t)(kbeg + TBK + wave) * pr.ldb));
+      stage0_busy = (flags >> 1) != 0 && ((nfull - 1) & 1) == 0;
+      if (kt_start > 0)
+        asm volatile(NK_TN_KSTEPS_ASM
+                     : NK_TN_ACC_OPERANDS, [cnt] "+s"(cnt)
+                     : NK_TN_IN_OPERANDS, [flags] "s"(flags)
+                     : NK_TN_CLOBBERS);
+    }
+    for (int kt = kt_start; kt < ktiles; ++kt) {
+      const int st = kt & 1;
+      const bool more = kt + 1 < ktiles;
+      frag(st, 1, a1, b1);
+      if (more) issue(kt + 1, st ^ 1);
+      mma(a0, b0);
+      __builtin_amdgcn_sched_barrier(0);
+      frag(st, 2, a0, b0);
+      __builtin_amdgcn_sched_barrier(0);
+      mma(a1, b1);
+      __builtin_amdgcn_sched_barrier(0);
+      frag(st, 3, a1, b1);
+      __builtin_amdgcn_sched_barrier(0);
+      mma(a0, b0);
+      __builtin_amdgcn_sched_barrier(0);
+      dma_wait_all();
+      __syncthreads();
+      if (more) frag(st ^ 1, 0, a0, b0);
+      __builtin_amdgcn_sched_barrier(0);
+      mma(a1, b1);
+      __builtin_amdgcn_sched_barrier(0);
+    }
+
+    const bool next_tile = EPI >= 1 && tm + 1 < tm_end;
+    if (next_tile) {
+      set_tile(tm + 1);
+      if (ktiles > 0) {
+        if (stage0_busy) __syncthreads();
+        issue(0, 0);
+      }
+      fetched = true;
+    }
+
+    if (EPI == 0 && P.splitk == 1) {
+      const bool mirror = pr.tri == TRI_UPPER_MIRROR && tm != tn;
+#pragma unroll
+      for (int i = 0; i < 4; ++i)
+#pragma unroll
+        for (int j = 0; j < 4; ++j)
+#pragma unroll
+          for (int reg = 0; reg < 4; ++reg) {
+            const int row = tm * TBM + wm * 64 + i * 16 + g4 + 4 * reg;
+            const int col = tn * TBM + wn * 64 + j * 16 + r16;
+            if (row < pr.M && col < pr.N) {
+              double v = pr.alpha * acc[i][j][reg];
+              if (pr.beta != 0.0) v += pr.beta * pr.C[(int64_t)row * pr.ldc + col];
+              pr.C[(int64_t)row * pr.ldc + col] = v;
+              if (mirror) pr.C[(int64_t)col * pr.ldc + row] = v;
+              if (pr.Ct) pr.Ct[(int64_t)col * pr.ldct + row] = v;
+              if (pr.Caff) {
+                pr.Caff[(int64_t)row * pr.ldc + col] = pr.aff_a * v + (row == col ? pr.aff_c : 0.0);
+                if (mirror) pr.Caff[(int64_t)col * pr.ldc + row] = pr.aff_a * v;
+              }
             }
           }
+    } else if (EPI == 0) {
+      double* out = P.slab + ((int64_t)gt * P.splitk + split) * (TBM * TBM);
+#pragma unroll
+      for (int i = 0; i < 4; ++i)
+#pragma unroll
+        for (int j = 0; j < 4; ++j)
+#pragma unroll
+          for (int reg = 0; reg < 4; ++reg) {
+            const int row = wm * 64 + i * 16 + g4 + 4 * reg;
+            const int col = wn * 64 + j * 16 + r16;
+            out[row * TBM + col] = acc[i][j][reg];
+          }
+    } else {
+      const bool interior = (tm + 1) * TBM <= pr.M && (tn + 1) * TBM <= pr.N;
+      const double exp_ca = exp_nonpos_ca();
+#pragma unroll
+      for (int i = 0; i < 4; ++i)
+#pragma unroll
+        for (int reg = 0; reg < 4; ++reg) {
+          const int row = tm * TBM + wm * 64 + i * 16 + g4 + 4 * reg;
+          if (!interior && row >= pr.M) continue;
+          const double sa = sqa_t[i][reg];
+          double* orow = pr.C + (int64_t)row * pr.ldc + tn * TBM + wn * 64 + r16;
+#pragma unroll
+          for (int j = 0; j < 4; ++j) {
+            const double dot = acc[i][j][reg];
+            double v;
+            if (EPI == 3) {
+              v = dot + P.sigma0sq;
+            } else {
+              const double D = fmax(sa + sqb_t[j] - 2.0 * dot, 0.0);
+              if (EPI == 1) {
+                v = exp_nonpos(-0.5 * D, exp_ca);
+              } else if (EPI == 4) {
+                v = tps_value(D);
+              } else {
+                const double t = sqrt(D) * 2.23606797749978969641;
+                v = (1.0 + t + t * t / 3.0) * exp_nonpos(-t, exp_ca);
+              }
+            }
+            if (interior || tn * TBM + wn * 64 + j * 16 + r16 < pr.N) orow[j * 16] = v;
+          }
         }
-  } else if (EPI == 0) {
-    double* out = P.slab + ((int64_t)gt * P.splitk + split) * (TBM * TBM);
-#pragma unroll
-    for (int i = 0; i < 4; ++i)
-#pragma unroll
-      for (int j = 0; j < 4; ++j)
-#pragma unroll
-        for (int reg = 0; reg < 4; ++reg) {
-          const int row = wm * 64 + i * 16 + g4 + 4 * reg;
-          const int col = wn * 64 + j * 16 + r16;
-          out[row * TBM + col] = acc[i][j][reg];
-        }
-  } else {
-    const bool interior = (tm + 1) * TBM <= pr.M && (tn + 1) * TBM <= pr.N;
-    const double exp_ca = exp_nonpos_ca();
-    double sb[4];
-#pragma unroll
-    for (int j = 0; j < 4; ++j) {
-      const int col = tn * TBM + wn * 64 + j * 16 + r16;
-      sb[j] = (EPI != 3 && col < pr.N) ? P.sqb[col] : 0.0;
-    }
-#pragma unroll
-    for (int i = 0; i < 4; ++i)
-#pragma unroll
-      for (int reg = 0; reg < 4; ++reg) {
-        const int row = tm * TBM + wm * 64 + i * 16 + g4 + 4 * reg;
-        if (!interior && row >= pr.M) continue;
-        const double sa = EPI != 3 ? P.sqa[row] : 0.0;
-        double* orow = P.out + (int64_t)row * P.ldo + tn * TBM + wn * 64 + r16;
-#pragma unroll
-        for (int j = 0; j < 4; ++j) {
-          const double dot = acc[i][j][reg];
-          double v;
-          if (EPI == 3) {
-            v = dot + P.sigma0sq;
-          } else {
-            const double D = fmax(sa + sb[j] - 2.0 * dot, 0.0);
-            if (EPI == 1) {
-              v = exp_nonpos(-0.5 * D, exp_ca);
-            } else if (EPI == 4) {
-              v = tps_value(D);
-            } else {
-              const double t = sqrt(D) * 2.23606797749978969641;
-              v = (1.0 + t + t * t / 3.0) * exp_nonpos(-t, exp_ca);
-            }
-          }
-          if (interior || tn * TBM + wn * 64 + j * 16 + r16 < pr.N) orow[j * 16] = v;
-        }
-      }
+    }
+    if (!next_tile) break;
+    ++tm;
   }
 }
 
@@ -445,6 +489,35 @@
 }
 
 static bool g_tn_attr_set = false;
+static int tn_set_attributes() {
+  if (g_tn_attr_set) return NK_OK;
+  NK_HIP(hipFuncSetAttribute(reinterpret_cast<const void*>(gemm_tn_f64_kernel<0>),
+                             hipFuncAttributeMaxDynamicSharedMemorySize, TN_LDS_BYTES));
+  NK_HIP(hipFuncSetAttribute(reinterpret_cast<const void*>(gram_fused_f64_kernel),
+                             hipFuncAttributeMaxDynamicSharedMemorySize, TN_LDS_BYTES));
+  NK_HIP(hipFuncSetAttribute(reinterpret_cast<const void*>(gemm_tn_f64_kernel<1>),
+                             hipFuncAttributeMaxDynamicSharedMemorySize, TN_LDS_BYTES));
+  NK_HIP(hipFuncSetAttribute(reinterpret_cast<const void*>(gemm_tn_f64_kernel<2>),
+                             hipFuncAttributeMaxDynamicSharedMemorySize, TN_LDS_BYTES));
+  NK_HIP(hipFuncSetAttribute(reinterpret_cast<const void*>(gemm_tn_f64_kernel<3>),
+                             hipFuncAttributeMaxDynamicSharedMemorySize, TN_LDS_BYTES));
+  NK_HIP(hipFuncSetAttribute(reinterpret_cast<const void*>(gemm_tn_f64_kernel<4>),
+                             hipFuncAttributeMaxDynamicSharedMemorySize, TN_LDS_BYTES));
+  NK_HIP(hipFuncSetAttribute(reinterpret_cast<const void*>(gemm_tn_f64_kernel_batched<0>),
+                             hipFuncAttributeMaxDynamicSharedMemorySize, TN_LDS_BYTES));
+  NK_HIP(hipFuncSetAttribute(reinterpret_cast<const void*>(gemm_tn_f64_kernel_batched<1>),
+                             hipFuncAttributeMaxDynamicSharedMemorySize, TN_LDS_BYTES));
+  NK_HIP(hipFuncSetAttribute(reinterpret_cast<const void*>(gemm_tn_f64_kernel_batched<2>),
+                             hipFuncAttributeMaxDynamicSharedMemorySize, TN_LDS_BYTES));
+  NK_HIP(hipFuncSetAttribute(reinterpret_cast<const void*>(gemm_tn_f64_kernel_batched<3>),
+                             hipFuncAttributeMaxDynamicSharedMemorySize, TN_LDS_BYTES));
+  NK_HIP(hipFuncSetAttribute(reinterpret_cast<const void*>(gemm_tn_f64_kernel_batched<4>),
+                             hipFuncAttributeMaxDynamicSharedMemorySize, TN_LDS_BYTES));
+  NK_HIP(hipFuncSetAttribute(reinterpret_cast<const void*>(gram_fused_f64_kernel_batched),
+                             hipFuncAttributeMaxDynamicSharedMemorySize, TN_LDS_BYTES));
+  g_tn_attr_set = true;
+  return NK_OK;
+}
 static int tn_use_asm() {
   const char* e = getenv("NYSKOOP_TN_ASM");
   return (e && e[0] == '0') ? 0 : 1;
@@ -476,6 +549,7 @@
     d.C = s.C; d.ldc = s.ldc; d.alpha = s.alpha; d.beta = s.beta; d.Ct = s.Ct; d.ldct = s.ldct;
     d.A_even = s.A_even; d.B_even = s.B_even;
     d.Caff = s.Caff; d.aff_a = s.aff_a; d.aff_c = s.aff_c;
+    d.sqa = d.sqb = nullptr;
     TnRed& r = R.p[q];
     r.Caff = s.Caff; r.aff_a = s.aff_a; r.aff_c = s.aff_c;
     r.Ct = s.Ct; r.ldct = s.ldct;
@@ -527,35 +601,9 @@
   P.select_state = skip ? skip->select : nullptr;
   R.resid_partials = (skip && splitk > 1 && nprob == 1) ? skip->resid_partials : nullptr;
   if (skip && skip->resid_count) *skip->resid_count = R.resid_partials ? ntiles * RPARTS : 0;
-  if (!g_tn_attr_set) {
-    NK_HIP(hipFuncSetAttribute(reinterpret_cast<const void*>(gemm_tn_f64_kernel<0>),
-                               hipFuncAttributeMaxDynamicSharedMemorySize, TN_LDS_BYTES));
-    NK_HIP(hipFuncSetAttribute(reinterpret_cast<const void*>(gram_fused_f64_kernel),
-                               hipFuncAttributeMaxDynamicSharedMemorySize, TN_LDS_BYTES));
-    NK_HIP(hipFuncSetAttribute(reinterpret_cast<const void*>(gemm_tn_f64_kernel<1>),
-                               hipFuncAttributeMaxDynamicSharedMemorySize, TN_LDS_BYTES));
-    NK_HIP(hipFuncSetAttribute(reinterpret_cast<const void*>(gemm_tn_f64_kernel<2>),
-                               hipFuncAttributeMaxDynamicSharedMemorySize, TN_LDS_BYTES));
-    NK_HIP(hipFuncSetAttribute(reinterpret_cast<const void*>(gemm_tn_f64_kernel<3>),
-                               hipFuncAttributeMaxDynamicSharedMemorySize, TN_LDS_BYTES));
-    NK_HIP(hipFuncSetAttribute(reinterpret_cast<const void*>(gemm_tn_f64_kernel<4>),
-                               hipFuncAttributeMaxDynamicSharedMemorySize, TN_LDS_BYTES));
-    NK_HIP(hipFuncSetAttribute(reinterpret_cast<const void*>(gemm_tn_f64_kernel_batched<0>),
-                               hipFuncAttributeMaxDynamicSharedMemorySize, TN_LDS_BYTES));
-    NK_HIP(hipFuncSetAttribute(reinterpret_cast<const void*>(gemm_tn_f64_kernel_batched<1>),
-                               hipFuncAttributeMaxDynamicSharedMemorySize, TN_LDS_BYTES));
-    NK_HIP(hipFuncSetAttribute(reinterpret_cast<const void*>(gemm_tn_f64_kernel_batched<2>),
-                               hipFuncAttributeMaxDynamicSharedMemorySize, TN_LDS_BYTES));
-    NK_HIP(hipFuncSetAttribute(reinterpret_cast<const void*>(gemm_tn_f64_kernel_batched<3>),
-                               hipFuncAttributeMaxDynamicSharedMemorySize, TN_LDS_BYTES));
-    NK_HIP(hipFuncSetAttribute(reinterpret_cast<const void*>(gemm_tn_f64_kernel_batched<4>),
-                               hipFuncAttributeMaxDynamicSharedMemorySize, TN_LDS_BYTES));
-    NK_HIP(hipFuncSetAttribute(reinterpret_cast<const void*>(gram_fused_f64_kernel_batched),
-                               hipFuncAttributeMaxDynamicSharedMemorySize, TN_LDS_BYTES));
-    g_tn_attr_set = true;
-  }
+  NK_TRY(tn_set_attributes());
   if (ms_kernel) NK_HIP(hipEventRecord(ctx->ev[EV_GEMM_T0], ctx->stream));
-  P.sqa = P.sqb = nullptr; P.out = nullptr; P.ldo = 0; P.ktype = 0; P.sigma0sq = 0.0;
+  P.run = 1; P.stagger = 0; P.ktype = 0; P.sigma0sq = 0.0;
   if (nprob >= 3)
     hipLaunchKernelGGL(gram_fused_f64_kernel, dim3((unsigned)(ntiles * splitk)), dim3(256), TN_LDS_BYTES, ctx->stream, P);
   else
@@ -658,53 +706,31 @@
   return NK_OK;
 }
 
-int launch_kmat_gram(nk_ctx* ctx, int ktype, const double* At, int64_t ldat, const double* sqa, int64_t nA,
-                     const double* Bt, int64_t ldbt, const double* sqb, int64_t nB, int d, double sigma0, double* out,
-                     int64_t ldo) {
+static int launch_kmat_gram_probs(nk_ctx* ctx, int ktype, const KmatGramProblem* probs, int nprob, int64_t nA, int64_t nB,
+                                  int d, double sigma0, int run, int stagger) {
   NK_TRY(tn_ensure_zero_page(ctx));
-  TnProblem tp;
-  tp.A = At; tp.B = Bt; tp.lda = ldat; tp.ldb = ldbt; tp.M = (int)nA; tp.N = (int)nB;
-  NK_REQUIRE(tn_fast_ok(tp), "kmat_gram: operands violate the alignment contract");
   TnParams P;
   P.skip_state = nullptr; P.skip_step = 0; P.select_state = nullptr;
   const int tmn = (int)((nA + TBM - 1) / TBM), tnn = (int)((nB + TBM - 1) / TBM);
-  TnDev& dv = P.p[0];
-  dv.A = At; dv.B = Bt; dv.lda = ldat; dv.ldb = ldbt; dv.M = (int)nA; dv.N = (int)nB; dv.tiles_n = tnn; dv.tri = TRI_FULL;
-  dv.tile_begin = 0; dv.ktrim = KTRIM_NONE; dv.A_even = dv.B_even = nullptr; dv.Caff = nullptr; dv.aff_a = dv.aff_c = 0.0;
-  dv.C = nullptr; dv.ldc = 0; dv.alpha = 1.0; dv.beta = 0.0; dv.Ct = nullptr; dv.ldct = 0;
-  for (int q = 1; q < TN_MAXP; ++q) { P.p[q] = P.p[0]; P.p[q].tile_begin = 1 << 30; }
-  P.nprob = 1; P.ntiles = tmn * tnn; P.K = d; P.splitk = 1; P.kmask = -1; P.use_asm = tn_use_asm();
+  for (int q = 0; q < nprob; ++q) {
+    const KmatGramProblem& s = probs[q];
+    TnProblem tp;
+    tp.A = s.At; tp.B = s.Bt; tp.lda = s.ldat; tp.ldb = s.ldbt; tp.M = (int)nA; tp.N = (int)nB;
+    NK_REQUIRE(tn_fast_ok(tp), "kmat_gram: operands violate the alignment contract");
+    TnDev& dv = P.p[q];
+    dv.A = s.At; dv.B = s.Bt; dv.lda = s.ldat; dv.ldb = s.ldbt; dv.M = (int)nA; dv.N = (int)nB; dv.tiles_n = tnn;
+    dv.tri = TRI_FULL; dv.tile_begin = 0; dv.ktrim = KTRIM_NONE; dv.A_even = dv.B_even = nullptr; dv.Caff = nullptr;
+    dv.aff_a = dv.aff_c = 0.0; dv.C = s.out; dv.ldc = s.ldo; dv.alpha = 1.0; dv.beta = 0.0; dv.Ct = nullptr; dv.ldct = 0;
+    dv.sqa = s.sqa; dv.sqb = s.sqb;
+  }
+  for (int q = nprob; q < TN_MAXP; ++q) { P.p[q] = P.p[0]; P.p[q].tile_begin = 1 << 30; }
+  P.nprob = nprob; P.ntiles = nprob * tmn * tnn; P.K = d; P.splitk = 1; P.kmask = -1; P.use_asm = tn_use_asm();
   P.klen = ((d + TBK - 1) / TBK) * TBK;
   P.zeros = ctx->d_zeros; P.slab = nullptr;
-  P.sqa = sqa; P.sqb = sqb; P.out = out; P.ldo = ldo; P.ktype = ktype; P.sigma0sq = sigma0 * sigma0;
-  if (!g_tn_attr_set) {
-    NK_HIP(hipFuncSetAttribute(reinterpret_cast<const void*>(gemm_tn_f64_kernel<0>),
-                               hipFuncAttributeMaxDynamicSharedMemorySize, TN_LDS_BYTES));
-    NK_HIP(hipFuncSetAttribute(reinterpret_cast<const void*>(gram_fused_f64_kernel),
-                               hipFuncAttributeMaxDynamicSharedMemorySize, TN_LDS_BYTES));
-    NK_HIP(hipFuncSetAttribute(reinterpret_cast<const void*>(gemm_tn_f64_kernel<1>),
-                               hipFuncAttributeMaxDynamicSharedMemorySize, TN_LDS_BYTES));
-    NK_HIP(hipFuncSetAttribute(reinterpret_cast<const void*>(gemm_tn_f64_kernel<2>),
-                               hipFuncAttributeMaxDynamicSharedMemorySize, TN_LDS_BYTES));
-    NK_HIP(hipFuncSetAttribute(reinterpret_cast<const void*>(gemm_tn_f64_kernel<3>),
-                               hipFuncAttributeMaxDynamicSharedMemorySize, TN_LDS_BYTES));
-    NK_HIP(hipFuncSetAttribute(reinterpret_cast<const void*>(gemm_tn_f64_kernel<4>),
-                               hipFuncAttributeMaxDynamicSharedMemorySize, TN_LDS_BYTES));
-    NK_HIP(hipFuncSetAttribute(reinterpret_cast<const void*>(gemm_tn_f64_kernel_batched<0>),
-                               hipFuncAttributeMaxDynamicSharedMemorySize, TN_LDS_BYTES));
-    NK_HIP(hipFuncSetAttribute(reinterpret_cast<const void*>(gemm_tn_f64_kernel_batched<1>),
-                               hipFuncAttributeMaxDynamicSharedMemorySize, TN_LDS_BYTES));
-    NK_HIP(hipFuncSetAttribute(reinterpret_cast<const void*>(gemm_tn_f64_kernel_batched<2>),
-                               hipFuncAttributeMaxDynamicSharedMemorySize, TN_LDS_BYTES));
-    NK_HIP(hipFuncSetAttribute(reinterpret_cast<const void*>(gemm_tn_f64_kernel_batched<3>),
-                               hipFuncAttributeMaxDynamicSharedMemorySize, TN_LDS_BYTES));
-    NK_HIP(hipFuncSetAttribute(reinterpret_cast<const void*>(gemm_tn_f64_kernel_batched<4>),
-                               hipFuncAttributeMaxDynamicSharedMemorySize, TN_LDS_BYTES));
-    NK_HIP(hipFuncSetAttribute(reinterpret_cast<const void*>(gram_fused_f64_kernel_batched),
-                               hipFuncAttributeMaxDynamicSharedMemorySize, TN_LDS_BYTES));
-    g_tn_attr_set = true;
-  }
-  const unsigned grid = 8u * (unsigned)tmn * (unsigned)((tnn + 7) / 8);
+  P.run = run; P.stagger = stagger; P.ktype = ktype; P.sigma0sq = sigma0 * sigma0;
+  NK_TRY(tn_set_attributes());
+  const int runs = (tmn + (stagger ? run / 2 : 0) + run - 1) / run;
+  const unsigned grid = 8u * (unsigned)runs * (unsigned)(nprob * ((tnn + 7) / 8));
   if (ktype == NK_KERNEL_RBF)
     hipLaunchKernelGGL(gemm_tn_f64_kernel<1>, dim3(grid), dim3(256), TN_LDS_BYTES, ctx->stream, P);
   else if (ktype == NK_KERNEL_MATERN52)
@@ -717,4 +743,25 @@
   return NK_OK;
 }
 
-}
+int launch_kmat_gram(nk_ctx* ctx, int ktype, const double* At, int64_t ldat, const double* sqa, int64_t nA,
+                     const double* Bt, int64_t ldbt, const double* sqb, int64_t nB, int d, double sigma0, double* out,
+                     int64_t ldo) {
+  const KmatGramProblem pb{At, ldat, sqa, Bt, ldbt, sqb, out, ldo};
+  return launch_kmat_gram_probs(ctx, ktype, &pb, 1, nA, nB, d, sigma0, 1, 0);
+}
+
+#ifndef NK_KB_RUN
+#define NK_KB_RUN 4
+#endif
+#ifndef NK_KB_STAGGER
+#define NK_KB_STAGGER 0
+#endif
+int launch_kmat_gram_pair(nk_ctx* ctx, int ktype, const KmatGramProblem& in, const KmatGramProblem& outp, int64_t nA,
+                          int64_t nB, int d, double sigma0) {
+  static_assert(NK_KB_RUN >= 1 && (NK_KB_STAGGER == 0 || NK_KB_RUN % 2 == 0), "staggered runs start with half a run");
+  const KmatGramProblem pb[2] = {in, outp};
+  count_event(CNT_KB_PAIR);
+  return launch_kmat_gram_probs(ctx, ktype, pb, 2, nA, nB, d, sigma0, NK_KB_RUN, NK_KB_STAGGER);
+}
+
+}
```
